# alexlee-gk/video_prediction

Measured on AMD Instinct MI355X. Metric: train frames/sec (whole node), BAIR 64x64 seq30 SAVP, higher is better.
Workload: dtype bf16

## Files before the change

include/savp_hip.h:

```cpp
#ifndef SAVP_HIP_H
#define SAVP_HIP_H

#include <stdint.h>

#ifdef __cplusplus
extern "C" {
#endif

#define SAVP_OK 0
#define SAVP_EINVAL (-1)
#define SAVP_ELAUNCH (-2)

const char* savp_version(void);

int savp_set_option(const char* name, int32_t value);
int savp_get_option(const char* name, int32_t* value);

int savp_allreduce_bucket(void* comm, void* stream, void* buf, int64_t count);

int savp_prof_event_create(void** ev);
int savp_prof_event_destroy(void* ev);
int savp_prof_arm(void* start, void* stop);
int savp_prof_armed(void);
int savp_prof_elapsed_us(void* start, void* stop, float* us);

enum { SAVP_CONV_FPROP = 0, SAVP_CONV_DGRAD = 1, SAVP_CONV_WGRAD = 2 };
enum { SAVP_PREC_F32 = 0, SAVP_PREC_BF16 = 1 };
enum { SAVP_ACT_NONE = 0, SAVP_ACT_LRELU = 1, SAVP_ACT_SIGMOID = 2, SAVP_ACT_DLRELU_FROM_OUT = 3 };

typedef struct SavpConvArgs {
    int32_t mode;
    int32_t N, D, H, W, Cx;
    int32_t Do, Ho, Wo, Cy;
    int32_t kd, kh, kw;
    int32_t sd, sh, sw;
    int32_t pd, ph, pw;
    int32_t beta;
    int32_t act;
    float alpha;
    int32_t splitk;
    int32_t tile;
    int32_t precision;
    void* x; int64_t x_sn, x_sd, x_sh, x_sw;
    void* y; int64_t y_sn, y_sd, y_sh, y_sw;
    void* w;
    const float* bias;
    const float* aux;
    const void* w_bf16;
    int32_t src_bf16;
    int32_t out_bf16;
    double* stats;
    void* ws; int64_t ws_bytes;
    int32_t dst_gap_at, dst_gap;
    const float* nb_x; int64_t nb_x_sn, nb_x_sp;
    const float *nb_mean, *nb_rstd;
    const float *nb_gamma, *nb_beta;
    double* nb_ws;
    int32_t nb_c0, nb_nc, nb_act; float nb_alpha;
    const void* w_frag;
    const void* w_frag_il;
} SavpConvArgs;

int savp_conv(void* stream, const SavpConvArgs* args);

int savp_tiled_z_weff(void* stream, const float* w, int32_t kh, int32_t kw, int32_t ph, int32_t pw, int32_t Cin, int32_t Cout,
                      int32_t z0, int32_t nz, float* weff);
int savp_tiled_z_grad(void* stream, const void* dy, int32_t dy_bf16, int64_t nimg, int32_t H, int32_t W, int32_t C,
                      const float* weff, int32_t nz, float* dz, int32_t beta, void* ws, int64_t ws_bytes);
int64_t savp_tiled_z_workspace_bytes(int64_t nimg, int32_t C);
int savp_conv_stats_ok(const SavpConvArgs* args);
int64_t savp_conv_workspace_bytes(const SavpConvArgs* args);
int savp_conv_special(const SavpConvArgs* args);


typedef struct SavpView { void* p; int64_t sn; int64_t sp; } SavpView;

typedef struct SavpInormArgs {
    int32_t N, HW, C;
    int32_t act; float alpha; float eps;
    SavpView x;
    const float* gamma; const float* beta;
    int32_t nout; SavpView out[4];
    float* mean; float* rstd;
    int32_t ndy; SavpView dy[4];
    SavpView dx; int32_t dx_beta;
    double* dgamma; double* dbeta;
    void* ws;
    int32_t ws_clean;
    int32_t out_c0[4], out_nc[4];
    int32_t dy_c0[4], dy_nc[4];
    int32_t out_bf16;
    int32_t stats_ready;
    const float* stats_shift;
    int32_t dx_bf16;
} SavpInormArgs;
int savp_instnorm_act_fwd(void* stream, const SavpInormArgs* a);
int savp_instnorm_act_bwd(void* stream, const SavpInormArgs* a);

typedef struct SavpGnormArgs {
    SavpInormArgs norm;
    int32_t G;
    double* ws_group;
    double* dsum;
} SavpGnormArgs;
int savp_groupnorm_act_fwd(void* stream, const SavpGnormArgs* a);
int savp_groupnorm_act_bwd(void* stream, const SavpGnormArgs* a);

typedef struct SavpLnLstmArgs {
    int32_t N, HW, F; float forget_bias;
    const float* gn;
    SavpView c_prev;
    float* c_pre;
    const float* cn;
    int32_t nh; SavpView h[4]; int32_t h_bf16;
    int32_t ndh; SavpView dh[4];
    const float* dc_new;
    float* dcn;
    float* dgn;
    const float* dc_pre;
    float* dc_prev;
} SavpLnLstmArgs;
int savp_lnlstm_fwd(void* stream, const SavpLnLstmArgs* a, int32_t stage);
int savp_lnlstm_bwd(void* stream, const SavpLnLstmArgs* a, int32_t stage);

typedef struct SavpLstmArgs {
    int32_t N, HW, F;
    float eps, forget_bias;
    const void* gates;
    SavpView c_prev;
    const float *gamma1, *beta1, *gamma2, *beta2;
    float* c_new;
    int32_t nh; SavpView h[4];
    float *mean1, *rstd1, *mean2, *rstd2;
    int32_t ndh; SavpView dh[4];
    const float* dc_new;
    float* dgates;
    float* dc_prev;
    double *dgamma1, *dbeta1, *dgamma2, *dbeta2;
    float* ws; int64_t ws_floats;
    float* ws_stats;
    int32_t ws_stats_clean;
    int32_t gates_bf16;
    int32_t stats1_ready;
    int32_t h_bf16;
    int32_t dgates_bf16;
    float* dgates_raw;
    int32_t no_norm;
} SavpLstmArgs;
int savp_convlstm_gates_fwd(void* stream, const SavpLstmArgs* a);
int savp_convlstm_gates_bwd(void* stream, const SavpLstmArgs* a);

int savp_tile_channels(void* stream, const float* z, int64_t R, int32_t HW, int32_t C, float scale, SavpView out, int32_t beta);
int savp_tile_channels_bf16(void* stream, const float* z, int64_t R, int32_t HW, int32_t C, float scale, SavpView out);
#define SAVP_COLSUM_WS_FLOATS (1024 * 4 * 256)
int savp_colsum(void* stream, SavpView in, int64_t R, int32_t HW, int32_t C, float scale, float* out, int32_t per_row,
                float* ws, int64_t ws_floats);
int savp_select(void* stream, int32_t N, int32_t HW, int32_t C, const int32_t* mask, SavpView a, SavpView b, int32_t nout,
                const SavpView* outs);
int savp_select_bwd(void* stream, int32_t N, int32_t HW, int32_t C, const int32_t* mask, int32_t nin, const SavpView* dins,
                    SavpView db);
int savp_gather_clips(void* stream, float* src, float* dst, const int32_t* t_start, int32_t B, int32_t clip, int64_t E,
                      int64_t src_t_stride, int32_t adjoint);
int savp_sigmoid_bwd(void* stream, SavpView dy, SavpView y, float* out, int64_t N, int32_t HW, int32_t C);
int savp_dense_fwd(void* stream, const float* x, int64_t x_row_stride, int32_t M, int64_t K, int32_t C, const float* W,
                   const float* bias, const float* scale, float* out, float* ws, int64_t ws_floats);
int savp_axpby(void* stream, int64_t n, float a, const float* x, float b, const float* y, float* out);
int savp_fill_view(void* stream, SavpView out, int64_t R, int32_t HW, int32_t C, float value);
int savp_adam(void* stream, int64_t n, float* p, const float* g, float* m, float* v, float lr_t, float beta1, float beta2,
              float eps, float gscale, const float* lr_t_dev);

int savp_cdna_kernels_fwd(void* stream, const float* raw, float* kern, int32_t N, int32_t kh, int32_t kw, int32_t K);
int savp_cdna_kernels_bwd(void* stream, const float* raw, const double* dkern, float* draw, int32_t N, int32_t kh, int32_t kw,
                          int32_t K);
typedef struct SavpCdnaArgs {
    int32_t N, H, W, C, K, kh, kw;
    SavpView img;
    const float* kern;
    SavpView out;
    SavpView dout;
    SavpView dimg; int32_t dimg_beta;
    double* dkern;
} SavpCdnaArgs;
int savp_cdna_apply_fwd(void* stream, const SavpCdnaArgs* a);
int savp_cdna_apply_bwd(void* stream, const SavpCdnaArgs* a);
#define SAVP_MAX_SOURCES 4
typedef struct SavpCdnaMultiArgs {
    int32_t N, H, W, C, K, kh, kw;
    int32_t nsrc;
    SavpView img[SAVP_MAX_SOURCES];
    const float* kern;
    SavpView out;
    SavpView dout;
    SavpView dimg[SAVP_MAX_SOURCES]; int32_t dimg_beta[SAVP_MAX_SOURCES];
    double* dkern;
} SavpCdnaMultiArgs;
int savp_cdna_apply_multi_fwd(void* stream, const SavpCdnaMultiArgs* a);
int savp_cdna_apply_multi_bwd(void* stream, const SavpCdnaMultiArgs* a);
typedef struct SavpCompositeArgs {
    int32_t N, HW, M, C;
    const float* logits;
// ... 195 lines not shown
```

video_prediction_amd/csrc/common.hip:

```cpp
#include <hip/hip_runtime.h>
#include <dlfcn.h>
#include <string.h>
#include "savp_hip.h"
#include "opts.h"
#include "conv_common.h"

extern "C" const char* savp_version(void) { return "savp_hip 0.1 gfx950"; }

thread_local hipEvent_t g_savp_prof_start = nullptr;
thread_local hipEvent_t g_savp_prof_stop = nullptr;

extern "C" int savp_prof_event_create(void** ev) {
    if (!ev) return SAVP_EINVAL;
    hipEvent_t e;
    if (hipEventCreate(&e) != hipSuccess) return SAVP_ELAUNCH;
    *ev = (void*)e;
    return SAVP_OK;
}
extern "C" int savp_prof_event_destroy(void* ev) { return (ev && hipEventDestroy((hipEvent_t)ev) == hipSuccess) ? SAVP_OK : SAVP_EINVAL; }
extern "C" int savp_prof_arm(void* start, void* stop) {
    if ((start == nullptr) != (stop == nullptr)) return SAVP_EINVAL;
    g_savp_prof_start = (hipEvent_t)start; g_savp_prof_stop = (hipEvent_t)stop;
    return SAVP_OK;
}
extern "C" int savp_prof_armed(void) { return g_savp_prof_start != nullptr; }
extern "C" int savp_prof_elapsed_us(void* start, void* stop, float* us) {
    if (!start || !stop || !us) return SAVP_EINVAL;
    float ms = 0.f;
    if (hipEventElapsedTime(&ms, (hipEvent_t)start, (hipEvent_t)stop) != hipSuccess) return SAVP_ELAUNCH;
    *us = ms * 1e3f;
    return SAVP_OK;
}

static struct { const char* name; int value; } g_opts[OPT_COUNT] = {
    {"conv_ring", 0}, {"s2dgrad", 1}, {"thin", 1}, {"wgp_cfg", 0}, {"wgp_split", 0}, {"inorm_min_hw", 64}, {"colsum_2stage", 1},
    {"dense_legacy", 0}, {"cdna_legacy", 0}, {"lstm_fused", 1}, {"ring_dma", 1}, {"lstm_q", 0}, {"ring_wwarm", 1}, {"wgp_dma", 1}, {"ring_early", 1}, {"gate_kernel", 1}, {"gate_alt", 0}, {"gate_cell", 1}, {"gate_wwarm", 1}, {"splitk_reduced", 0},
};
int savp_opt(int id) { return g_opts[id].value; }
void savp_opt_count(int id) { ++g_opts[id].value; }
extern "C" int savp_set_option(const char* name, int value) {
    if (!name) return SAVP_EINVAL;
    for (int i = 0; i < OPT_COUNT; ++i)
        if (!strcmp(g_opts[i].name, name)) { g_opts[i].value = value; return SAVP_OK; }
    return SAVP_EINVAL;
}
extern "C" int savp_get_option(const char* name, int* value) {
    if (!name || !value) return SAVP_EINVAL;
    for (int i = 0; i < OPT_COUNT; ++i)
        if (!strcmp(g_opts[i].name, name)) { *value = g_opts[i].value; return SAVP_OK; }
    return SAVP_EINVAL;
}

typedef int (*rccl_allreduce_fn)(const void*, void*, size_t, int, int, void*, hipStream_t);
extern "C" int savp_allreduce_bucket(void* comm, void* stream, void* buf, int64_t count) {
    if (!comm || !buf || count < 0) return SAVP_EINVAL;
    if (count == 0) return SAVP_OK;
    static rccl_allreduce_fn fn = nullptr;
    if (!fn) {
        void* h = dlopen("librccl.so", RTLD_NOW | RTLD_GLOBAL);
        if (!h) h = dlopen("librccl.so.1", RTLD_NOW | RTLD_GLOBAL);
        if (!h) h = dlopen("/opt/rocm/lib/librccl.so", RTLD_NOW | RTLD_GLOBAL);
        if (!h) return SAVP_ELAUNCH;
        fn = (rccl_allreduce_fn)dlsym(h, "ncclAllReduce");
        if (!fn) return SAVP_ELAUNCH;
    }
    return fn(buf, buf, (size_t)count, 7, 0, comm, (hipStream_t)stream) == 0 ? SAVP_OK : SAVP_ELAUNCH;
}

int splitk_fit(const SavpConvArgs* a, int want, long long block_elems) {
    if (want <= 1) return 1;
    if (!a->ws || a->ws_bytes <= 0 || block_elems <= 0 || (((uintptr_t)a->ws) & 15)) { savp_opt_count(OPT_SPLITK_REDUCED); return 1; }
    const long long fit = a->ws_bytes / (block_elems * (long long)sizeof(float));
    if (fit < want) savp_opt_count(OPT_SPLITK_REDUCED);
    if (fit < 2) return 1;
    return want < fit ? want : (int)fit;
}

__global__ __launch_bounds__(256) void splitk_fold_kernel(float* __restrict__ out, const float* __restrict__ part, int splitk, long long n4, long long n,
                                                          int beta, int Cd, int gap_at, int gap) {
    const long long stride = (long long)gridDim.x * 256;
    for (long long i = (long long)blockIdx.x * 256 + threadIdx.x; i < n4; i += stride) {
        float4 s = beta ? reinterpret_cast<const float4*>(out)[i] : make_float4(0.f, 0.f, 0.f, 0.f);
        for (int k = 0; k < splitk; ++k) {
            const float4 v = reinterpret_cast<const float4*>(part + (long long)k * n)[i];
            s.x += v.x; s.y += v.y; s.z += v.z; s.w += v.w;
        }
        if (gap) {
            const int c = (int)((i * 4) % Cd);
            float* e = &s.x;
// ... 66 lines not shown
```

video_prediction_amd/csrc/conv_gate.hip:

```cpp
#include "conv_common.h"
#include "opts.h"
#include <hip/hip_ext.h>
#include <type_traits>

extern thread_local hipEvent_t g_savp_prof_start;
extern thread_local hipEvent_t g_savp_prof_stop;

struct GateP {
    const unsigned short* x;
    const uint4* wfrag;
    unsigned short* y;
    double* stats;
    const void* zero16;
    int N, Cy, mtiles, ntiles;
    int wwarm;
    int F; float eps, forget_bias;
    const float* c_prev; long long cp_sn, cp_sp;
    const float *g1, *b1, *g2, *b2;
    float* c_new;
    int nh; void* h[4]; long long h_sn[4], h_sp[4]; int h16;
    float *mean1, *rstd1, *mean2, *rstd2;
};

__device__ __attribute__((aligned(16))) unsigned g_gate_zero[4] = {0u, 0u, 0u, 0u};

#ifdef SAVP_GATE_STAMPS
__device__ unsigned long long g_gate_t[4][8];
__constant__ int g_gate_blk = 0;
#define GT(i) do { if ((int)blockIdx.x == g_gate_blk && (threadIdx.x & 63) == 0) g_gate_t[threadIdx.x >> 6][i] = __builtin_readcyclecounter(); } while (0)
extern "C" int savp_debug_gate_times(unsigned long long* out) { return hipMemcpyFromSymbol(out, HIP_SYMBOL(g_gate_t), sizeof(g_gate_t)) == hipSuccess ? 0 : -1; }
extern "C" int savp_debug_gate_block(int b) { return hipMemcpyToSymbol(HIP_SYMBOL(g_gate_blk), &b, sizeof(int)) == hipSuccess ? 0 : -1; }
#else
#define GT(i) do {} while (0)
#endif

__device__ __forceinline__ void gate_touch4(const void* gsrc, unsigned lds_dst) {
    unsigned keep;
    asm volatile("s_mov_b32 %0, m0\n\ts_mov_b32 m0, %2\n\ts_nop 0\n\tglobal_load_lds_dword %1, off\n\ts_mov_b32 m0, %0"
                 : "=&s"(keep) : "v"(gsrc), "s"(lds_dst) : "memory");
}

__device__ __forceinline__ void gate_dma16(const void* gsrc, unsigned lds_dst) {
    unsigned keep;
    asm volatile("s_mov_b32 %0, m0\n\ts_mov_b32 m0, %2\n\ts_nop 0\n\tglobal_load_lds_dwordx4 %1, off\n\ts_mov_b32 m0, %0"
                 : "=&s"(keep) : "v"(gsrc), "s"(lds_dst) : "memory");
}

template <int S, int CIN, int TM, int TN, int NWN>
struct GateCfg {
    static constexpr int KH = 5, KW = 5, PAD = 2, TAPS = KH * KW;
    static constexpr int KSPLIT = 4 / NWN;
    static constexpr int PIX = 32 * TM;
    static constexpr int C8 = CIN / 8;
    static constexpr int C8P = (C8 & 1) ? C8 : C8 + 1;
    static constexpr int PXB = C8P * 16;
    static constexpr int TC = S >= 16 ? 16 : 8;
    static constexpr int TR = (S * S >= PIX) ? PIX / TC : S;
    static constexpr int NI = PIX / (TR * TC);
    static constexpr int PR = TR + 2 * PAD, PC = TC + 2 * PAD;
    static constexpr int RPAD = (256 - (4 * PXB) % 256) % 256;
    static constexpr int RP = PC * PXB + RPAD;
    static constexpr int IMGB = PR * RP;
    static constexpr int PATCHB = NI * IMGB;
    static constexpr int NCH = TAPS * C8;
    static constexpr int KS = (NCH + 1) / 2;
    static constexpr int KPAD = 8;
    static constexpr int ETABB = ((2 * (KS + KPAD) * 4) + 15) & ~15;
    static constexpr int NCW = 32 * TN;
// ... 222 lines not shown
    const int odd = kq & 1, hi = kq >> 1;
    if (!odd) xput(wave, ICH{}, ICH{}); else xput(wave, IC0{}, ICH{});
    __syncthreads();
    if (!odd) xadd(wave ^ NWN, IC0{}, ICH{}); else xadd(wave ^ NWN, ICH{}, ICH{});
    __syncthreads();
    if constexpr (KSPLIT == 4) {
        if (!odd && !hi) xput(wave, ICQ{}, ICQ{});
        else if (!odd && hi) xput(wave, IC0{}, ICQ{});
        else if (odd && !hi) xput(wave, ICHQ{}, ICQ{});
        else xput(wave, ICH{}, ICQ{});
        __syncthreads();
        if (!odd && !hi) xadd(wave ^ 2, IC0{}, ICQ{});
        else if (!odd && hi) xadd(wave ^ 2, ICQ{}, ICQ{});
        else if (odd && !hi) xadd(wave ^ 2, ICH{}, ICQ{});
        else xadd(wave ^ 2, ICHQ{}, ICQ{});
        __syncthreads();
    }
    GT(5);

#ifndef SAVP_CELL_ABL
#define SAVP_CELL_ABL 0
#endif
    if constexpr (CELL) {
        static_assert(TN == 1 && NWN == 1 && G::TR == S && G::TC == S, "plane-local cell: whole images per tile, one 32-column block per workgroup");
        constexpr int TMFc = TM / 4, HWI = S * S;
        constexpr int FINS[4] = {0, TMQ, TMH, TMH + TMQ};
        const int fin = kq == 0 ? 0 : (kq == 2 ? TMQ : (kq == 1 ? TMH : TMH + TMQ));
        const int F = p.F;
        const int ch = l31 >> 2, g = l31 & 3;
        const int cch = nt * 8 + ch;
        const int pc = g * F + cch;
        float* stat = reinterpret_cast<float*>(gsm + G::PIX * 32 * 2);
        float* stat2 = stat + 4 * 32 * 2;
        unsigned short* T16 = reinterpret_cast<unsigned short*>(gsm);
        float v[TMFc][16];
        auto grab = [&](auto fin_c) {
            constexpr int FIN = decltype(fin_c)::value;
#pragma unroll
            for (int i = 0; i < TMFc; ++i)
#pragma unroll
                for (int r = 0; r < 16; ++r) v[i][r] = acc[FIN + i][0][r];
        };
        if (kq == 0) grab(IC0{}); else if (kq == 2) grab(ICQ{}); else if (kq == 1) grab(ICH{}); else grab(ICHQ{});
        (void)FINS;
        const int pix0 = fin * 32 + 4 * khalf;
        const int im = pix0 / HWI;
        const int n = img0 + im;
        const bool live = n < p.N;
        const int nn = live ? n : p.N - 1;
        constexpr int NE = TMFc * 4;
        auto erow = [&](int i, int m) { return pix0 + i * 32 + g + 8 * m; };
        float cp[NE];
        if (p.c_prev) {
            const float* __restrict__ cpb = p.c_prev + (long long)nn * p.cp_sn + cch;
#pragma unroll
            for (int i = 0; i < TMFc; ++i)
#pragma unroll
                for (int m = 0; m < 4; ++m) cp[i * 4 + m] = cpb[(erow(i, m) % HWI) * (int)p.cp_sp];
        } else {
#pragma unroll
            for (int e = 0; e < NE; ++e) cp[e] = 0.f;
        }
        const float ga1 = p.g1[pc], be1 = p.b1[pc], ga2 = p.g2[cch], be2 = p.b2[cch];
        float xq[TMFc][16];
        {
            float sm = 0.f, q = 0.f;
#pragma unroll
            for (int i = 0; i < TMFc; ++i)
#pragma unroll
                for (int r = 0; r < 16; ++r) {
                    const float a = v[i][r];
                    sm += a; q += a * a;
                    const __bf16 b = (__bf16)a;
                    xq[i][r] = (float)b;
                    const int row = pix0 + i * 32 + (r & 3) + 8 * (r >> 2);
                    T16[row * 32 + g * 8 + ch] = __builtin_bit_cast(unsigned short, b);
                }
            sm += __shfl_xor(sm, 32); q += __shfl_xor(q, 32);
            if (khalf == 0) { stat[(kq * 32 + l31) * 2] = sm; stat[(kq * 32 + l31) * 2 + 1] = q; }
        }
        asm volatile("s_waitcnt lgkmcnt(0)" ::: "memory");
        __builtin_amdgcn_s_barrier();
        constexpr int WPI = 4 / G::NI;
        const float inv = 1.f / (float)HWI;
        float mu, rs;
        {
            float t0 = 0.f, t1 = 0.f;
#pragma unroll
            for (int o = 0; o < WPI; ++o) {
                const int ord = im * WPI + o, w = ((ord & 1) << 1) | (ord >> 1);
                t0 += stat[(w * 32 + l31) * 2]; t1 += stat[(w * 32 + l31) * 2 + 1];
            }
            const double m = (double)t0 * (double)inv;
            mu = (float)m;
            rs = rsqrtf(fmaxf((float)((double)t1 * (double)inv - m * m), 0.f) + p.eps);
        }
        const int first_of_image = (((im * WPI) & 1) << 1) | ((im * WPI) >> 1);
        if (live && kq == first_of_image && khalf == 0) { p.mean1[(long long)n * 4 * F + pc] = mu; p.rstd1[(long long)n * 4 * F + pc] = rs; }
        const float kk = g == 1 ? 2.f : 1.f;
        const float sc = -1.4426950408889634f * kk * rs * ga1, sh = -1.4426950408889634f * kk * (be1 - mu * rs * ga1 + (g == 2 ? p.forget_bias : 0.f));
        const float oa = kk, ob = 1.f - kk;
        float cpre[NE], so[NE];
        float s2 = 0.f, q2 = 0.f;
#pragma unroll
        for (int i = 0; i < TMFc; ++i)
#pragma unroll
            for (int m = 0; m < 4; ++m) {
                float a4[4];
#pragma unroll
                for (int t = 0; t < 4; ++t) {
                    const float e = __builtin_amdgcn_exp2f(xq[i][4 * m + t] * sc + sh);
                    a4[t] = __builtin_amdgcn_rcpf(1.f + e) * oa + ob;
                }
                float gk[4];
#pragma unroll
                for (int k = 0; k < 4; ++k) {
                    float b[4];
#pragma unroll
                    for (int t = 0; t < 4; ++t) {
                        const int ai = __builtin_bit_cast(int, a4[t]);
                        const int bi = k == 0 ? __builtin_amdgcn_mov_dpp(ai, 0x00, 0xF, 0xF, true) : k == 1 ? __builtin_amdgcn_mov_dpp(ai, 0x55, 0xF, 0xF, true)
                                     : k == 2 ? __builtin_amdgcn_mov_dpp(ai, 0xAA, 0xF, 0xF, true) : __builtin_amdgcn_mov_dpp(ai, 0xFF, 0xF, 0xF, true);
                        b[t] = __builtin_bit_cast(float, bi);
                    }
                    gk[k] = g == 0 ? b[0] : (g == 1 ? b[1] : (g == 2 ? b[2] : b[3]));
                }
                const float c = cp[i * 4 + m] * gk[2] + gk[0] * gk[1];
                cpre[i * 4 + m] = c; so[i * 4 + m] = gk[3];
                s2 += c; q2 += c * c;
            }
        s2 += __shfl_xor(s2, 1); q2 += __shfl_xor(q2, 1);
        s2 += __shfl_xor(s2, 2); q2 += __shfl_xor(q2, 2);
        s2 += __shfl_xor(s2, 32); q2 += __shfl_xor(q2, 32);
        if (khalf == 0 && g == 0) { stat2[(kq * 8 + ch) * 2] = s2; stat2[(kq * 8 + ch) * 2 + 1] = q2; }
        asm volatile("s_waitcnt lgkmcnt(0)" ::: "memory");
        __builtin_amdgcn_s_barrier();
        float mu2, rs2;
        {
            float t0 = 0.f, t1 = 0.f;
#pragma unroll
            for (int o = 0; o < WPI; ++o) {
                const int ord = im * WPI + o, w = ((ord & 1) << 1) | (ord >> 1);
                t0 += stat2[(w * 8 + ch) * 2]; t1 += stat2[(w * 8 + ch) * 2 + 1];
            }
            const double m = (double)t0 * (double)inv;
            mu2 = (float)m;
            rs2 = rsqrtf(fmaxf((float)((double)t1 * (double)inv - m * m), 0.f) + p.eps);
        }
        if (live && kq == first_of_image && khalf == 0 && g == 0) { p.mean2[(long long)n * F + cch] = mu2; p.rstd2[(long long)n * F + cch] = rs2; }
        GT(6);
        if (live && !(SAVP_CELL_ABL & 2)) {
            const float sc2 = rs2 * ga2, sh2 = be2 - mu2 * rs2 * ga2;
            float cn[NE], hv[NE];
#pragma unroll
            for (int e = 0; e < NE; ++e) {
                cn[e] = cpre[e] * sc2 + sh2;
                const float ee = __expf(-2.f * fabsf(cn[e]));
                hv[e] = copysignf((1.f - ee) * __builtin_amdgcn_rcpf(1.f + ee), cn[e]) * so[e];
            }
            float* __restrict__ cb = p.c_new + (long long)n * HWI * F + cch;
#pragma unroll
            for (int i = 0; i < TMFc; ++i)
#pragma unroll
                for (int m = 0; m < 4; ++m) cb[(erow(i, m) % HWI) * F] = cn[i * 4 + m];
#pragma unroll
            for (int k = 0; k < 4; ++k) {
                if (k >= p.nh) break;
                const int hsp = (int)p.h_sp[k];
                if ((p.h16 >> k) & 1) {
                    unsigned short* __restrict__ hb = reinterpret_cast<unsigned short*>(p.h[k]) + (long long)n * p.h_sn[k] + cch;
#pragma unroll
                    for (int i = 0; i < TMFc; ++i)
#pragma unroll
                        for (int m = 0; m < 4; ++m) hb[(erow(i, m) % HWI) * hsp] = __builtin_bit_cast(unsigned short, (__bf16)hv[i * 4 + m]);
                } else {
                    float* __restrict__ hb = reinterpret_cast<float*>(p.h[k]) + (long long)n * p.h_sn[k] + cch;
#pragma unroll
                    for (int i = 0; i < TMFc; ++i)
#pragma unroll
                        for (int m = 0; m < 4; ++m) hb[(erow(i, m) % HWI) * hsp] = hv[i * 4 + m];
                }
            }
        }
        for (int idx = tid; idx < G::PIX * 4; idx += 256) {
            const int pix = idx >> 2, gg = idx & 3;
            const int imp = pix / HWI, px = pix - imp * HWI;
            const int np = img0 + imp;
            if (np >= p.N) continue;
            const uint4 w = *reinterpret_cast<const uint4*>(T16 + pix * 32 + gg * 8);
            *reinterpret_cast<uint4*>(p.y + ((long long)np * HWI + px) * (long long)p.Cy + gg * F + nt * 8) = w;
        }
        GT(7);
        return;
    }

    float* stat = reinterpret_cast<float*>(gsm + (4 * G::XB > G::STGB ? 4 * G::XB : G::STGB));
    unsigned* T = reinterpret_cast<unsigned*>(gsm);
    constexpr int TMF = TM / KSPLIT;
    auto finish = [&](auto fin_c) {
        constexpr int FIN = decltype(fin_c)::value;
        const bool oddl = lane & 1;
#pragma unroll
        for (int i = FIN; i < FIN + TMF; ++i)
#pragma unroll
            for (int j = 0; j < TN; ++j) {
                const int cp = (nw * G::NCW + 32 * j + (l31 & ~1)) >> 1;
#pragma unroll
                for (int m = 0; m < 8; ++m) {
                    const float e = acc[i][j][2 * m], o = acc[i][j][2 * m + 1];
                    const float en = __builtin_bit_cast(float, __builtin_amdgcn_mov_dpp(__builtin_bit_cast(int, e), 0xB1, 0xF, 0xF, true));
                    const float on = __builtin_bit_cast(float, __builtin_amdgcn_mov_dpp(__builtin_bit_cast(int, o), 0xB1, 0xF, 0xF, true));
                    const int r = 2 * m + (oddl ? 1 : 0);
                    const int row = i * 32 + (r & 3) + 8 * (r >> 2) + 4 * khalf;
                    typedef __bf16 bf16x2 __attribute__((ext_vector_type(2)));
                    T[row * G::TP + cp] = oddl ? __builtin_bit_cast(unsigned, bf16x2{(__bf16)on, (__bf16)o}) : __builtin_bit_cast(unsigned, bf16x2{(__bf16)e, (__bf16)en});
                }
            }
        if (p.stats) {
#pragma unroll
            for (int j = 0; j < TN; ++j) {
                float sm = 0.f, q = 0.f;
#pragma unroll
                for (int i = FIN; i < FIN + TMF; ++i)
#pragma unroll
                    for (int r = 0; r < 16; ++r) { const float v = acc[i][j][r]; sm += v; q += v * v; }
                sm += __shfl_xor(sm, 32); q += __shfl_xor(q, 32);
                if (khalf == 0) { stat[(kq * NC + nw * G::NCW + 32 * j + l31) * 2] = sm; stat[(kq * NC + nw * G::NCW + 32 * j + l31) * 2 + 1] = q; }
            }
        }
    };
    if constexpr (KSPLIT == 4) {
        if (!odd && !hi) finish(IC0{});
        else if (!odd && hi) finish(ICQ{});
        else if (odd && !hi) finish(ICH{});
        else finish(ICHQ{});
    } else {
        if (!odd) finish(IC0{}); else finish(ICH{});
    }
    __syncthreads();
    GT(6);
    {
        constexpr int CH = NC / 8;
        for (int idx = tid; idx < G::PIX * CH; idx += 256) {
            const int pix = idx / CH, c8 = idx - pix * CH;
            const int im = pix / (G::TR * G::TC), rr = pix - im * (G::TR * G::TC);
            const int n = img0 + im;
            if (n >= p.N) continue;
            const int oy = ty0 + rr / G::TC, ox = tx0 + rr % G::TC;
            const uint4 v = *reinterpret_cast<const uint4*>(T + pix * G::TP + c8 * 4);
            unsigned short* dst = p.y + (((long long)n * S + oy) * S + ox) * (long long)p.Cy + n0 + c8 * 8;
            *reinterpret_cast<uint4*>(dst) = v;
        }
    }
    if (p.stats) {
        constexpr int WPI = KSPLIT / G::NI;
        for (int i = tid; i < G::NI * NC * 2; i += 256) {
            const int im = i / (NC * 2), rem = i - im * (NC * 2);
            const int n = img0 + im;
            if (n >= p.N) continue;
            float t = 0.f;
#pragma unroll
            for (int o = 0; o < WPI; ++o) {
                const int ord = im * WPI + o;
                const int q_ = KSPLIT == 4 ? (((ord & 1) << 1) | (ord >> 1)) : ord;
                t += stat[q_ * NC * 2 + rem];
            }
            unsafeAtomicAdd(p.stats + ((long long)n * p.Cy + n0 + (rem >> 1)) * 2 + (rem & 1), (double)t);
        }
    }
    GT(7);
}

#define GATE_PACK_PAD_KSTEPS 8
__global__ __launch_bounds__(256) void pack_gate_weights_kernel(const float* __restrict__ src, int taps, int Cx, int Cy, uint4* __restrict__ out, int il_F) {
    const int C8 = Cx >> 3, nch = taps * C8, KS = (nch + 1) >> 1;
    const long long total = (long long)(Cy >> 5) * KS * 64;
    for (long long t = total + (long long)blockIdx.x * 256 + threadIdx.x; t < total + GATE_PACK_PAD_KSTEPS * 64; t += (long long)gridDim.x * 256)
        out[t] = make_uint4(0u, 0u, 0u, 0u);
    for (long long t = (long long)blockIdx.x * 256 + threadIdx.x; t < total; t += (long long)gridDim.x * 256) {
        const int lane = (int)(t & 63);
        const long long r = t >> 6;
        const int ks = (int)(r % KS), cb = (int)(r / KS);
        const int c = 2 * ks + (lane >> 5);
        typedef __bf16 bf16x2 __attribute__((ext_vector_type(2)));
        unsigned w[4] = {0u, 0u, 0u, 0u};
        if (c < nch) {
            const int tap = c / C8, ch = c - tap * C8;
            const int l = lane & 31, col = il_F ? (l & 3) * il_F + cb * 8 + (l >> 2) : cb * 32 + l;
            const float* s = src + ((long long)tap * Cx + ch * 8) * Cy + col;
#pragma unroll
            for (int j = 0; j < 4; ++j) w[j] = __builtin_bit_cast(unsigned, bf16x2{(__bf16)s[(long long)(2 * j) * Cy], (__bf16)s[(long long)(2 * j + 1) * Cy]});
        }
        out[t] = make_uint4(w[0], w[1], w[2], w[3]);
    }
// ... 21 lines not shown
    static bool attr = false;
    if (!attr) {
        hipFuncSetAttribute((const void*)conv_gate_kernel<S, CIN, TM, TN, NWN, CELL>, hipFuncAttributeMaxDynamicSharedMemorySize, G::LDSB);
        attr = true;
    }
    const dim3 grid((unsigned)(p.mtiles * p.ntiles));
    if (g_savp_prof_start) {
        hipExtLaunchKernelGGL((conv_gate_kernel<S, CIN, TM, TN, NWN, CELL>), grid, dim3(256), G::LDSB, st, g_savp_prof_start, g_savp_prof_stop, 0, p);
        g_savp_prof_start = g_savp_prof_stop = nullptr;
    } else {
        hipLaunchKernelGGL((conv_gate_kernel<S, CIN, TM, TN, NWN, CELL>), grid, dim3(256), G::LDSB, st, p);
    }
    return hipGetLastError();
}

#define GATE_SHAPES(X)                                                                                                    \
    X(32, 72, 8, 1, 2, 0) X(16, 136, 4, 1, 1, 0) X(8, 264, 4, 1, 1, 0)        \
    X(32, 96, 8, 1, 2, 0) X(16, 160, 4, 1, 1, 0)                            \
    X(32, 64, 8, 1, 2, 0) X(16, 128, 4, 1, 1, 0) X(8, 256, 4, 1, 1, 0)      \
    X(32, 136, 8, 1, 2, 0) X(32, 264, 4, 1, 2, 0) X(16, 264, 4, 1, 2, 0)    \
    X(32, 72, 4, 1, 2, 1) X(16, 136, 4, 1, 2, 2) X(32, 96, 4, 1, 2, 1) X(16, 160, 4, 1, 2, 2) X(32, 72, 4, 1, 1, 4) X(32, 72, 4, 2, 1, 8)

static bool gate_shape_ok(const SavpConvArgs* a) {
#define X(S_, C_, TM_, TN_, NWN_, ALT_) if (a->H == S_ && a->Cx == C_) return true;
    GATE_SHAPES(X)
#undef X
    return false;
}

bool conv_gate_applies(const SavpConvArgs* a) {
    if (!savp_opt(OPT_GATE_KERNEL)) return false;
    if (!(a->mode == SAVP_CONV_FPROP && a->precision == SAVP_PREC_BF16 && a->src_bf16 && a->out_bf16 && a->w_frag && !a->bias && !a->aux &&
          a->act == SAVP_ACT_NONE && !a->beta && !a->dst_gap && !a->nb_ws && a->splitk <= 1))
        return false;
    if (!(a->D == 1 && a->Do == 1 && a->kd == 1 && a->kh == 5 && a->kw == 5 && a->sd == 1 && a->sh == 1 && a->sw == 1 && a->pd == 0 && a->ph == 2 &&
          a->pw == 2 && a->H == a->W && a->Ho == a->H && a->Wo == a->W))
        return false;
    if (!(a->x_sw == a->Cx && a->x_sh == (long long)a->W * a->Cx && a->x_sn == (long long)a->H * a->W * a->Cx && a->y_sw == a->Cy &&
          a->y_sh == (long long)a->W * a->Cy && a->y_sn == (long long)a->H * a->W * a->Cy && aligned16(a->x) && aligned16(a->y) && aligned16(a->w_frag)))
        return false;
    if ((a->Cy & 127) || a->N < 1 || (a->stats && (((uintptr_t)a->stats) & 7))) return false;
    return gate_shape_ok(a);
}

bool conv_gate_try(const SavpConvArgs* a, hipStream_t st, int* rc) {
    if (!conv_gate_applies(a)) return false;
    static const void* zero_of[64] = {nullptr};
    int dev_ord = 0;
    if (hipGetDevice(&dev_ord) != hipSuccess || dev_ord < 0 || dev_ord >= 64) dev_ord = 0;
    if (!zero_of[dev_ord] && hipGetSymbolAddress((void**)&zero_of[dev_ord], HIP_SYMBOL(g_gate_zero)) != hipSuccess) { *rc = SAVP_ELAUNCH; return true; }
    GateP p;
    p.x = (const unsigned short*)a->x; p.wfrag = (const uint4*)a->w_frag; p.y = (unsigned short*)a->y; p.stats = (double*)a->stats;
    p.zero16 = zero_of[dev_ord]; p.N = a->N; p.Cy = a->Cy; p.wwarm = savp_opt(OPT_GATE_WWARM);
    hipError_t err = hipErrorInvalidValue;
    const int alt = savp_opt(OPT_GATE_ALT);
    bool done = false;
#define X(S_, C_, TM_, TN_, NWN_, ALT_)                                                                  \
    if (!done && a->H == S_ && a->Cx == C_ && (want ? (ALT_ & want) != 0 : ALT_ == 0)) {                 \
        using G = GateCfg<S_, C_, TM_, TN_, NWN_>;                                                       \
        p.mtiles = G::NI == 1 ? a->N * G::TPI : (a->N + G::NI - 1) / G::NI; p.ntiles = a->Cy / G::NC;    \
        err = launch_gate<S_, C_, TM_, TN_, NWN_>(p, st);                                                \
        done = true;                                                                                     \
    }
    { const int want = alt; GATE_SHAPES(X) }
    { const int want = 0; GATE_SHAPES(X) }
#undef X
    *rc = err == hipSuccess ? SAVP_OK : SAVP_ELAUNCH;
    return true;
}

#define GATE_CELL_SHAPES(X) X(16, 136, 8) X(8, 264, 4) X(16, 160, 8) X(16, 128, 8) X(8, 256, 4)

bool conv_gate_cell_try(const SavpConvLstmCellArgs* c, hipStream_t st, int* rc) {
    const SavpConvArgs* a = &c->conv;
    const SavpLstmArgs* g = &c->gates;
    if (!savp_opt(OPT_GATE_KERNEL) || !savp_opt(OPT_GATE_CELL) || !a->w_frag_il) return false;
    SavpConvArgs b = *a;
    b.w_frag = a->w_frag_il;
    if (!b.stats) b.stats = (double*)(uintptr_t)16;
    if (!conv_gate_applies(&b)) return false;
    bool shape = false;
#define X(S_, C_, TM_) if (a->H == S_ && a->Cx == C_) shape = true;
    GATE_CELL_SHAPES(X)
#undef X
    if (!shape) return false;
    if (g->no_norm || !g->gates_bf16 || g->F * 4 != a->Cy || g->N != a->N || g->HW != a->H * a->W || g->nh < 0 || g->nh > 4 || !g->gamma1 || !g->beta1 ||
        !g->gamma2 || !g->beta2 || !g->c_new || !g->mean1 || !g->rstd1 || !g->mean2 || !g->rstd2 || (g->F & 7))
        return false;
    if (g->c_prev.sp * (long long)g->HW >= (1ll << 31)) return false;
    for (int i = 0; i < g->nh; ++i)
        if (g->h[i].sp * (long long)g->HW >= (1ll << 31)) return false;
    static const void* zero_of[64] = {nullptr};
    int dev_ord = 0;
    if (hipGetDevice(&dev_ord) != hipSuccess || dev_ord < 0 || dev_ord >= 64) dev_ord = 0;
    if (!zero_of[dev_ord] && hipGetSymbolAddress((void**)&zero_of[dev_ord], HIP_SYMBOL(g_gate_zero)) != hipSuccess) { *rc = SAVP_ELAUNCH; return true; }
    GateP p;
    p.x = (const unsigned short*)a->x; p.wfrag = (const uint4*)a->w_frag_il; p.y = (unsigned short*)a->y; p.stats = nullptr;
    p.zero16 = zero_of[dev_ord]; p.N = a->N; p.Cy = a->Cy; p.wwarm = savp_opt(OPT_GATE_WWARM);
    p.F = g->F; p.eps = g->eps; p.forget_bias = g->forget_bias;
    p.c_prev = (const float*)g->c_prev.p; p.cp_sn = g->c_prev.sn; p.cp_sp = g->c_prev.sp;
    p.g1 = g->gamma1; p.b1 = g->beta1; p.g2 = g->gamma2; p.b2 = g->beta2;
    p.c_new = g->c_new; p.nh = g->nh; p.h16 = g->h_bf16;
    for (int i = 0; i < 4; ++i) { p.h[i] = i < g->nh ? g->h[i].p : nullptr; p.h_sn[i] = i < g->nh ? g->h[i].sn : 0; p.h_sp[i] = i < g->nh ? g->h[i].sp : 0; }
    p.mean1 = g->mean1; p.rstd1 = g->rstd1; p.mean2 = g->mean2; p.rstd2 = g->rstd2;
    hipError_t err = hipErrorInvalidValue;
#define X(S_, C_, TM_)                                                                                   \
    if (a->H == S_ && a->Cx == C_) {                                                                     \
        using G = GateCfg<S_, C_, TM_, 1, 1>;                                                            \
        p.mtiles = (a->N + G::NI - 1) / G::NI; p.ntiles = a->Cy / 32;                                    \
        err = launch_gate<S_, C_, TM_, 1, 1, true>(p, st);                                               \
    }
    GATE_CELL_SHAPES(X)
#undef X
    *rc = err == hipSuccess ? SAVP_OK : SAVP_ELAUNCH;
    return true;
}
```

video_prediction_amd/csrc/conv_igemm.hip:

```cpp
#include <hip/hip_runtime.h>
#include <stdint.h>
#include "savp_hip.h"
#include "zero_fill.h"

#include "conv_common.h"
#include <stdlib.h>

template <int WM, int WN, bool VEC, bool BF16, bool WB16>
__global__ __launch_bounds__(NTHREADS) void conv_fd_kernel(ConvP p) {
    constexpr int BM = 64 * WM, BN = 64 * WN;
    constexpr int BKT = BF16 ? 64 : 32;
    constexpr int KV = BKT / 4;
    constexpr int RP = NTHREADS / KV;
    constexpr int RA = BM / RP, RB = BN / RP;
    constexpr int ROWB = BF16 ? (BKT + 8) * 2 : BKP * 4;
    extern __shared__ __attribute__((aligned(16))) float smem[];
    char* As = reinterpret_cast<char*>(smem);
    char* Bs = As + 2 * BM * ROWB;

    const bool dgrad = (p.mode == SAVP_CONV_DGRAD);
    const int split = blockIdx.z % p.splitk;
    int fz = blockIdx.z / p.splitk;
    int fw = dgrad ? fz % p.sw : 0; fz = dgrad ? fz / p.sw : 0;
    int fh = dgrad ? fz % p.sh : 0; fz = dgrad ? fz / p.sh : 0;
// ... 700 lines not shown
    if (splitk <= 0) {
        long long want = (512 + tiles - 1) / tiles;
        long long maxs = g.ktiles / 8 > 0 ? g.ktiles / 8 : 1;
        splitk = want < maxs ? want : maxs;
    }
    if (splitk > g.ktiles) splitk = g.ktiles;
    if (splitk < 1) splitk = 1;
    const long long per = (g.ktiles + splitk - 1) / splitk;
    g.splitk = (int)((g.ktiles + per - 1) / per);
    g.part_sz = g.M * a->Cy;
    return true;
}

extern "C" int64_t savp_conv_workspace_bytes(const SavpConvArgs* a) {
    if (!a) return 0;
    if (a->mode == SAVP_CONV_FPROP || a->mode == SAVP_CONV_DGRAD) {
        if (a->act != SAVP_ACT_NONE || a->out_bf16 || a->stats || a->splitk == 1) return 0;
        const bool dg = a->mode == SAVP_CONV_DGRAD;
        const long long dD = dg ? a->D : a->Do, dH = dg ? a->H : a->Ho, dW_ = dg ? a->W : a->Wo;
        const long long Cd = (dg ? a->Cx : a->Cy) + (a->dst_gap > 0 ? a->dst_gap : 0);
        const long long block = (long long)a->N * dD * dH * dW_ * Cd;
        long long S = a->splitk;
        if (S <= 0) {
            const long long tiles = ((block / Cd + 255) / 256) * ((Cd + 127) / 128);
            if (tiles > 192) return 0;
            S = 512 / tiles;
            if (S > 16) S = 16;
        }
        return S > 1 ? S * block * (long long)sizeof(float) : 0;
    }
    if (a->mode != SAVP_CONV_WGRAD) return 0;
    const int algo = (a->tile >> 8) & 3;
    long long need = 0;
    const long long thin = algo == 0 ? conv_thin_workspace_bytes(a) : 0;
    if (thin) need = thin;
    else {
        int wm = 0, wn = 0;
        if (a->tile & 0xff) { wm = (a->tile >> 4) & 15; wn = a->tile & 15; if (wm < 1 || wm > 2 || wn < 1 || wn > 2) return 0; }
        ConvP p;
        p.bf16 = (a->precision == SAVP_PREC_BF16) ? 1 : 0;
        int rc = SAVP_OK;
        long long patch_bytes = 0;
        WgPlan g;
        if (algo != 1 && conv_wgrad_patch_try(p, a, nullptr, &rc, &patch_bytes)) need = patch_bytes;
        else if (algo != 2 && wgrad_generic_plan(a, p.bf16 != 0, wm, wn, g) && g.splitk > 1) need = (long long)g.splitk * g.part_sz * (long long)sizeof(float);
        const long long bias = a->bias ? (long long)SAVP_COLSUM_WS_FLOATS * 4 : 0;
        if (bias > need) need = bias;
    }
    return need;
}

extern "C" int savp_conv_special(const SavpConvArgs* a) {
    if (a && conv_gate_applies(a)) return 1;
    if (!a || ((a->tile >> 8) & 3) != 0) return 0;
    return (conv_thin_applies(a) || conv_s2dgrad_applies(a) || conv_gate_applies(a)) ? 1 : 0;
}

extern "C" int savp_conv_stats_ok(const SavpConvArgs* a) {
    if (!a || (a->mode != SAVP_CONV_FPROP && a->mode != SAVP_CONV_DGRAD) || a->precision != SAVP_PREC_BF16) return 0;
    if (((a->tile >> 8) & 3) == 0 && (conv_thin_applies(a) || conv_s2dgrad_applies(a))) return 0;
    const bool dg = a->mode == SAVP_CONV_DGRAD;
    const int Cred = dg ? a->Cy : a->Cx;
    if (!(a->w_bf16 && (Cred % 8 == 0) && aligned16(a->w_bf16))) return 0;
    ConvP p;
    p.bf16 = 1; p.w16 = (const unsigned short*)a->w_bf16; p.src16 = a->src_bf16 ? 1 : 0; p.splitk = 1; p.tm = p.tn = 1;
    p.gap_at = a->dst_gap ? a->dst_gap_at : 0x7fffffff; p.gap = a->dst_gap;
    p.nb_ws = (double*)a->nb_ws; p.nb_c0 = a->nb_c0; p.nb_nc = a->nb_nc; p.part = nullptr; p.part_sz = 0;
    if (a->dst_gap && !a->nb_ws) return 0;
    SavpConvArgs b = *a;
    if (!b.stats && !b.nb_ws) b.stats = (double*)(uintptr_t)16;
    int wm = 0, wn = 0;
    if (b.tile & 0xff) { wm = (b.tile >> 4) & 15; wn = b.tile & 15; if (wm < 1 || wm > 2 || wn < 1 || wn > 2) return 0; }
    int rc = SAVP_OK;
    return conv_ring_try(p, &b, wm, wn, nullptr, &rc, true) ? 1 : 0;
}

extern "C" int savp_conv(void* stream, const SavpConvArgs* a) {
    if (!a || !a->x || !a->y || !a->w) return SAVP_EINVAL;
    if (a->sd < 1 || a->sh < 1 || a->sw < 1 || a->kd < 1 || a->kh < 1 || a->kw < 1) return SAVP_EINVAL;
    hipStream_t st = (hipStream_t)stream;
    ConvP p;
    p.mode = a->mode;
    p.N = a->N; p.D = a->D; p.H = a->H; p.W = a->W; p.Cx = a->Cx;
    p.Do = a->Do; p.Ho = a->Ho; p.Wo = a->Wo; p.Cy = a->Cy;
    p.kd = a->kd; p.kh = a->kh; p.kw = a->kw; p.sd = a->sd; p.sh = a->sh; p.sw = a->sw;
    p.pd = a->pd; p.ph = a->ph; p.pw = a->pw;
    p.beta = a->beta; p.act = a->act; p.alpha = a->alpha;
    p.x = (const float*)a->x; p.x_sn = a->x_sn; p.x_sd = a->x_sd; p.x_sh = a->x_sh; p.x_sw = a->x_sw;
    p.y = (const float*)a->y; p.y_sn = a->y_sn; p.y_sd = a->y_sd; p.y_sh = a->y_sh; p.y_sw = a->y_sw;
    p.w = (const float*)a->w;
    p.w16 = nullptr;
    p.bias = a->bias; p.aux = a->aux;
    p.splitk = 1; p.tm = p.tn = 1; p.part = nullptr; p.part_sz = 0;
    p.src16 = a->src_bf16 ? 1 : 0; p.cell = 0; p.stats = nullptr;
    p.bf16 = (a->precision == SAVP_PREC_BF16) ? 1 : 0;
    const bool gapped = a->dst_gap != 0;
    if (gapped && (a->dst_gap < 0 || a->dst_gap_at < 0 || a->mode == SAVP_CONV_WGRAD)) return SAVP_EINVAL;
    p.gap_at = gapped ? a->dst_gap_at : 0x7fffffff; p.gap = gapped ? a->dst_gap : 0;
    p.nb_ws = (double*)a->nb_ws;
    if (a->nb_ws) {
        if (a->mode == SAVP_CONV_WGRAD || !a->nb_x || !a->nb_mean || !a->nb_rstd || !a->nb_gamma || !a->nb_beta || a->nb_c0 < 0 || a->nb_nc < 1 ||
            a->nb_act < 0 || a->nb_act > 2)
            return SAVP_EINVAL;
        p.nb_x = a->nb_x; p.nb_x_sn = a->nb_x_sn; p.nb_x_sp = a->nb_x_sp; p.nb_mean = a->nb_mean; p.nb_rstd = a->nb_rstd;
        p.nb_gamma = a->nb_gamma; p.nb_beta = a->nb_beta; p.nb_c0 = a->nb_c0; p.nb_nc = a->nb_nc; p.nb_act = a->nb_act; p.nb_alpha = a->nb_alpha;
    }
    p.magW = magic40(a->Wo); p.magHW = magic40(a->Ho * a->Wo); p.magDHW = magic40(a->Do * a->Ho * a->Wo);
    int wm = 0, wn = 0;
    const int algo = (a->tile >> 8) & 3;
    if (a->tile & 0xff) { wm = (a->tile >> 4) & 15; wn = a->tile & 15; if (wm < 1 || wm > 2 || wn < 1 || wn > 2) return SAVP_EINVAL; }
    hipError_t err;
    ablate_init();
    const bool xs4 = (a->x_sn % 4 == 0) && (a->x_sd % 4 == 0) && (a->x_sh % 4 == 0) && (a->x_sw % 4 == 0) && aligned16(a->x);
    const bool ys4 = (a->y_sn % 4 == 0) && (a->y_sd % 4 == 0) && (a->y_sh % 4 == 0) && (a->y_sw % 4 == 0) && aligned16(a->y);
    if (algo == 0 && !gapped && !a->nb_ws) {
        int rc = SAVP_OK;
        if (conv_thin_try(a, st, &rc)) return rc;
    }
    if (algo == 0 && !gapped && !a->nb_ws && a->mode == SAVP_CONV_DGRAD) {
        int rc = SAVP_OK;
        if (conv_s2dgrad_try(a, st, &rc)) return rc;
    }
    if (a->mode == SAVP_CONV_FPROP) {
        int rc = SAVP_OK;
        if (conv_gate_try(a, st, &rc)) return rc;
    }
    if (a->mode == SAVP_CONV_FPROP || a->mode == SAVP_CONV_DGRAD) {
        const bool dg = a->mode == SAVP_CONV_DGRAD;
        p.out = (float*)(dg ? a->x : a->y);
        const int Cred = dg ? a->Cy : a->Cx;
        const int Nout = dg ? a->Cx : a->Cy;
        const bool vec = (Cred % 4 == 0) && (dg ? ys4 : xs4) && aligned16(a->w);
        if (a->w_bf16 && (Cred % 8 == 0) && aligned16(a->w_bf16)) p.w16 = (const unsigned short*)a->w_bf16;
        long long Mmax;
        int phases = 1;
        if (dg) {
            phases = a->sd * a->sh * a->sw;
            Mmax = (long long)a->N * ((a->D + a->sd - 1) / a->sd) * ((a->H + a->sh - 1) / a->sh) * ((a->W + a->sw - 1) / a->sw);
        } else {
            Mmax = (long long)a->N * a->Do * a->Ho * a->Wo;
        }
        if (Mmax <= 0 || Nout <= 0) return SAVP_EINVAL;
        const bool needs_ring = a->out_bf16 || a->src_bf16 || a->stats || gapped || a->nb_ws;
        if (algo == 3 || needs_ring || (algo == 0 && ring_default())) {
            int rc = SAVP_OK;
            if (conv_ring_try(p, a, wm, wn, st, &rc)) return rc;
            if (algo == 3 || needs_ring) return SAVP_EINVAL;
        }
        if (algo != 1) {
            int rc = SAVP_OK;
            if (conv_patch_try(p, a, wm, wn, algo == 2, st, &rc)) return rc;
            if (algo == 2) return SAVP_EINVAL;
        }
        if (!wm) pick_tile(Mmax * phases, Nout, wm, wn);
        const int BM = 64 * wm, BN = 64 * wn;
        int splitk = a->splitk;
        const long long tiles = ((Mmax + BM - 1) / BM) * ((Nout + BN - 1) / BN) * phases;
        const long long taps_max = (long long)a->kd * a->kh * a->kw / (dg ? phases : 1);
        const long long nkt = (taps_max * Cred + (p.bf16 ? 63 : 31)) / (p.bf16 ? 64 : 32);
        const bool can_split = (a->act == SAVP_ACT_NONE);
        if (!can_split) splitk = 1;
        else if (splitk <= 0) {
            splitk = 1;
            if (tiles <= 192 && nkt >= 16) {
                long long s1 = 512 / tiles, s2 = nkt / 8;
                splitk = (int)(s1 < s2 ? s1 : s2);
                if (splitk < 1) splitk = 1;
                if (splitk > 16) splitk = 16;
            }
        }
        if (splitk > 1) {
            const long long dD = dg ? a->D : a->Do, dH = dg ? a->H : a->Ho, dW_ = dg ? a->W : a->Wo;
            const long long s_n = dg ? a->x_sn : a->y_sn, s_d = dg ? a->x_sd : a->y_sd, s_h = dg ? a->x_sh : a->y_sh,
                            s_w = dg ? a->x_sw : a->y_sw;
            const bool dense = (s_w == Nout) && (s_h == dW_ * Nout) && (dD == 1 || s_d == dH * dW_ * Nout) &&
                               (s_n == dD * dH * dW_ * Nout);
            if (!dense) splitk = 1;
            else {
                p.part_sz = (long long)a->N * dD * dH * dW_ * Nout;
// ... 69 lines not shown
```

video_prediction_amd/csrc/fused_ops.hip:

```cpp
#include <hip/hip_runtime.h>
#include <stdint.h>
#include "savp_hip.h"

bool conv_gate_cell_try(const SavpConvLstmCellArgs* c, hipStream_t st, int* rc);

extern "C" int savp_convlstm_cell_fwd(void* stream, const SavpConvLstmCellArgs* a) {
    if (!a || a->conv.mode != SAVP_CONV_FPROP) return SAVP_EINVAL;
    const SavpConvArgs& c = a->conv;
    const SavpLstmArgs& g = a->gates;
    if (c.y != g.gates || (c.out_bf16 != 0) != (g.gates_bf16 != 0)) return SAVP_EINVAL;
    if (c.Cy != 4 * g.F || c.N != g.N || (long long)c.Do * c.Ho * c.Wo != g.HW) return SAVP_EINVAL;
    if ((c.stats != nullptr) != (g.stats1_ready != 0)) return SAVP_EINVAL;
    if (c.stats && (void*)c.stats != g.ws_stats) return SAVP_EINVAL;
    if (c.stats && c.bias) return SAVP_EINVAL;
    {
        int rc1 = SAVP_OK;
        if (conv_gate_cell_try(a, (hipStream_t)stream, &rc1)) return rc1;
    }
    int rc = savp_conv(stream, &c);
    if (rc != SAVP_OK) return rc;
    return savp_convlstm_gates_fwd(stream, &g);
}

extern "C" int savp_convlstm_cell_bwd(void* stream, const SavpConvLstmCellArgs* a) {
    if (!a || a->conv.mode != SAVP_CONV_DGRAD) return SAVP_EINVAL;
    const SavpConvArgs& c = a->conv;
    const SavpLstmArgs& g = a->gates;
    if (c.y != (void*)g.dgates || (c.src_bf16 != 0) != (g.dgates_bf16 != 0)) return SAVP_EINVAL;
    if (c.Cy != 4 * g.F || c.N != g.N || (long long)c.Do * c.Ho * c.Wo != g.HW) return SAVP_EINVAL;
    int rc = savp_convlstm_gates_bwd(stream, &g);
    if (rc != SAVP_OK) return rc;
    return savp_conv(stream, &c);
}

extern "C" int savp_conv_in_act_fwd(void* stream, const SavpConvNormArgs* a) {
    if (!a || (a->conv.mode != SAVP_CONV_FPROP && a->conv.mode != SAVP_CONV_DGRAD)) return SAVP_EINVAL;
    const SavpConvArgs& c = a->conv;
    const SavpInormArgs& n = a->norm;
    const void* dst = c.mode == SAVP_CONV_FPROP ? c.y : c.x;
    const int cdst = c.mode == SAVP_CONV_FPROP ? c.Cy : c.Cx;
    if (dst != n.x.p || cdst != n.C || c.N != n.N) return SAVP_EINVAL;
    if ((c.stats != nullptr) != (n.stats_ready != 0)) return SAVP_EINVAL;
    if (c.stats && (c.stats != n.ws || (c.bias != nullptr) != (n.stats_shift != nullptr) || (c.bias && c.bias != n.stats_shift))) return SAVP_EINVAL;
    int rc = savp_conv(stream, &c);
    if (rc != SAVP_OK) return rc;
    return savp_instnorm_act_fwd(stream, &n);
}

extern "C" int savp_conv_in_act_bwd(void* stream, const SavpConvNormArgs* a) {
    if (!a || (a->conv.mode != SAVP_CONV_FPROP && a->conv.mode != SAVP_CONV_DGRAD)) return SAVP_EINVAL;
    const SavpConvArgs& c = a->conv;
    const SavpInormArgs& n = a->norm;
    const void* src = c.mode == SAVP_CONV_DGRAD ? c.y : c.x;
    if (src != n.dx.p || (c.src_bf16 != 0) != (n.dx_bf16 != 0) || c.N != n.N) return SAVP_EINVAL;
    int rc = savp_instnorm_act_bwd(stream, &n);
    if (rc != SAVP_OK) return rc;
    return savp_conv(stream, &c);
}
```

video_prediction_amd/csrc/norm_lstm.hip:

```cpp
#include <hip/hip_runtime.h>
#include <hip/hip_ext.h>
#include <stdint.h>
#include <stdlib.h>
#include "savp_hip.h"
#include "zero_fill.h"
extern thread_local hipEvent_t g_savp_prof_start, g_savp_prof_stop;
#include "opts.h"

#define NT 256

__device__ __forceinline__ float wave_sum(float v) {
#pragma unroll
    for (int o = 32; o > 0; o >>= 1) v += __shfl_xor(v, o);
    return v;
}

template <int NV>
__device__ __forceinline__ void block_sum(float (&v)[NV], float* sh) {
    const int lane = threadIdx.x & 63, wave = threadIdx.x >> 6;
    __syncthreads();
#pragma unroll
    for (int i = 0; i < NV; ++i) {
        float s = wave_sum(v[i]);
        if (lane == 0) sh[wave * NV + i] = s;
// ... 384 lines not shown
    p.x = (const float*)a->x.p; p.x_sn = a->x.sn; p.x_sp = a->x.sp;
    p.gamma = a->gamma; p.beta = a->beta; p.eps = a->eps; p.act = a->act; p.alpha = a->alpha;
    p.mean = a->mean; p.rstd = a->rstd;
    p.ndy = a->ndy;
    for (int i = 0; i < a->ndy; ++i) {
        p.dy[i] = (const float*)a->dy[i].p; p.dy_sn[i] = a->dy[i].sn; p.dy_sp[i] = a->dy[i].sp;
        p.dy_c0[i] = a->dy_c0[i]; p.dy_c1[i] = a->dy_nc[i] > 0 ? a->dy_c0[i] + a->dy_nc[i] : a->C;
        if ((p.dy_c0[i] & 3) || (p.dy_c1[i] & 3) || p.dy_c0[i] < 0 || p.dy_c1[i] > a->C) return SAVP_EINVAL;
    }
    p.dx = (float*)a->dx.p; p.dx_sn = a->dx.sn; p.dx_sp = a->dx.sp; p.dx_beta = a->dx_beta;
    p.dx16 = a->dx_bf16 ? 1 : 0;
    if (p.dx16 && (a->dx_beta || (a->dx.sn & 3) || (a->dx.sp & 3) || (((uintptr_t)a->dx.p) & 7))) return SAVP_EINVAL;
    p.dgamma = a->dgamma; p.dbeta = a->dbeta;
    if (a->stats_ready) {
        if (!a->ws || a->C > 256 || (NT % (a->C / 4)) != 0) return SAVP_EINVAL;
        hipStream_t st = (hipStream_t)stream;
        p.chunk = inorm_chunk(a);
        dim3 grid((a->HW + p.chunk - 1) / p.chunk, a->N);
        hipLaunchKernelGGL(inorm_bwd_apply_kernel, grid, dim3(NT), 0, st, p, (const double*)a->ws);
        return hipGetLastError() == hipSuccess ? SAVP_OK : SAVP_ELAUNCH;
    }
    if (use_large_plane_path(a)) {
        hipStream_t st = (hipStream_t)stream;
        if (!a->ws_clean) savp_zero_async(a->ws, (size_t)a->N * a->C * 2 * sizeof(double), st);
        p.chunk = inorm_chunk(a);
        dim3 grid((a->HW + p.chunk - 1) / p.chunk, a->N);
        size_t lds = (size_t)(NT / (a->C / 4)) * 2 * a->C * sizeof(float);
        hipLaunchKernelGGL(inorm_bwd_stats_kernel, grid, dim3(NT), lds, st, p, (double*)a->ws);
        hipLaunchKernelGGL(inorm_bwd_apply_kernel, grid, dim3(NT), 0, st, p, (const double*)a->ws);
        return hipGetLastError() == hipSuccess ? SAVP_OK : SAVP_ELAUNCH;
    }
    hipLaunchKernelGGL(inorm_bwd_kernel, dim3(a->N * (a->C / 4)), dim3(NT), 0, (hipStream_t)stream, p);
    return hipGetLastError() == hipSuccess ? SAVP_OK : SAVP_ELAUNCH;
}

#define MAXPPT 4
struct LstmP {
    int N, HW, F;
    const float* gates;
    int gates16, stats1_ready;
    const float* c_prev; long long cp_sn, cp_sp;
    const float *g1, *b1, *g2, *b2;
    float eps, forget_bias;
    float* c_new;
    int nh; float* h[4]; long long h_sn[4], h_sp[4];
    int h16[4];
    float *mean1, *rstd1, *mean2, *rstd2;
    int ndh; const float* dh[4]; long long dh_sn[4], dh_sp[4];
    const float* dc_new;
    float* dgates;
    float* draw;
    int dgates16;
    float* dc_prev;
    double *dg1, *db1, *dg2, *db2;
};

__global__ __launch_bounds__(NT) void lstm_fwd_kernel(LstmP p) {
    __shared__ float sh[4 * 16];
    const int cg = p.F / 4;
    const int n = blockIdx.x / cg, c0 = (blockIdx.x % cg) * 4;
    const int F = p.F;
    const float* gp = p.gates + (long long)n * p.HW * 4 * F + c0;
    float4 gi[MAXPPT], gj[MAXPPT], gf[MAXPPT], go[MAXPPT];
    float s[16];
#pragma unroll
    for (int i = 0; i < 16; ++i) s[i] = 0.f;
#pragma unroll
    for (int t = 0; t < MAXPPT; ++t) {
        const int px = threadIdx.x + t * NT;
        if (px < p.HW) {
            const float* q = gp + (long long)px * 4 * F;
            gi[t] = ld4(q); gj[t] = ld4(q + F); gf[t] = ld4(q + 2 * F); go[t] = ld4(q + 3 * F);
            s[0] += gi[t].x; s[1] += gi[t].y; s[2] += gi[t].z; s[3] += gi[t].w;
            s[4] += gj[t].x; s[5] += gj[t].y; s[6] += gj[t].z; s[7] += gj[t].w;
            s[8] += gf[t].x; s[9] += gf[t].y; s[10] += gf[t].z; s[11] += gf[t].w;
            s[12] += go[t].x; s[13] += go[t].y; s[14] += go[t].z; s[15] += go[t].w;
        }
    }
    block_sum<16>(s, sh);
    const float inv = 1.f / (float)p.HW;
    float mu[16];
#pragma unroll
    for (int i = 0; i < 16; ++i) mu[i] = s[i] * inv;
#pragma unroll
    for (int i = 0; i < 16; ++i) s[i] = 0.f;
#define SQ(a, m) (((a) - (m)) * ((a) - (m)))
#pragma unroll
    for (int t = 0; t < MAXPPT; ++t) {
        const int px = threadIdx.x + t * NT;
        if (px < p.HW) {
            s[0] += SQ(gi[t].x, mu[0]); s[1] += SQ(gi[t].y, mu[1]); s[2] += SQ(gi[t].z, mu[2]); s[3] += SQ(gi[t].w, mu[3]);
            s[4] += SQ(gj[t].x, mu[4]); s[5] += SQ(gj[t].y, mu[5]); s[6] += SQ(gj[t].z, mu[6]); s[7] += SQ(gj[t].w, mu[7]);
            s[8] += SQ(gf[t].x, mu[8]); s[9] += SQ(gf[t].y, mu[9]); s[10] += SQ(gf[t].z, mu[10]); s[11] += SQ(gf[t].w, mu[11]);
            s[12] += SQ(go[t].x, mu[12]); s[13] += SQ(go[t].y, mu[13]); s[14] += SQ(go[t].z, mu[14]); s[15] += SQ(go[t].w, mu[15]);
        }
    }
    block_sum<16>(s, sh);
    float rs[16];
#pragma unroll
    for (int i = 0; i < 16; ++i) rs[i] = rsqrtf(s[i] * inv + p.eps);
    if (threadIdx.x < 16) {
        const int q = threadIdx.x >> 2, c = threadIdx.x & 3;
        p.mean1[(long long)n * 4 * F + q * F + c0 + c] = mu[threadIdx.x];
        p.rstd1[(long long)n * 4 * F + q * F + c0 + c] = rs[threadIdx.x];
    }
    float ga[16], be[16];
// ... 507 lines not shown
    __syncthreads();
    {
        const int i = tid % NV, rest = tid / NV, q = rest % Q, pt = rest / Q;
        float s = 0.f;
#pragma unroll
        for (int k = 0; k < NV; ++k) s += sh[((pt * NV + k) * Q + q) * (NV + 1) + i];
        part[tid] = s;
    }
    __syncthreads();
    constexpr int NP = NT / (NV * Q);
    if (tid < NV * Q) {
        const int i = tid % NV, q = tid / NV;
        float s = 0.f;
#pragma unroll
        for (int k = 0; k < NP; ++k) s += part[(k * Q + q) * NV + i];
        fin[q * NV + i] = s;
    }
    __syncthreads();
    const int q = tid & (Q - 1);
#pragma unroll
    for (int i = 0; i < NV; ++i) v[i] = fin[q * NV + i];
}

#ifdef SAVP_LSTM_STAMPS
__device__ unsigned long long g_lstm_t[3][8];
#define LT(i) do { if (threadIdx.x == 0 && (blockIdx.x == 0 || blockIdx.x == gridDim.x / 2 || blockIdx.x == gridDim.x - 1)) \
    g_lstm_t[blockIdx.x == 0 ? 0 : (blockIdx.x == gridDim.x - 1 ? 2 : 1)][i] = __builtin_readcyclecounter(); } while (0)
#define LT_WAITVM() asm volatile("s_waitcnt vmcnt(0)" ::: "memory")
extern "C" int savp_debug_lstm_times(unsigned long long* out) {
    return hipMemcpyFromSymbol(out, HIP_SYMBOL(g_lstm_t), sizeof(g_lstm_t)) == hipSuccess ? 0 : -1;
}
#else
#define LT(i) do {} while (0)
#define LT_WAITVM() do {} while (0)
#endif

template <bool G16> struct GateQuad;
template <> struct GateQuad<true> {
    uint2 u;
    __device__ __forceinline__ void load(const float* base, long long idx) {
        u = *reinterpret_cast<const uint2*>(reinterpret_cast<const unsigned short*>(base) + idx);
    }
    __device__ __forceinline__ void get(float* o) const {
        o[0] = __uint_as_float(u.x << 16); o[1] = __uint_as_float(u.x & 0xffff0000u);
        o[2] = __uint_as_float(u.y << 16); o[3] = __uint_as_float(u.y & 0xffff0000u);
    }
};
template <> struct GateQuad<false> {
    float4 v;
    __device__ __forceinline__ void load(const float* base, long long idx) { v = ld4(base + idx); }
    __device__ __forceinline__ void get(float* o) const { o[0] = v.x; o[1] = v.y; o[2] = v.z; o[3] = v.w; }
};

__device__ __forceinline__ void lstm_block_owner(int nslab, int xcd_map, int& n, int& slab) {
    const int b = blockIdx.x;
    if (xcd_map) { const int r = b >> 3; slab = r % nslab; n = (b & 7) + 8 * (r / nslab); }
    else { n = b / nslab; slab = b % nslab; }
}

template <int Q, int PPT, bool G16>
__global__ __launch_bounds__(NT) void lstm_fused_fwd_kernel(LstmP p, const double* __restrict__ s1, int nslab, int xcd_map) {
    __shared__ float sh[LSTM_SUM_FLOATS(16, Q)];
    LT(0);
    constexpr int ROWS = NT / Q;
    int n, slab;
    lstm_block_owner(nslab, xcd_map, n, slab);
    const int q = threadIdx.x & (Q - 1), prow = threadIdx.x / Q;
    const int F = p.F, HW = p.HW, c0 = (slab * Q + q) * 4;
    const long long g0 = (long long)n * HW * 4 * F + c0;
    GateQuad<G16> gq[PPT][4];
    float4 cpq[PPT];
    int pxs[PPT];
    bool ok[PPT];
#pragma unroll
    for (int t = 0; t < PPT; ++t) {
        const int px = prow + t * ROWS;
        ok[t] = px < HW;
        pxs[t] = ok[t] ? px : HW - 1;
        const long long idx = g0 + (long long)pxs[t] * 4 * F;
#pragma unroll
        for (int g = 0; g < 4; ++g) gq[t][g].load(p.gates, idx + g * F);
    }
    if (p.c_prev) {
#pragma unroll
        for (int t = 0; t < PPT; ++t) cpq[t] = ld4(p.c_prev + (long long)n * p.cp_sn + (long long)pxs[t] * p.cp_sp + c0);
    } else {
#pragma unroll
        for (int t = 0; t < PPT; ++t) cpq[t] = make_float4(0.f, 0.f, 0.f, 0.f);
    }
    float4 g1q[4], b1q[4];
    double2 sd[4][4];
#pragma unroll
    for (int g = 0; g < 4; ++g) { g1q[g] = ld4(p.g1 + g * F + c0); b1q[g] = ld4(p.b1 + g * F + c0); }
    if (s1) {
#pragma unroll
        for (int g = 0; g < 4; ++g) {
            const double2* s = reinterpret_cast<const double2*>(s1 + ((long long)n * 4 * F + g * F + c0) * 2);
#pragma unroll
            for (int c = 0; c < 4; ++c) sd[g][c] = s[c];
        }
    }
    const float4 g2q = ld4(p.g2 + c0), b2q = ld4(p.b2 + c0);
    LT(1);
    LT_WAITVM();
    LT(2);
    const float inv = 1.f / (float)HW;
    float x[PPT][16];
#pragma unroll
    for (int t = 0; t < PPT; ++t)
#pragma unroll
        for (int g = 0; g < 4; ++g) gq[t][g].get(&x[t][g * 4]);
    float mu[16], rs[16];
    if (s1) {
#pragma unroll
        for (int g = 0; g < 4; ++g) {
#pragma unroll
            for (int c = 0; c < 4; ++c) {
                const double m = sd[g][c].x * (double)inv;
                mu[g * 4 + c] = (float)m;
                rs[g * 4 + c] = rsqrtf(fmaxf((float)(sd[g][c].y * (double)inv - m * m), 0.f) + p.eps);
            }
        }
    } else {
        float s[16];
#pragma unroll
        for (int i = 0; i < 16; ++i) s[i] = 0.f;
#pragma unroll
        for (int t = 0; t < PPT; ++t)
#pragma unroll
            for (int i = 0; i < 16; ++i) s[i] += ok[t] ? x[t][i] : 0.f;
        block_sum_q<16, Q>(s, sh);
#pragma unroll
        for (int i = 0; i < 16; ++i) { mu[i] = s[i] * inv; s[i] = 0.f; }
#pragma unroll
        for (int t = 0; t < PPT; ++t)
#pragma unroll
            for (int i = 0; i < 16; ++i) { const float d = x[t][i] - mu[i]; s[i] += ok[t] ? d * d : 0.f; }
        block_sum_q<16, Q>(s, sh);
// ... 9 lines not shown
        }
    }
    float ga[16], be[16];
#pragma unroll
    for (int g = 0; g < 4; ++g) {
        ga[g * 4] = g1q[g].x; ga[g * 4 + 1] = g1q[g].y; ga[g * 4 + 2] = g1q[g].z; ga[g * 4 + 3] = g1q[g].w;
        be[g * 4] = b1q[g].x; be[g * 4 + 1] = b1q[g].y; be[g * 4 + 2] = b1q[g].z; be[g * 4 + 3] = b1q[g].w;
    }
    float cpre[PPT][4], so[PPT][4];
    float s2[4] = {0.f, 0.f, 0.f, 0.f};
#pragma unroll
    for (int t = 0; t < PPT; ++t) {
        const float cpv[4] = {cpq[t].x, cpq[t].y, cpq[t].z, cpq[t].w};
#pragma unroll
        for (int c = 0; c < 4; ++c) {
            const float in_ = (x[t][c] - mu[c]) * rs[c] * ga[c] + be[c];
            const float jn = (x[t][4 + c] - mu[4 + c]) * rs[4 + c] * ga[4 + c] + be[4 + c];
            const float fn = (x[t][8 + c] - mu[8 + c]) * rs[8 + c] * ga[8 + c] + be[8 + c];
            const float on = (x[t][12 + c] - mu[12 + c]) * rs[12 + c] * ga[12 + c] + be[12 + c];
            cpre[t][c] = cpv[c] * sigmoidf_(fn + p.forget_bias) + sigmoidf_(in_) * tanhf_(jn);
            so[t][c] = sigmoidf_(on);
            s2[c] += ok[t] ? cpre[t][c] : 0.f;
        }
    }
    LT(3);
    block_sum_q<4, Q>(s2, sh);
    LT(4);
    float mu2[4], rs2[4];
#pragma unroll
    for (int c = 0; c < 4; ++c) { mu2[c] = s2[c] * inv; s2[c] = 0.f; }
#pragma unroll
    for (int t = 0; t < PPT; ++t)
#pragma unroll
        for (int c = 0; c < 4; ++c) { const float d = cpre[t][c] - mu2[c]; s2[c] += ok[t] ? d * d : 0.f; }
    block_sum_q<4, Q>(s2, sh);
#pragma unroll
    for (int c = 0; c < 4; ++c) rs2[c] = rsqrtf(s2[c] * inv + p.eps);
    if (prow == 0) {
        st4(p.mean2 + (long long)n * F + c0, make_float4(mu2[0], mu2[1], mu2[2], mu2[3]));
        st4(p.rstd2 + (long long)n * F + c0, make_float4(rs2[0], rs2[1], rs2[2], rs2[3]));
    }
    const float g2v[4] = {g2q.x, g2q.y, g2q.z, g2q.w}, b2v[4] = {b2q.x, b2q.y, b2q.z, b2q.w};
    LT(5);
#pragma unroll
    for (int t = 0; t < PPT; ++t) {
        if (!ok[t]) continue;
        float cn[4], hv[4];
#pragma unroll
        for (int c = 0; c < 4; ++c) {
            cn[c] = (cpre[t][c] - mu2[c]) * rs2[c] * g2v[c] + b2v[c];
            hv[c] = tanhf_(cn[c]) * so[t][c];
        }
        const int px = pxs[t];
        st4(p.c_new + ((long long)n * HW + px) * F + c0, make_float4(cn[0], cn[1], cn[2], cn[3]));
        const float4 h4 = make_float4(hv[0], hv[1], hv[2], hv[3]);
#pragma unroll
        for (int k = 0; k < 4; ++k)
            if (k < p.nh) st4x(p.h[k], (long long)n * p.h_sn[k] + (long long)px * p.h_sp[k] + c0, h4, p.h16[k]);
    }
    LT(6);
    LT_WAITVM();
    LT(7);
}

template <int Q, int PPT, bool G16>
__global__ __launch_bounds__(NT) void lstm_fused_bwd_kernel(LstmP p, int nslab, int xcd_map) {
    __shared__ float sh[LSTM_SUM_FLOATS(32, Q)];
    LT(0);
    constexpr int ROWS = NT / Q;
    int n, slab;
    lstm_block_owner(nslab, xcd_map, n, slab);
    const int q = threadIdx.x & (Q - 1), prow = threadIdx.x / Q;
    const int F = p.F, HW = p.HW, c0 = (slab * Q + q) * 4;
    const long long g0 = (long long)n * HW * 4 * F + c0;
    GateQuad<G16> gq[PPT][4];
    float4 cpq[PPT], dhq[PPT], dcq[PPT];
    int pxs[PPT];
    float okf[PPT];
#pragma unroll
    for (int t = 0; t < PPT; ++t) {
        const int px = prow + t * ROWS;
        okf[t] = px < HW ? 1.f : 0.f;
        pxs[t] = px < HW ? px : HW - 1;
        const long long idx = g0 + (long long)pxs[t] * 4 * F;
#pragma unroll
        for (int g = 0; g < 4; ++g) gq[t][g].load(p.gates, idx + g * F);
        dhq[t] = make_float4(0.f, 0.f, 0.f, 0.f);
        cpq[t] = make_float4(0.f, 0.f, 0.f, 0.f);
        dcq[t] = make_float4(0.f, 0.f, 0.f, 0.f);
    }
    if (p.c_prev) {
#pragma unroll
        for (int t = 0; t < PPT; ++t) cpq[t] = ld4(p.c_prev + (long long)n * p.cp_sn + (long long)pxs[t] * p.cp_sp + c0);
    }
    if (p.dc_new) {
#pragma unroll
        for (int t = 0; t < PPT; ++t) dcq[t] = ld4(p.dc_new + ((long long)n * HW + pxs[t]) * F + c0);
    }
    float4 dhs[3][PPT];
    {
        const int nd = p.ndh > 0 ? p.ndh : 1;
#pragma unroll
        for (int k = 0; k < 3; ++k) {
            const int kk = k < nd ? k : nd - 1;
            const float* src = p.ndh > 0 ? p.dh[kk] : p.gates;
            const long long sn = p.ndh > 0 ? p.dh_sn[kk] : 0, sp = p.ndh > 0 ? p.dh_sp[kk] : 0;
#pragma unroll
            for (int t = 0; t < PPT; ++t) dhs[k][t] = ld4(src + (long long)n * sn + (long long)pxs[t] * sp + (p.ndh > 0 ? c0 : 0));
        }
    }
    if (p.ndh > 3) {
#pragma unroll
        for (int t = 0; t < PPT; ++t) dhq[t] = ld4(p.dh[3] + (long long)n * p.dh_sn[3] + (long long)pxs[t] * p.dh_sp[3] + c0);
    }
    float mu[16], rs[16], ga[16], be[16];
#pragma unroll
    for (int g = 0; g < 4; ++g) {
        const long long o = (long long)n * 4 * F + g * F + c0;
        const float4 m = ld4(p.mean1 + o), r = ld4(p.rstd1 + o), gg = ld4(p.g1 + g * F + c0), bb = ld4(p.b1 + g * F + c0);
        mu[g * 4] = m.x; mu[g * 4 + 1] = m.y; mu[g * 4 + 2] = m.z; mu[g * 4 + 3] = m.w;
        rs[g * 4] = r.x; rs[g * 4 + 1] = r.y; rs[g * 4 + 2] = r.z; rs[g * 4 + 3] = r.w;
        ga[g * 4] = gg.x; ga[g * 4 + 1] = gg.y; ga[g * 4 + 2] = gg.z; ga[g * 4 + 3] = gg.w;
        be[g * 4] = bb.x; be[g * 4 + 1] = bb.y; be[g * 4 + 2] = bb.z; be[g * 4 + 3] = bb.w;
    }
    const float4 m2q = ld4(p.mean2 + (long long)n * F + c0), r2q = ld4(p.rstd2 + (long long)n * F + c0), g2q = ld4(p.g2 + c0), b2q = ld4(p.b2 + c0);
    const float mu2[4] = {m2q.x, m2q.y, m2q.z, m2q.w}, rs2[4] = {r2q.x, r2q.y, r2q.z, r2q.w};
    const float g2v[4] = {g2q.x, g2q.y, g2q.z, g2q.w}, b2v[4] = {b2q.x, b2q.y, b2q.z, b2q.w};
    const float inv = 1.f / (float)HW;
    LT(1);
    LT_WAITVM();
    LT(2);
    float xh[PPT][16];
    float dg[PPT][16];
    float dz[PPT][4];
    float r2[8];
#pragma unroll
    for (int i = 0; i < 8; ++i) r2[i] = 0.f;
#pragma unroll
    for (int t = 0; t < PPT; ++t) {
        float raw[16];
#pragma unroll
        for (int g = 0; g < 4; ++g) gq[t][g].get(&raw[g * 4]);
#pragma unroll
        for (int i = 0; i < 16; ++i) xh[t][i] = (raw[i] - mu[i]) * rs[i];
        const float cpv[4] = {cpq[t].x, cpq[t].y, cpq[t].z, cpq[t].w};
        float dhv[4] = {dhq[t].x, dhq[t].y, dhq[t].z, dhq[t].w};
#pragma unroll
        for (int k = 0; k < 3; ++k) {
            const float wk = k < p.ndh ? 1.f : 0.f;
            dhv[0] += wk * dhs[k][t].x; dhv[1] += wk * dhs[k][t].y; dhv[2] += wk * dhs[k][t].z; dhv[3] += wk * dhs[k][t].w;
        }
        const float dcnv[4] = {dcq[t].x, dcq[t].y, dcq[t].z, dcq[t].w};
#pragma unroll
        for (int c = 0; c < 4; ++c) {
            const float in_ = xh[t][c] * ga[c] + be[c];
            const float jn = xh[t][4 + c] * ga[4 + c] + be[4 + c];
            const float fn = xh[t][8 + c] * ga[8 + c] + be[8 + c];
            const float on = xh[t][12 + c] * ga[12 + c] + be[12 + c];
            const float cpre = cpv[c] * sigmoidf_(fn + p.forget_bias) + sigmoidf_(in_) * tanhf_(jn);
            const float x2 = (cpre - mu2[c]) * rs2[c];
            const float th = tanhf_(x2 * g2v[c] + b2v[c]), so = sigmoidf_(on);
            dz[t][c] = (dhv[c] * so * (1.f - th * th) + dcnv[c]) * okf[t];
            dg[t][12 + c] = dhv[c] * th * so * (1.f - so) * okf[t];
            r2[c] += dz[t][c]; r2[4 + c] += dz[t][c] * x2;
        }
    }
    LT(3);
    block_sum_q<8, Q>(r2, sh);
    LT(4);
    if (prow == 0) {
#pragma unroll
        for (int c = 0; c < 4; ++c) { unsafeAtomicAdd(p.db2 + c0 + c, r2[c]); unsafeAtomicAdd(p.dg2 + c0 + c, r2[4 + c]); }
    }
    float r1[32];
#pragma unroll
    for (int i = 0; i < 32; ++i) r1[i] = 0.f;
#pragma unroll
    for (int t = 0; t < PPT; ++t) {
        const float cpv[4] = {cpq[t].x, cpq[t].y, cpq[t].z, cpq[t].w};
        float dcp[4];
#pragma unroll
        for (int c = 0; c < 4; ++c) {
            const float in_ = xh[t][c] * ga[c] + be[c];
            const float jn = xh[t][4 + c] * ga[4 + c] + be[4 + c];
            const float fn = xh[t][8 + c] * ga[8 + c] + be[8 + c];
            const float si = sigmoidf_(in_), tj = tanhf_(jn), sf = sigmoidf_(fn + p.forget_bias);
            const float x2 = (cpv[c] * sf + si * tj - mu2[c]) * rs2[c];
            const float dcpre = g2v[c] * rs2[c] * (dz[t][c] - r2[c] * inv - x2 * r2[4 + c] * inv) * okf[t];
            dcp[c] = dcpre * sf;
            dg[t][c] = dcpre * tj * si * (1.f - si);
            dg[t][4 + c] = dcpre * si * (1.f - tj * tj);
            dg[t][8 + c] = dcpre * cpv[c] * sf * (1.f - sf);
        }
        if (p.dc_prev && okf[t] != 0.f) st4(p.dc_prev + ((long long)n * HW + pxs[t]) * F + c0, make_float4(dcp[0], dcp[1], dcp[2], dcp[3]));
#pragma unroll
        for (int i = 0; i < 16; ++i) { r1[i] += dg[t][i]; r1[16 + i] += dg[t][i] * xh[t][i]; }
    }
    LT(5);
    block_sum_q<32, Q>(r1, sh);
    LT(6);
    if (prow == 0) {
#pragma unroll
        for (int g = 0; g < 4; ++g)
#pragma unroll
            for (int c = 0; c < 4; ++c) {
                unsafeAtomicAdd(p.db1 + g * F + c0 + c, r1[g * 4 + c]);
                unsafeAtomicAdd(p.dg1 + g * F + c0 + c, r1[16 + g * 4 + c]);
            }
    }
#pragma unroll
    for (int t = 0; t < PPT; ++t) {
        if (okf[t] == 0.f) continue;
        const long long idx = g0 + (long long)pxs[t] * 4 * F;
#pragma unroll
        for (int g = 0; g < 4; ++g) {
            float o[4];
#pragma unroll
            for (int c = 0; c < 4; ++c) {
                const int i = g * 4 + c;
                o[c] = ga[i] * rs[i] * (dg[t][i] - r1[i] * inv - xh[t][i] * r1[16 + i] * inv);
            }
            st4x(p.dgates, idx + g * F, make_float4(o[0], o[1], o[2], o[3]), p.dgates16);
        }
    }
    LT_WAITVM();
    LT(7);
}

static bool lstm_fused_cfg(const SavpLstmArgs* a, bool fwd, int& Q, int& PPT, int& nslab, int& xcd_map) {
    if (!savp_opt(OPT_LSTM_FUSED) || a->F % 4 || a->HW < 1 || a->HW > 4 * NT || a->N < 1) return false;
    if (fwd && a->gates_bf16 && !a->stats1_ready) return false;
    if (fwd && a->stats1_ready && !a->ws_stats) return false;
    Q = 1;
    for (int c = 4; c > 1; c >>= 1)
        if (a->F % (4 * c) == 0 && a->HW <= 4 * (NT / c) && (long long)a->N * (a->F / (4 * c)) >= 256) { Q = c; break; }
    const int fq = savp_opt(OPT_LSTM_Q);
    if ((fq == 1 || fq == 2 || fq == 4) && a->F % (4 * fq) == 0 && a->HW <= 4 * (NT / fq)) Q = fq;
    const int rows = NT / Q;
    PPT = a->HW <= rows ? 1 : (a->HW <= 2 * rows ? 2 : 4);
    nslab = a->F / (4 * Q);
    xcd_map = (a->N % 8 == 0) ? 1 : 0;
    return true;
}

#define LSTM_FUSED_DISPATCH(KERNEL, ...)                                                                                   \
    do {                                                                                                                   \
        const dim3 grid((unsigned)(a->N * nslab));                                                                         \
        if (a->gates_bf16) {                                                                                               \
            if (Q == 1) { if (PPT == 1) KERNEL(1, 1, true, __VA_ARGS__); else if (PPT == 2) KERNEL(1, 2, true, __VA_ARGS__); else KERNEL(1, 4, true, __VA_ARGS__); } \
            else if (Q == 2) { if (PPT == 1) KERNEL(2, 1, true, __VA_ARGS__); else if (PPT == 2) KERNEL(2, 2, true, __VA_ARGS__); else KERNEL(2, 4, true, __VA_ARGS__); } \
            else { if (PPT == 1) KERNEL(4, 1, true, __VA_ARGS__); else if (PPT == 2) KERNEL(4, 2, true, __VA_ARGS__); else KERNEL(4, 4, true, __VA_ARGS__); } \
        } else {                                                                                                           \
            if (Q == 1) { if (PPT == 1) KERNEL(1, 1, false, __VA_ARGS__); else if (PPT == 2) KERNEL(1, 2, false, __VA_ARGS__); else KERNEL(1, 4, false, __VA_ARGS__); } \
            else if (Q == 2) { if (PPT == 1) KERNEL(2, 1, false, __VA_ARGS__); else if (PPT == 2) KERNEL(2, 2, false, __VA_ARGS__); else KERNEL(2, 4, false, __VA_ARGS__); } \
            else { if (PPT == 1) KERNEL(4, 1, false, __VA_ARGS__); else if (PPT == 2) KERNEL(4, 2, false, __VA_ARGS__); else KERNEL(4, 4, false, __VA_ARGS__); } \
        }                                                                                                                  \
    } while (0)
#define LSTM_FWD_LAUNCH(Q_, P_, G_, ...)                                                                                      \
    do {                                                                                                                   \
        if (g_savp_prof_start) {                                                                                           \
            hipExtLaunchKernelGGL((lstm_fused_fwd_kernel<Q_, P_, G_>), grid, dim3(NT), 0, st, g_savp_prof_start, g_savp_prof_stop, 0, __VA_ARGS__); \
            g_savp_prof_start = g_savp_prof_stop = nullptr;                                                                \
        } else hipLaunchKernelGGL((lstm_fused_fwd_kernel<Q_, P_, G_>), grid, dim3(NT), 0, st, __VA_ARGS__);                \
    } while (0)
#define LSTM_BWD_LAUNCH(Q_, P_, G_, ...) hipLaunchKernelGGL((lstm_fused_bwd_kernel<Q_, P_, G_>), grid, dim3(NT), 0, st, __VA_ARGS__)

static int fill_lstm(LstmP& p, const SavpLstmArgs* a) {
    if (!a || a->F % 4 || a->HW < 1) return SAVP_EINVAL;
    p.N = a->N; p.HW = a->HW; p.F = a->F;
    p.gates = (const float*)a->gates; p.gates16 = a->gates_bf16 ? 1 : 0; p.stats1_ready = a->stats1_ready ? 1 : 0;
    p.c_prev = (const float*)a->c_prev.p; p.cp_sn = a->c_prev.sn; p.cp_sp = a->c_prev.sp;
    p.g1 = a->gamma1; p.b1 = a->beta1; p.g2 = a->gamma2; p.b2 = a->beta2;
    p.eps = a->eps; p.forget_bias = a->forget_bias;
    p.c_new = a->c_new;
    p.nh = a->nh;
    if (a->nh < 0 || a->nh > 4 || a->ndh < 0 || a->ndh > 4) return SAVP_EINVAL;
    for (int i = 0; i < a->nh; ++i) { p.h[i] = (float*)a->h[i].p; p.h_sn[i] = a->h[i].sn; p.h_sp[i] = a->h[i].sp; p.h16[i] = (a->h_bf16 >> i) & 1; }
    p.mean1 = a->mean1; p.rstd1 = a->rstd1; p.mean2 = a->mean2; p.rstd2 = a->rstd2;
    p.ndh = a->ndh;
    for (int i = 0; i < a->ndh; ++i) { p.dh[i] = (const float*)a->dh[i].p; p.dh_sn[i] = a->dh[i].sn; p.dh_sp[i] = a->dh[i].sp; }
    p.dc_new = a->dc_new; p.dgates = a->dgates; p.dc_prev = a->dc_prev;
    p.dgates16 = a->dgates_bf16 ? 1 : 0;
    p.draw = a->dgates_bf16 ? a->dgates_raw : a->dgates;
    p.dg1 = a->dgamma1; p.db1 = a->dbeta1; p.dg2 = a->dgamma2; p.db2 = a->dbeta2;
    return SAVP_OK;
}

#define LSTM_RED_FLOATS 22
static long long lstm_ws_floats(const SavpLstmArgs* a) { return (long long)a->N * a->F * ((a->ws_stats ? 0 : LSTM_RED_FLOATS) + (long long)a->HW); }
static bool lstm_coalesced_ok(const SavpLstmArgs* a) {
    const int F = a->F;
    return a->ws && a->ws_floats >= lstm_ws_floats(a) && F >= 16 && F <= 256 && (F & (F - 1)) == 0 && a->HW >= 16;
}

__global__ __launch_bounds__(NT) void lstm_plain_fwd_kernel(LstmP p) {
    const int F4 = p.F >> 2;
    const long long total = (long long)p.N * p.HW * F4;
    for (long long i = (long long)blockIdx.x * NT + threadIdx.x; i < total; i += (long long)gridDim.x * NT) {
        const int c0 = (int)(i % F4) * 4;
        const long long px = i / F4;
        const int n = (int)(px / p.HW), q = (int)(px - (long long)n * p.HW);
        const float* g = p.gates + px * 4 * p.F + c0;
        const float4 gi = ld4(g), gj = ld4(g + p.F), gf = ld4(g + 2 * p.F), go = ld4(g + 3 * p.F);
        float4 cp = make_float4(0.f, 0.f, 0.f, 0.f);
        if (p.c_prev) cp = ld4(p.c_prev + (long long)n * p.cp_sn + (long long)q * p.cp_sp + c0);
        const float iv[4] = {gi.x, gi.y, gi.z, gi.w}, jv[4] = {gj.x, gj.y, gj.z, gj.w}, fv[4] = {gf.x, gf.y, gf.z, gf.w},
                    ov[4] = {go.x, go.y, go.z, go.w}, cv[4] = {cp.x, cp.y, cp.z, cp.w};
        float cn[4], h[4];
#pragma unroll
        for (int c = 0; c < 4; ++c) {
            cn[c] = cv[c] * sigmoidf_(fv[c] + p.forget_bias) + sigmoidf_(iv[c]) * tanhf_(jv[c]);
            h[c] = tanhf_(cn[c]) * sigmoidf_(ov[c]);
        }
        st4(p.c_new + px * p.F + c0, make_float4(cn[0], cn[1], cn[2], cn[3]));
        for (int k = 0; k < p.nh; ++k)
            st4x(p.h[k], (long long)n * p.h_sn[k] + (long long)q * p.h_sp[k] + c0, make_float4(h[0], h[1], h[2], h[3]), p.h16[k]);
    }
}

__global__ __launch_bounds__(NT) void lstm_plain_bwd_kernel(LstmP p) {
    const int F4 = p.F >> 2;
    const long long total = (long long)p.N * p.HW * F4;
    for (long long i = (long long)blockIdx.x * NT + threadIdx.x; i < total; i += (long long)gridDim.x * NT) {
        const int c0 = (int)(i % F4) * 4;
        const long long px = i / F4;
        const int n = (int)(px / p.HW), q = (int)(px - (long long)n * p.HW);
        const float* g = p.gates + px * 4 * p.F + c0;
        const float4 gi = ld4(g), gj = ld4(g + p.F), gf = ld4(g + 2 * p.F), go = ld4(g + 3 * p.F);
        float4 cp = make_float4(0.f, 0.f, 0.f, 0.f), dcn = cp, dh4 = cp;
        if (p.c_prev) cp = ld4(p.c_prev + (long long)n * p.cp_sn + (long long)q * p.cp_sp + c0);
        if (p.dc_new) dcn = ld4(p.dc_new + px * p.F + c0);
        for (int k = 0; k < p.ndh; ++k) {
            const float4 t = ld4(p.dh[k] + (long long)n * p.dh_sn[k] + (long long)q * p.dh_sp[k] + c0);
            dh4.x += t.x; dh4.y += t.y; dh4.z += t.z; dh4.w += t.w;
        }
        const float iv[4] = {gi.x, gi.y, gi.z, gi.w}, jv[4] = {gj.x, gj.y, gj.z, gj.w}, fv[4] = {gf.x, gf.y, gf.z, gf.w},
                    ov[4] = {go.x, go.y, go.z, go.w}, cv[4] = {cp.x, cp.y, cp.z, cp.w}, dhv[4] = {dh4.x, dh4.y, dh4.z, dh4.w},
                    dcv[4] = {dcn.x, dcn.y, dcn.z, dcn.w};
        float di[4], dj[4], df[4], dO[4], dcp[4];
#pragma unroll
        for (int c = 0; c < 4; ++c) {
            const float si = sigmoidf_(iv[c]), tj = tanhf_(jv[c]), sf = sigmoidf_(fv[c] + p.forget_bias), so = sigmoidf_(ov[c]);
            const float tc = tanhf_(cv[c] * sf + si * tj);
            const float dc = dhv[c] * so * (1.f - tc * tc) + dcv[c];
            di[c] = dc * tj * si * (1.f - si);
            dj[c] = dc * si * (1.f - tj * tj);
            df[c] = dc * cv[c] * sf * (1.f - sf);
            dO[c] = dhv[c] * tc * so * (1.f - so);
            dcp[c] = dc * sf;
        }
        float* d = p.dgates + px * 4 * p.F + c0;
        st4(d, make_float4(di[0], di[1], di[2], di[3])); st4(d + p.F, make_float4(dj[0], dj[1], dj[2], dj[3]));
        st4(d + 2 * p.F, make_float4(df[0], df[1], df[2], df[3])); st4(d + 3 * p.F, make_float4(dO[0], dO[1], dO[2], dO[3]));
        if (p.dc_prev) st4(p.dc_prev + px * p.F + c0, make_float4(dcp[0], dcp[1], dcp[2], dcp[3]));
    }
}

static int lstm_plain(void* stream, const SavpLstmArgs* a, const LstmP& p, bool fwd) {
    if (a->gates_bf16 || a->dgates_bf16 || a->stats1_ready || !a->gates || (((uintptr_t)a->gates) & 15)) return SAVP_EINVAL;
    if (fwd ? !a->c_new : !a->dgates) return SAVP_EINVAL;
    const long long total = (long long)a->N * a->HW * (a->F / 4);
    long long blocks = (total + NT - 1) / NT;
    if (blocks > 4096) blocks = 4096;
    if (fwd) hipLaunchKernelGGL(lstm_plain_fwd_kernel, dim3((unsigned)blocks), dim3(NT), 0, (hipStream_t)stream, p);
    else hipLaunchKernelGGL(lstm_plain_bwd_kernel, dim3((unsigned)blocks), dim3(NT), 0, (hipStream_t)stream, p);
    return hipGetLastError() == hipSuccess ? SAVP_OK : SAVP_ELAUNCH;
}

extern "C" int savp_convlstm_gates_fwd(void* stream, const SavpLstmArgs* a) {
    LstmP p;
    int rc = fill_lstm(p, a);
    if (rc) return rc;
    if (a->no_norm) return lstm_plain(stream, a, p, true);
    hipStream_t st = (hipStream_t)stream;
    {
        int Q, PPT, nslab, xcd_map;
        if (lstm_fused_cfg(a, true, Q, PPT, nslab, xcd_map)) {
            const double* s1 = a->stats1_ready ? (const double*)a->ws_stats : nullptr;
            LSTM_FUSED_DISPATCH(LSTM_FWD_LAUNCH, p, s1, nslab, xcd_map);
            return hipGetLastError() == hipSuccess ? SAVP_OK : SAVP_ELAUNCH;
        }
    }
    if (lstm_coalesced_ok(a)) {
        const int N = a->N, F = a->F, HW = a->HW;
        LstmWs w;
        float* red = a->ws_stats ? a->ws_stats : a->ws;
        if (((uintptr_t)red) & 7) return SAVP_EINVAL;
        w.s1 = reinterpret_cast<double*>(red);
        w.s2 = w.s1 + (size_t)N * 4 * F * 2; w.k2 = reinterpret_cast<float*>(w.s2 + (size_t)N * F * 2);
        w.so = a->ws_stats ? a->ws : red + (size_t)N * F * LSTM_RED_FLOATS;
        if (a->stats1_ready && !a->ws_stats) return SAVP_EINVAL;
        if (!a->stats1_ready) {
        if (!(a->ws_stats && a->ws_stats_clean)) savp_zero_async(w.s1, (size_t)N * F * 20 * sizeof(float), st);
        if (a->gates_bf16) return SAVP_EINVAL;
        InormP q;
        q.N = N; q.HW = HW; q.C = 4 * F;
        q.x = (const float*)a->gates; q.x_sn = (long long)HW * 4 * F; q.x_sp = 4 * F;
        const int rows1 = NT / F;
        long long c1 = ((long long)HW * N + 511) / 512;
        if (c1 < rows1) c1 = rows1;
        if (c1 > 256) c1 = 256;
        q.chunk = (int)c1;
        hipLaunchKernelGGL(inorm_stats_kernel, dim3((HW + q.chunk - 1) / q.chunk, N), dim3(NT), (size_t)rows1 * 2 * 4 * F * sizeof(float), st,
                           q, w.s1);
        }
        const int rows2 = NT / (F / 4);
        long long c2 = ((long long)HW * N + 511) / 512;
        if (c2 < rows2) c2 = rows2;
        if (c2 > 256) c2 = 256;
        dim3 grid((HW + (int)c2 - 1) / (int)c2, N);
        hipLaunchKernelGGL(lstm_cell_kernel, grid, dim3(NT), (size_t)rows2 * 2 * F * sizeof(float), st, p, w, (int)c2);
        hipLaunchKernelGGL(lstm_out_kernel, grid, dim3(NT), 0, st, p, w, (int)c2);
        return hipGetLastError() == hipSuccess ? SAVP_OK : SAVP_ELAUNCH;
    }
    if (a->HW > MAXPPT * NT || a->gates_bf16 || a->stats1_ready) return SAVP_EINVAL;
    hipLaunchKernelGGL(lstm_fwd_kernel, dim3(a->N * (a->F / 4)), dim3(NT), 0, st, p);
    return hipGetLastError() == hipSuccess ? SAVP_OK : SAVP_ELAUNCH;
}

extern "C" int savp_convlstm_gates_bwd(void* stream, const SavpLstmArgs* a) {
    LstmP p;
    int rc = fill_lstm(p, a);
    if (rc) return rc;
    if (a->no_norm) return lstm_plain(stream, a, p, false);
    {
        int Q, PPT, nslab, xcd_map;
        if (lstm_fused_cfg(a, false, Q, PPT, nslab, xcd_map)) {
            hipStream_t st = (hipStream_t)stream;
            LSTM_FUSED_DISPATCH(LSTM_BWD_LAUNCH, p, nslab, xcd_map);
            return hipGetLastError() == hipSuccess ? SAVP_OK : SAVP_ELAUNCH;
        }
    }
    if (a->dgates_bf16 && !a->dgates_raw) return SAVP_EINVAL;
    if (lstm_coalesced_ok(a)) {
        hipStream_t st = (hipStream_t)stream;
        const int N = a->N, F = a->F, HW = a->HW;
        LstmBws w;
        float* red = a->ws_stats ? a->ws_stats : a->ws;
        if (((uintptr_t)red) & 7) return SAVP_EINVAL;
        w.r2 = reinterpret_cast<double*>(red);
        w.r1 = w.r2 + (size_t)N * F * 2;
        w.dz2 = a->ws_stats ? a->ws : red + (size_t)N * F * LSTM_RED_FLOATS;
        if (!(a->ws_stats && a->ws_stats_clean)) savp_zero_async(w.r2, (size_t)N * F * 20 * sizeof(float), st);
        const int rows = NT / (F / 4);
        long long c = ((long long)HW * N + 511) / 512;
        if (c < rows) c = rows;
        if (c > 256) c = 256;
        dim3 grid((HW + (int)c - 1) / (int)c, N);
        hipLaunchKernelGGL(lstm_bwd1_kernel, grid, dim3(NT), (size_t)rows * 2 * F * sizeof(float), st, p, w, (int)c);
        hipLaunchKernelGGL(lstm_bwd2_kernel, grid, dim3(NT), (size_t)rows * 8 * F * sizeof(float), st, p, w, (int)c);
        hipLaunchKernelGGL(lstm_bwd3_kernel, grid, dim3(NT), 0, st, p, w, (int)c);
        return hipGetLastError() == hipSuccess ? SAVP_OK : SAVP_ELAUNCH;
    }
    if (a->HW > MAXPPT * NT || a->gates_bf16 || a->dgates_bf16) return SAVP_EINVAL;
    hipLaunchKernelGGL(lstm_bwd_kernel, dim3(a->N * (a->F / 4)), dim3(NT), 0, (hipStream_t)stream, p);
    return hipGetLastError() == hipSuccess ? SAVP_OK : SAVP_ELAUNCH;
}
```

video_prediction_amd/csrc/opts.h:

```cpp
#pragma once

enum SavpOptId {
    OPT_CONV_RING = 0,
    OPT_S2DGRAD,
    OPT_THIN,
    OPT_WGP_CFG,
    OPT_WGP_SPLIT,
    OPT_INORM_MIN_HW,
    OPT_COLSUM_2STAGE,
    OPT_DENSE_LEGACY,
    OPT_CDNA_LEGACY,
    OPT_LSTM_FUSED,
    OPT_RING_DMA,
    OPT_LSTM_Q,
    OPT_RING_WWARM,
    OPT_WGP_DMA,
    OPT_RING_EARLY,
    OPT_GATE_KERNEL,
    OPT_GATE_ALT,
    OPT_GATE_CELL,
    OPT_GATE_WWARM,
    OPT_SPLITK_REDUCED,
    OPT_COUNT
};

int savp_opt(int id);
void savp_opt_count(int id);

#ifdef __HIPCC__
template <int BYTES>
__device__ __forceinline__ void kernarg_warm() {
    constexpr int LINES = (BYTES + 63) / 64;
    const unsigned long long ka = (unsigned long long)__builtin_amdgcn_kernarg_segment_ptr();
    unsigned t[LINES];
#pragma unroll
    for (int i = 0; i < LINES; ++i) asm volatile("s_load_dword %0, %1, %2" : "=&s"(t[i]) : "s"(ka), "n"(i * 64) : "memory");
    asm volatile("s_waitcnt lgkmcnt(0)" ::: "memory");
#pragma unroll
    for (int i = 0; i < LINES; ++i) asm volatile("" :: "s"(t[i]));
}
#endif
```

video_prediction_amd/engine.py:

```python
import math
import os
from collections import OrderedDict

import numpy as np
import torch

from . import kernels as K
from . import lib
from .variables import is_trainable


def _align4(n):
    return (n + 3) // 4 * 4


class Arena(object):

    def __init__(self, shapes, device):
        self.offsets = OrderedDict()
        off = 0
        for name, shape in shapes.items():
            n = int(np.prod(shape)) if len(shape) else 1
            self.offsets[name] = (off, n, tuple(shape))
            off += _align4(n)
# ... 214 lines not shown
        self.need_wt = self.need_wd = True
        self.wfrag = None
        self.wfrag_il = None
        self.prof = None
        self.ktimer = None

    def sn_entry(self, update_u=False):
        return {'W': self.W, 'u': self.u.reshape(-1), 'ws': self.sn_ws, 'u_new': self.u_next.reshape(-1) if update_u else None}

    def sn_bwd_entry(self):
        return {'W': self.W, 'u': self.u.reshape(-1), 'ws': self.sn_ws, 'G': self.dwf, 'dW': self.dW, 'beta': 1}

    def prep(self, update_u=False, sn_done=False, defer_pack=None):
        scale = None
        if self.kind == 'pool':
            K.fold_pool(self.W, self.wf, self.W.shape[0])
        elif self.kind == 'up':
            k, _, cin, f = self.W.shape
            K.fold_bilinear(self.W, self.wf, k, cin, f)
        if self.sn_u_name:
            if not sn_done:
                K.sn_fwd(self.W, self.u.reshape(-1), self.sn_ws, self.u_next.reshape(-1) if update_u else None)
            scale = self.sn_ws[1:2]
        src = self.wf
        if self.padded:
            copy_view(self.wf.reshape(self.taps, self.cx0, self.cy0), [self.wfp[:, :self.cx0, :self.cy0]])
            if self.bias is not None:
                K.axpby(1.0, self.bias_master, 0.0, None, self.bias[:self.cy0])
            src = self.wfp
        b16 = K.PRECISION['value'] == 1
        entry = {'src': src, 'wt': self.wt if self.need_wt else None, 'wd': self.wd if self.need_wd else None, 'scale': scale,
                 'wt16': self.wt16 if (b16 and self.need_wt) else None, 'wd16': self.wd16 if (b16 and self.need_wd) else None}
        if defer_pack is not None:
            defer_pack.append(entry)
        else:
            K.pack_weights(**entry)
        if self.wfrag is not None and b16:
            K.pack_gate_weights(src, self.wfrag)
            if self.wfrag_il is not None:
                K.pack_gate_weights(src, self.wfrag_il, interleave=True)

    def enable_gate_pack(self, cell=False):
        if self.kind == 'conv' and not self.padded and not self.sn_u_name:
            n = K.gate_weights_elems(self.taps, self.cx, self.cy)
            if n:
                self.wfrag = torch.empty(n, device=self.W.device, dtype=torch.bfloat16)
                if cell and self.cy % 32 == 0:
                    self.wfrag_il = torch.empty(n, device=self.W.device, dtype=torch.bfloat16)

    def commit_u(self):
        if self.sn_u_name:
            self.u.copy_(self.u_next)

    def forward(self, x, y, beta=0, act=0, alpha=0.0, use_bias=True, stats=None, defer=False):
        b = self.bias if use_bias else None
        if self.kind == 'conv' and x.dim() == 2 and x.shape[0] <= 64 and not act and not beta and y.is_contiguous():
            if defer:
                return None
            K.dense_fwd(x, self.W.reshape(-1, self.cy), b, y, scale=self.sn_ws[1:2] if self.sn_u_name else None)
            return
        if defer:
            if self.ktimer is not None or self.prof is not None:
                return None
            if self.kind == 'up':
                return K.conv(lib.CONV_DGRAD, self.geom, y, x, self.wd, bias=b, beta=beta, act=act, alpha=alpha, w16=self.wd16, stats=stats,
                              defer=True)
            return K.conv(lib.CONV_FPROP, self.geom, x, y, self.wt, bias=b, beta=beta, act=act, alpha=alpha, w16=self.wt16, stats=stats,
                          defer=True, w_frag=self.wfrag, w_frag_il=self.wfrag_il)
        if self.ktimer is not None:
            self.ktimer.arm()
        if self.prof is not None:
            e0, e1 = torch.cuda.Event(enable_timing=True), torch.cuda.Event(enable_timing=True)
            e0.record()
        if self.kind == 'up':
            K.conv(lib.CONV_DGRAD, self.geom, y, x, self.wd, bias=b, beta=beta, act=act, alpha=alpha, w16=self.wd16, stats=stats)
        else:
            K.conv(lib.CONV_FPROP, self.geom, x, y, self.wt, bias=b, beta=beta, act=act, alpha=alpha, w16=self.wt16, stats=stats, w_frag=self.wfrag)
        if self.prof is not None:
            e1.record()
            self.prof.append((e0, e1))
        if self.ktimer is not None:
            self.ktimer.taken()

    def stats_ok(self, x, y):
        if K.PRECISION['value'] != 1:
            return False
        if self.kind == 'up':
            return K.conv_stats_ok(lib.CONV_DGRAD, self.geom, y, x, self.wd, bias=self.bias, w16=self.wd16)
        return K.conv_stats_ok(lib.CONV_FPROP, self.geom, x, y, self.wt, bias=self.bias, w16=self.wt16)

    def backward_data(self, dy, dx, beta=0, act=0, alpha=0.0, aux=None, skip=None, norm_bwd=None, defer=False):
        if self.kind == 'up':
            return K.conv(lib.CONV_FPROP, self.geom, dy, dx, self.wt, beta=beta, act=act, alpha=alpha, aux=aux, w16=self.wt16, dst_gap=skip,
                          norm_bwd=norm_bwd, defer=defer)
        return K.conv(lib.CONV_DGRAD, self.geom, dx, dy, self.wd, beta=beta, act=act, alpha=alpha, aux=aux, w16=self.wd16, dst_gap=skip,
                      norm_bwd=norm_bwd, defer=defer)

    def norm_bwd_ok(self, dy, dx, norm_bwd, skip=None):
        if K.PRECISION['value'] != 1:
            return False
        nb = dict(norm_bwd, ws=None)
        if self.kind == 'up':
            return K.conv_stats_ok(lib.CONV_FPROP, self.geom, dy, dx, self.wt, w16=self.wt16, dst_gap=skip, norm_bwd=nb)
        return K.conv_stats_ok(lib.CONV_DGRAD, self.geom, dx, dy, self.wd, w16=self.wd16, dst_gap=skip, norm_bwd=nb)

    def backward_weights(self, x, dy, feeds_instance_norm=False):
        target = self.dwfp if self.padded else (self.dwf if self.dwf is not None else self.dW)
        if dy.dtype == torch.bfloat16 and self.dbias is not None and not feeds_instance_norm:
            raise NotImplementedError('bias gradient from a bf16 output gradient: only for a convolution in front of an instance norm '
                                      '(feeds_instance_norm=True), whose bias gradient is identically zero')
        db = None if (feeds_instance_norm and dy.dtype == torch.bfloat16) else self.dbias
        if self.kind == 'up':
            K.conv(lib.CONV_WGRAD, self.geom, dy, x, target)
            if db is not None:
                K.colsum(dy, db)
        else:
            K.conv(lib.CONV_WGRAD, self.geom, x, dy, target, bias=db)

    def finish_weight_grad(self, sn_done=False):
        if self.padded:
            copy_view(self.dwfp[:, :self.cx0, :self.cy0], [self.dw_tmp])
            tgt = self.dwf if self.dwf is not None else self.dW
            K.axpby(1.0, self.dw_tmp.reshape(-1), 1.0, tgt.reshape(-1), tgt.reshape(-1))
            self.dwfp.zero_()
            if self.bias is not None:
                K.axpby(1.0, self.dbias[:self.cy0], 1.0, self.dbias_master, self.dbias_master)
                self.dbias.zero_()
        if self.dwf is None:
            return
        if self.sn_u_name:
# ... 130 lines not shown
```

video_prediction_amd/kernels.py:

```python
import ctypes

import torch

from . import debug as _debug
from . import lib
from .lib import (c_f32, c_i32, c_i64, c_vp, ptr)


def _nd(t):
    if t.stride(-1) != 1 and t.shape[-1] != 1:
        raise ValueError('channel stride must be 1')
    if t.dim() == 4:
        N, H, W, C = t.shape
        sn, sh, sw, _ = t.stride()
        return N, 1, H, W, C, sn, 0, sh, sw
    if t.dim() == 5:
        N, D, H, W, C = t.shape
        sn, sd, sh, sw, _ = t.stride()
        return N, D, H, W, C, sn, sd, sh, sw
    if t.dim() == 2:
        N, C = t.shape
        return N, 1, 1, 1, C, t.stride(0), 0, 0, 0
    raise ValueError('expected 2-D, 4-D or 5-D tensor')

# ... 209 lines not shown
    def run(cfg):
        out = torch.zeros(ext, device=like.device, dtype=like.dtype)
        sts = torch.zeros(max(nst, 1), device=like.device, dtype=torch.float64)
        nbs = torch.zeros(max(nnb, 1), device=like.device, dtype=torch.float64)
        if mode == lib.CONV_WGRAD:
            a.w = out.data_ptr()
        elif mode == lib.CONV_DGRAD:
            a.x = out.data_ptr()
        else:
            a.y = out.data_ptr()
        if nst:
            a.stats = sts.data_ptr()
        if nnb:
            a.nb_ws = nbs.data_ptr()
        a.tile, a.splitk = cfg
        a.ws, a.ws_bytes = None, 0
        if mode == lib.CONV_WGRAD or cfg[1] != 1:
            _conv_scratch(a, like.device)
        rc = fn(st, ctypes.byref(a))
        return rc, out, sts, nbs

    def differs(got, ref, tol):
        g, r = got.double(), ref.double()
        scale = float(r.abs().max())
        err = float((g - r).abs().max()) if g.numel() else 0.0
        if not (err <= tol * max(scale, 1e-30)):
            return 'max |diff| %.3g against max |ref| %.3g (tol %.1g)' % (err, scale, tol)
        return None

    bad = []
    try:
        rc, ref, ref_st, ref_nb = run((0, 0))
        if rc != 0:
            return []
        tol = 2e-2 if out_bf16 else (1e-2 if a.precision == 1 and mode == lib.CONV_WGRAD else 2e-4)
        for cfg in cfgs:
            rc, out, sts, nbs = run(cfg)
            why = 'rc %d' % rc if rc != 0 else (differs(out, ref, tol) or (nst and differs(sts, ref_st, 1e-3)) or (nnb and differs(nbs, ref_nb, 1e-3)))
            if why:
                bad.append((cfg, why))
    finally:
        a.x, a.y, a.w, a.stats, a.nb_ws, a.tile, a.splitk, a.ws, a.ws_bytes, a.beta = keep
    return bad


def _conv_scratch(a, device):
    need = lib.get().savp_conv_workspace_bytes(ctypes.byref(a))
    if need:
        ws = scratch(device, (need + 3) // 4)
        a.ws, a.ws_bytes = ws.data_ptr(), ws.numel() * 4


def conv(mode, geom, x, y, w, bias=None, beta=0, act=0, alpha=0.0, aux=None, splitk=0, tile=0, precision=None, w16=None, stats=None,
         dst_gap=None, norm_bwd=None, defer=False, w_frag=None, w_frag_il=None):
    lib.require_device(w, bias, aux)
    lib.require_stats(stats, (norm_bwd or {}).get('ws'))
    lib.require_device_any(x, y)
    a = _fill_conv_args(mode, geom, x, y, w, bias, beta, act, alpha, aux, splitk, tile, precision, w16, stats, dst_gap, norm_bwd, w_frag, w_frag_il)
    if AUTOTUNE['enabled'] and tile == 0 and splitk == 0 and not lib.get().savp_conv_special(ctypes.byref(a)):
        key = (mode, a.precision, a.N, a.D, a.H, a.W, a.Cx, a.Do, a.Ho, a.Wo, a.Cy, geom.k, geom.s, geom.p, a.act, a.beta,
               a.x_sw, a.y_sw, bias is not None, w16 is not None, a.src_bf16, a.out_bf16, stats is not None)
        if a.dst_gap:
            key = key + ((a.dst_gap_at, a.dst_gap),)
        if norm_bwd is not None:
            key = key + (('nb', a.nb_c0, a.nb_nc),)
        cfg = AUTOTUNE['cache'].get(key)
        if cfg is None:
            dst = x if mode == lib.CONV_DGRAD else y
            cfg = _tune(a, mode, dst, w)
            for bad_cfg, why in getattr(_tune, 'last_rejected', []):
                AUTOTUNE['rejected'].append((key, {'cfg': list(bad_cfg), 'why': why}))
            if AUTOTUNE['dist'] is not None:
                t = torch.tensor([int(cfg[0]), int(cfg[1])], dtype=torch.int32, device=dst.device)
                AUTOTUNE['dist'].broadcast(t, src=0)
                cfg = tuple(int(v) for v in t.tolist())
            AUTOTUNE['cache'][key] = cfg
            AUTOTUNE['log'].append((key, cfg))
        a.tile, a.splitk = cfg
        if INSITU is not None:
            if INSITU['mode'] == 'rank':
                if key in INSITU['targets'] and key not in INSITU['ranked']:
                    INSITU['ranked'][key] = _tune(a, mode, x if mode == lib.CONV_DGRAD else y, w, return_all=True)
                    a.tile, a.splitk = cfg
            elif INSITU['mode'] == 'all' or key in INSITU['targets']:
                if mode == lib.CONV_WGRAD or a.splitk != 1:
                    _conv_scratch(a, w.device)
                e0, e1 = torch.cuda.Event(enable_timing=True), torch.cuda.Event(enable_timing=True)
                e0.record()
                lib.check(lib.get().savp_conv(lib.stream(), ctypes.byref(a)), 'savp_conv')
                e1.record()
                INSITU['events'].append((key, e0, e1))
                return
    if mode == lib.CONV_WGRAD or a.splitk != 1:
        _conv_scratch(a, w.device)
    if CONV_CALL_LOG is not None:
        CONV_CALL_LOG.append((mode, a.N, a.D, a.H, a.W, a.Cx, a.Do, a.Ho, a.Wo, a.Cy, tuple(geom.k), tuple(geom.s), a.tile, a.splitk))
    if defer:
        return a
    rc = lib.get().savp_conv(lib.stream(), ctypes.byref(a))
    if rc:
        lib.check(rc, 'savp_conv(%s)' % describe_conv(a))


def describe_conv(a):
    return ('%s N=%d in=%dx%dx%dx%d out=%dx%dx%dx%d k=%dx%dx%d s=%dx%dx%d prec=%s x=%s%s y=%s%s tile=0x%x splitk=%d act=%d beta=%d bias=%d' %
            (('fprop', 'dgrad', 'wgrad')[a.mode], a.N, a.D, a.H, a.W, a.Cx, a.Do, a.Ho, a.Wo, a.Cy, a.kd, a.kh, a.kw, a.sd, a.sh, a.sw,
             'bf16' if a.precision == 1 else 'f32', 'bf16' if a.src_bf16 else 'f32', '/sw%d' % a.x_sw, 'bf16' if a.out_bf16 else 'f32',
             '/sw%d' % a.y_sw, a.tile, a.splitk, a.act, a.beta, 1 if a.bias else 0))


def conv_stats_ok(mode, geom, x, y, w, bias=None, w16=None, dst_gap=None, norm_bwd=None):
# ... 313 lines not shown
    a.cn, a.dc_new, a.dcn, a.dgn = _contig(cn), _contig(dc_new), _contig(dcn), _contig(dgn)
    a.ndh = len(dhs)
    _set_views(a.dh, dhs)
    lib.check(lib.get().savp_lnlstm_bwd(lib.stream(), ctypes.byref(a), 0), 'savp_lnlstm_bwd')


def lnlstm_state_bwd(gn, c_prev, dc_pre, dgn, dc_prev, forget_bias=1.0):
    a = _lnlstm_args(gn, c_prev, forget_bias)
    a.dc_pre, a.dgn, a.dc_prev = _contig(dc_pre), _contig(dgn), _contig(dc_prev)
    lib.check(lib.get().savp_lnlstm_bwd(lib.stream(), ctypes.byref(a), 1), 'savp_lnlstm_bwd')


def _lstm_args(gates, c_prev, g1, b1, g2, b2, stats, eps, forget_bias):
    a = lib.SavpLstmArgs()
    N = gates.shape[0]
    F = gates.shape[-1] // 4
    a.N, a.HW, a.F = N, _hw(gates), F
    a.eps, a.forget_bias = float(eps), float(forget_bias)
    if not gates.is_contiguous():
        raise ValueError('gates must be contiguous')
    a.gates = gates.data_ptr()
    a.gates_bf16 = int(gates.dtype == torch.bfloat16)
    if c_prev is not None:
        a.c_prev = view(c_prev)
    if g1 is None:
        a.no_norm = 1
        return a
    a.gamma1, a.beta1, a.gamma2, a.beta2 = g1.data_ptr(), b1.data_ptr(), g2.data_ptr(), b2.data_ptr()
    a.mean1, a.rstd1, a.mean2, a.rstd2 = [s.data_ptr() for s in stats]
    return a


LSTM_RED_FLOATS = 22


def lstm_ws_floats(N, HW, F):
    return N * F * HW


def _lstm_ws(a, gates, ws, ws_stats=None):
    if ws is not None:
        lib.require_device(ws)
        a.ws, a.ws_floats = ws.data_ptr(), ws.numel()
    if ws_stats is None:
        ws_stats = zero_arena(gates.device).take(a.N * a.F * LSTM_RED_FLOATS)
    a.ws_stats, a.ws_stats_clean = ws_stats.data_ptr(), 1


def lstm_stats_ws(device, N, F):
    ws = zero_arena(device).take(N * F * LSTM_RED_FLOATS)
    return ws, ws[:N * 4 * F * 4].view(torch.float64).view(N, 4 * F, 2)


def convlstm_gates_fwd(gates, c_prev, g1, b1, g2, b2, c_new, hs, stats, eps=1e-6, forget_bias=1.0, ws=None, stats1=None, defer=False):
    a = _lstm_args(gates, c_prev, g1, b1, g2, b2, stats, eps, forget_bias)
    a.c_new = c_new.data_ptr()
    if ws is not None or stats1 is not None:
        _lstm_ws(a, gates, ws, stats1)
        a.stats1_ready = int(stats1 is not None)
    a.nh = len(hs)
    _set_views(a.h, hs, any_dtype=True)
    a.h_bf16 = _bf16_mask(hs)
    if defer:
        return a
    lib.check(lib.get().savp_convlstm_gates_fwd(lib.stream(), ctypes.byref(a)), 'savp_convlstm_gates_fwd')


def convlstm_gates_bwd(gates, c_prev, g1, b1, g2, b2, stats, dhs, dc_new, dgates, dc_prev, dparams, eps=1e-6,
                       forget_bias=1.0, ws=None, dgates_raw=None, defer=False):
    a = _lstm_args(gates, c_prev, g1, b1, g2, b2, stats, eps, forget_bias)
    if dgates.dtype == torch.bfloat16:
        if dgates_raw is None or dgates_raw.dtype != torch.float32 or dgates_raw.numel() < dgates.numel():
            raise ValueError('bf16 dgates need an fp32 dgates_raw scratch of the same size')
        a.dgates_bf16 = 1
        a.dgates_raw = dgates_raw.data_ptr()
    if ws is not None:
        _lstm_ws(a, gates, ws)
    a.ndh = len(dhs)
    _set_views(a.dh, dhs)
    a.dc_new = dc_new.data_ptr() if dc_new is not None else None
    a.dgates = dgates.data_ptr()
    a.dc_prev = dc_prev.data_ptr() if dc_prev is not None else None
    acc = _Acc64(*(dparams if not a.no_norm else ()))
    if not a.no_norm:
        a.dgamma1, a.dbeta1, a.dgamma2, a.dbeta2 = [acc.addr(i) for i in range(4)]
    if defer:
        acc.finish(deferred=True)
        return a
    lib.check(lib.get().savp_convlstm_gates_bwd(lib.stream(), ctypes.byref(a)), 'savp_convlstm_gates_bwd')
    acc.finish()


def fused_ok():
    return INSITU is None and CONV_CALL_LOG is None


def convlstm_cell_fwd(conv_args, lstm_args):
    c = lib.SavpConvLstmCellArgs()
    c.conv, c.gates = conv_args, lstm_args
    lib.check(lib.get().savp_convlstm_cell_fwd(lib.stream(), ctypes.byref(c)), 'savp_convlstm_cell_fwd')


def convlstm_cell_bwd(conv_args, lstm_args):
    c = lib.SavpConvLstmCellArgs()
    c.conv, c.gates = conv_args, lstm_args
    lib.check(lib.get().savp_convlstm_cell_bwd(lib.stream(), ctypes.byref(c)), 'savp_convlstm_cell_bwd')


def conv_in_act_fwd(conv_args, norm_args):
    c = lib.SavpConvNormArgs()
    c.conv, c.norm = conv_args, norm_args
    lib.check(lib.get().savp_conv_in_act_fwd(lib.stream(), ctypes.byref(c)), 'savp_conv_in_act_fwd')


def conv_in_act_bwd(conv_args, norm_args):
    c = lib.SavpConvNormArgs()
    c.conv, c.norm = conv_args, norm_args
    lib.check(lib.get().savp_conv_in_act_bwd(lib.stream(), ctypes.byref(c)), 'savp_conv_in_act_bwd')


def _L():
    return lib.get()

# ... 349 lines not shown
    acc = _Acc64(loss_out)
    lib.check(_L().savp_lp_loss(lib.stream(), rows, row_len, pred.stride(0), target.stride(0), int(p2), _p(pred), _p(target),
                                float(weight), acc.addr(0), _p(dpred)), 'savp_lp_loss')
    acc.finish()


def tv_loss(flows, n_channels, s1, s2, weight, loss_out=None, dflows=None):
    lib.require_device_any(flows)
    assert flows.dtype == torch.float32 and flows.dim() == 4 and flows.stride(3) == 1 and flows.stride(1) == flows.shape[2] * flows.stride(2)
    if dflows is not None:
        assert dflows.stride() == flows.stride() and dflows.dtype == torch.float32
    lib.require_stats(loss_out)
    n, H, W, _ = flows.shape
    lib.check(_L().savp_tv_loss(lib.stream(), _p(flows), n, H, W, int(n_channels), flows.stride(0), flows.stride(2), float(s1), float(s2),
                                float(weight), _p(loss_out), _p(dflows)), 'savp_tv_loss')


def lsgan_loss(logits, label, weight, loss_out=None, dlogits=None, beta=0):
    acc = _Acc64(loss_out)
    lib.check(_L().savp_lsgan_loss(lib.stream(), logits.numel(), _p(logits), float(label), float(weight), acc.addr(0), _p(dlogits),
                                   int(beta)), 'savp_lsgan_loss')
    acc.finish()


def cosine_distance(f0, f1, weight, loss_out=None, df0=None, beta=0, eps=1e-10):
    assert f0.is_contiguous() and f1.is_contiguous()
    C = f0.shape[-1]
    acc = _Acc64(loss_out)
    lib.check(_L().savp_cosine_distance(lib.stream(), f0.numel() // C, C, _p(f0), _p(f1), float(weight), float(eps), acc.addr(0),
                                        _p(df0), int(beta)), 'savp_cosine_distance')
    acc.finish()


def pack_weights(src, wt=None, wd=None, scale=None, wt16=None, wd16=None):
    Cx, Cy = src.shape[-2], src.shape[-1]
    T = src.numel() // (Cx * Cy)
    lib.check(_L().savp_pack_weights(lib.stream(), _p(src), T, Cx, Cy, _p(scale), _p(wt), _p(wd), _p(wt16), _p(wd16)),
              'savp_pack_weights')


def pack_weights_batch(entries):
    for lo in range(0, len(entries), 32):
        part = entries[lo:lo + 32]
        arr = (lib.SavpPackItem * len(part))()
        for i, e in enumerate(part):
            src = e['src']
            lib.require_device(src)
            it = arr[i]
            it.src, it.scale = _p(src), _p(e.get('scale'))
            it.wt, it.wd, it.wt_bf16, it.wd_bf16 = _p(e.get('wt')), _p(e.get('wd')), _p(e.get('wt16')), _p(e.get('wd16'))
            it.Cx, it.Cy = src.shape[-2], src.shape[-1]
            it.T = src.numel() // (it.Cx * it.Cy)
        lib.check(_L().savp_pack_weights_batch(lib.stream(), len(part), arr), 'savp_pack_weights_batch')


def gate_weights_elems(taps, Cx, Cy):
    return int(lib.get().savp_gate_weights_bytes(int(taps), int(Cx), int(Cy))) // 2


def pack_gate_weights(src, out, interleave=False):
    lib.require_device(src)
    Cx, Cy = src.shape[-2], src.shape[-1]
    taps = src.numel() // (Cx * Cy)
    if out.dtype != torch.bfloat16 or out.numel() != gate_weights_elems(taps, Cx, Cy):
        raise ValueError('gate weight pack: expected %d bf16 elements' % gate_weights_elems(taps, Cx, Cy))
    lib.check(_L().savp_pack_gate_weights(lib.stream(), _p(src), taps, Cx, Cy, _p(out), int(bool(interleave))), 'savp_pack_gate_weights')


def fold_pool(inp, out, k, adjoint=False):
    C = (out.numel() if adjoint else inp.numel()) // (k * k)
    lib.check(_L().savp_fold_pool(lib.stream(), _p(inp), _p(out), k, C, int(adjoint)), 'savp_fold_pool')


def fold_bilinear(inp, out, k, Cin, F, adjoint=False):
    lib.check(_L().savp_fold_bilinear(lib.stream(), _p(inp), _p(out), k, Cin, F, int(adjoint)), 'savp_fold_bilinear')


def sn_ws_size(K, C):
    return 8 + 2 * C + 2 * K + 2 * (C + 2)


def sn_fwd(W, u, ws, u_new=None):
    C = W.shape[-1]
    K = W.numel() // C
    lib.check(_L().savp_sn_fwd(lib.stream(), _p(W), K, C, _p(u), _p(ws), _p(u_new)), 'savp_sn_fwd')


def _sn_items(entries, bwd):
    arr = (lib.SavpSnItem * len(entries))()
    for i, e in enumerate(entries):
        W = e['W']
        C = W.shape[-1]
        arr[i].W, arr[i].K, arr[i].C = W.data_ptr(), W.numel() // C, C
        arr[i].u, arr[i].ws = e['u'].data_ptr(), e['ws'].data_ptr()
        arr[i].u_new = e['u_new'].data_ptr() if e.get('u_new') is not None else None
        if bwd:
            arr[i].G, arr[i].dW, arr[i].beta = e['G'].data_ptr(), e['dW'].data_ptr(), int(e.get('beta', 0))
    return arr


def sn_fwd_batch(entries):
    for lo in range(0, len(entries), 16):
        part = entries[lo:lo + 16]
        arr = _sn_items(part, False)
        lib.check(_L().savp_sn_fwd_batch(lib.stream(), len(part), arr), 'savp_sn_fwd_batch')

# ... 300 lines not shown
```

video_prediction_amd/lib.py:

```python
import ctypes
import os

import torch

from . import debug as _debug

_HERE = os.path.dirname(os.path.abspath(__file__))
LIB_PATH = os.environ.get('SAVP_LIB') or os.path.join(_HERE, 'libsavp_hip.so')

c_i32, c_i64, c_f32, c_vp = ctypes.c_int32, ctypes.c_int64, ctypes.c_float, ctypes.c_void_p

CONV_FPROP, CONV_DGRAD, CONV_WGRAD = 0, 1, 2
ACT_NONE, ACT_LRELU, ACT_SIGMOID, ACT_DLRELU_FROM_OUT = 0, 1, 2, 3


class SavpConvArgs(ctypes.Structure):
    _fields_ = [
        ('mode', c_i32),
        ('N', c_i32), ('D', c_i32), ('H', c_i32), ('W', c_i32), ('Cx', c_i32),
        ('Do', c_i32), ('Ho', c_i32), ('Wo', c_i32), ('Cy', c_i32),
        ('kd', c_i32), ('kh', c_i32), ('kw', c_i32),
        ('sd', c_i32), ('sh', c_i32), ('sw', c_i32),
        ('pd', c_i32), ('ph', c_i32), ('pw', c_i32),
        ('beta', c_i32), ('act', c_i32), ('alpha', c_f32), ('splitk', c_i32), ('tile', c_i32), ('precision', c_i32),
        ('x', c_vp), ('x_sn', c_i64), ('x_sd', c_i64), ('x_sh', c_i64), ('x_sw', c_i64),
        ('y', c_vp), ('y_sn', c_i64), ('y_sd', c_i64), ('y_sh', c_i64), ('y_sw', c_i64),
        ('w', c_vp), ('bias', c_vp), ('aux', c_vp), ('w_bf16', c_vp),
        ('src_bf16', c_i32), ('out_bf16', c_i32), ('stats', c_vp),
        ('ws', c_vp), ('ws_bytes', c_i64),
        ('dst_gap_at', c_i32), ('dst_gap', c_i32),
        ('nb_x', c_vp), ('nb_x_sn', c_i64), ('nb_x_sp', c_i64), ('nb_mean', c_vp), ('nb_rstd', c_vp), ('nb_gamma', c_vp), ('nb_beta', c_vp),
        ('nb_ws', c_vp), ('nb_c0', c_i32), ('nb_nc', c_i32), ('nb_act', c_i32), ('nb_alpha', c_f32),
        ('w_frag', c_vp), ('w_frag_il', c_vp),
    ]


_lib = None


def get():
    global _lib
    if _lib is None:
        if not os.path.exists(LIB_PATH):
            raise RuntimeError(
                'libsavp_hip.so not found at %s -- build it first (python -c "import __graft_entry__ as g; g.build()"). '
                'video_prediction_amd has no non-HIP fallback.' % LIB_PATH)
        lib = ctypes.CDLL(LIB_PATH)
        lib.savp_version.restype = ctypes.c_char_p
        _declare(lib)
        _lib = lib
        _forward_env_options(lib)
    if _debug.POISON['lds']:
        return _LdsPoisonProxy(_lib)
    return _lib


def get_raw():
    lib = get()
    return lib._lib if isinstance(lib, _LdsPoisonProxy) else lib


class _LdsPoisonProxy(object):

    def __init__(self, lib):
        self._lib = lib

    def __getattr__(self, name):
        fn = getattr(self._lib, name)
        at = getattr(fn, 'argtypes', None)
        if not name.startswith('savp_') or name.startswith(('savp_debug_', 'savp_prof_')) or not at or at[0] is not c_vp or \
                name in ('savp_allreduce_bucket',):
            return fn
        poison = self._lib.savp_debug_poison_lds

        def call(st, *args):
            poison(st, _debug.NAN_WORD, None)
            _debug.COUNTS['lds'] += 1
            return fn(st, *args)
        return call


OPTION_NAMES = ('conv_ring', 's2dgrad', 'thin', 'wgp_cfg', 'wgp_split', 'inorm_min_hw', 'colsum_2stage', 'dense_legacy', 'cdna_legacy',
                'lstm_fused', 'ring_dma', 'lstm_q', 'ring_wwarm', 'wgp_dma', 'ring_early', 'gate_kernel', 'gate_alt', 'gate_cell', 'gate_wwarm', 'splitk_reduced')


def set_option(name, value):
    check(get().savp_set_option(name.encode(), int(value)), 'savp_set_option(%s)' % name)


def get_option(name):
    v = c_i32()
    check(get().savp_get_option(name.encode(), ctypes.byref(v)), 'savp_get_option(%s)' % name)
    return v.value


def _forward_env_options(lib):
    for name in OPTION_NAMES:
        v = os.environ.get('SAVP_' + name.upper())
        if v is not None:
            check(lib.savp_set_option(name.encode(), int(v)), 'savp_set_option(%s)' % name)


EXPORTS = {}


def _sig(lib, name, argtypes, restype=c_i32):
    try:
        fn = getattr(lib, name)
    except AttributeError:
        if os.environ.get('SAVP_LIB'):
            return None
        raise
    fn.argtypes = argtypes
    fn.restype = restype
    EXPORTS[name] = fn
    return fn


def _declare(lib):
    P = ctypes.POINTER
    _sig(lib, 'savp_conv', [c_vp, P(SavpConvArgs)])
    _sig(lib, 'savp_conv_workspace_bytes', [P(SavpConvArgs)], restype=c_i64)
    _sig(lib, 'savp_conv_special', [P(SavpConvArgs)])
    _sig(lib, 'savp_gate_weights_bytes', [c_i32, c_i32, c_i32], restype=c_i64)
    _sig(lib, 'savp_conv_stats_ok', [P(SavpConvArgs)])
    _sig(lib, 'savp_set_option', [ctypes.c_char_p, c_i32])
    _sig(lib, 'savp_get_option', [ctypes.c_char_p, P(c_i32)])
    _sig(lib, 'savp_allreduce_bucket', [c_vp, c_vp, c_vp, c_i64])
    _sig(lib, 'savp_tiled_z_weff', [c_vp, c_vp, c_i32, c_i32, c_i32, c_i32, c_i32, c_i32, c_i32, c_i32, c_vp])
    _sig(lib, 'savp_tiled_z_grad', [c_vp, c_vp, c_i32, c_i64, c_i32, c_i32, c_i32, c_vp, c_i32, c_vp, c_i32, c_vp, c_i64])
    _sig(lib, 'savp_tiled_z_workspace_bytes', [c_i64, c_i32], restype=c_i64)
    _sig(lib, 'savp_eval_fold_ws_floats', [c_i32, c_i32, c_i32, c_i32], restype=c_i64)
    for name, argtypes in _EXTRA_SIGS.items():
        _sig(lib, name, argtypes)


# ... 54 lines not shown
        if t.dtype != torch.float64 or (t.data_ptr() & 7):
            raise RuntimeError('statistics workspaces are float64 (kernels.stats_ws), got %s' % t.dtype)


def require_device_any(*tensors):
    for t in tensors:
        if t is None:
            continue
        if not t.is_cuda:
            raise RuntimeError('video_prediction_amd kernels need device tensors (got %s); there is no CPU path' % t.device)
        if t.dtype not in (torch.float32, torch.bfloat16):
            raise RuntimeError('expected float32 or bfloat16, got %s' % t.dtype)


class SavpView(ctypes.Structure):
    _fields_ = [('p', c_vp), ('sn', c_i64), ('sp', c_i64)]


class SavpInormArgs(ctypes.Structure):
    _fields_ = [
        ('N', c_i32), ('HW', c_i32), ('C', c_i32), ('act', c_i32), ('alpha', c_f32), ('eps', c_f32),
        ('x', SavpView), ('gamma', c_vp), ('beta', c_vp),
        ('nout', c_i32), ('out', SavpView * 4), ('mean', c_vp), ('rstd', c_vp),
        ('ndy', c_i32), ('dy', SavpView * 4), ('dx', SavpView), ('dx_beta', c_i32),
        ('dgamma', c_vp), ('dbeta', c_vp), ('ws', c_vp), ('ws_clean', c_i32),
        ('out_c0', c_i32 * 4), ('out_nc', c_i32 * 4), ('dy_c0', c_i32 * 4), ('dy_nc', c_i32 * 4), ('out_bf16', c_i32),
        ('stats_ready', c_i32), ('stats_shift', c_vp), ('dx_bf16', c_i32),
    ]


class SavpGnormArgs(ctypes.Structure):
    _fields_ = [('norm', SavpInormArgs), ('G', c_i32), ('ws_group', c_vp), ('dsum', c_vp)]


class SavpLnLstmArgs(ctypes.Structure):
    _fields_ = [
        ('N', c_i32), ('HW', c_i32), ('F', c_i32), ('forget_bias', c_f32), ('gn', c_vp), ('c_prev', SavpView), ('c_pre', c_vp),
        ('cn', c_vp), ('nh', c_i32), ('h', SavpView * 4), ('h_bf16', c_i32), ('ndh', c_i32), ('dh', SavpView * 4),
        ('dc_new', c_vp), ('dcn', c_vp), ('dgn', c_vp), ('dc_pre', c_vp), ('dc_prev', c_vp),
    ]


class SavpLstmArgs(ctypes.Structure):
    _fields_ = [
        ('N', c_i32), ('HW', c_i32), ('F', c_i32), ('eps', c_f32), ('forget_bias', c_f32),
        ('gates', c_vp), ('c_prev', SavpView),
        ('gamma1', c_vp), ('beta1', c_vp), ('gamma2', c_vp), ('beta2', c_vp),
        ('c_new', c_vp), ('nh', c_i32), ('h', SavpView * 4),
        ('mean1', c_vp), ('rstd1', c_vp), ('mean2', c_vp), ('rstd2', c_vp),
        ('ndh', c_i32), ('dh', SavpView * 4), ('dc_new', c_vp), ('dgates', c_vp), ('dc_prev', c_vp),
        ('dgamma1', c_vp), ('dbeta1', c_vp), ('dgamma2', c_vp), ('dbeta2', c_vp),
        ('ws', c_vp), ('ws_floats', ctypes.c_int64), ('ws_stats', c_vp), ('ws_stats_clean', c_i32),
        ('gates_bf16', c_i32), ('stats1_ready', c_i32), ('h_bf16', c_i32), ('dgates_bf16', c_i32), ('dgates_raw', c_vp), ('no_norm', c_i32),
    ]


class SavpConvLstmCellArgs(ctypes.Structure):
    _fields_ = [('conv', SavpConvArgs), ('gates', SavpLstmArgs)]


class SavpConvNormArgs(ctypes.Structure):
    _fields_ = [('conv', SavpConvArgs), ('norm', SavpInormArgs)]


register('savp_convlstm_cell_fwd', [c_vp, ctypes.POINTER(SavpConvLstmCellArgs)])
register('savp_convlstm_cell_bwd', [c_vp, ctypes.POINTER(SavpConvLstmCellArgs)])
register('savp_conv_in_act_fwd', [c_vp, ctypes.POINTER(SavpConvNormArgs)])
register('savp_conv_in_act_bwd', [c_vp, ctypes.POINTER(SavpConvNormArgs)])
register('savp_instnorm_act_fwd', [c_vp, ctypes.POINTER(SavpInormArgs)])
register('savp_instnorm_act_bwd', [c_vp, ctypes.POINTER(SavpInormArgs)])
register('savp_groupnorm_act_fwd', [c_vp, ctypes.POINTER(SavpGnormArgs)])
register('savp_groupnorm_act_bwd', [c_vp, ctypes.POINTER(SavpGnormArgs)])
register('savp_lnlstm_fwd', [c_vp, ctypes.POINTER(SavpLnLstmArgs), c_i32])
register('savp_lnlstm_bwd', [c_vp, ctypes.POINTER(SavpLnLstmArgs), c_i32])
register('savp_convlstm_gates_fwd', [c_vp, ctypes.POINTER(SavpLstmArgs)])
register('savp_convlstm_gates_bwd', [c_vp, ctypes.POINTER(SavpLstmArgs)])


class SavpCdnaArgs(ctypes.Structure):
    _fields_ = [
        ('N', c_i32), ('H', c_i32), ('W', c_i32), ('C', c_i32), ('K', c_i32), ('kh', c_i32), ('kw', c_i32),
        ('img', SavpView), ('kern', c_vp), ('out', SavpView), ('dout', SavpView),
        ('dimg', SavpView), ('dimg_beta', c_i32), ('dkern', c_vp),
    ]


class SavpCompositeArgs(ctypes.Structure):
    _fields_ = [
        ('N', c_i32), ('HW', c_i32), ('M', c_i32), ('C', c_i32),
        ('logits', c_vp), ('logits_stride', c_i32), ('timgs', SavpView), ('gen', SavpView), ('masks', c_vp),
        ('dgen', SavpView), ('dlogits', c_vp), ('drow', SavpView), ('timgs_offset', c_i32), ('row_channels', c_i32),
        ('nnext', c_i32), ('next', SavpView * 2), ('gt_mask', c_vp), ('gt_img', SavpView),
    ]


_PV = ctypes.POINTER(SavpView)
register('savp_tile_channels', [c_vp, c_vp, c_i64, c_i32, c_i32, c_f32, SavpView, c_i32])
register('savp_tile_channels_bf16', [c_vp, c_vp, c_i64, c_i32, c_i32, c_f32, SavpView])
register('savp_colsum', [c_vp, SavpView, c_i64, c_i32, c_i32, c_f32, c_vp, c_i32, c_vp, c_i64])
register('savp_select', [c_vp, c_i32, c_i32, c_i32, c_vp, SavpView, SavpView, c_i32, _PV])
register('savp_select_bwd', [c_vp, c_i32, c_i32, c_i32, c_vp, c_i32, _PV, SavpView])
register('savp_gather_clips', [c_vp, c_vp, c_vp, c_vp, c_i32, c_i32, c_i64, c_i64, c_i32])
register('savp_sigmoid_bwd', [c_vp, SavpView, SavpView, c_vp, c_i64, c_i32, c_i32])
register('savp_axpby', [c_vp, c_i64, c_f32, c_vp, c_f32, c_vp, c_vp])
register('savp_fill_view', [c_vp, SavpView, c_i64, c_i32, c_i32, c_f32])
register('savp_u8_frames_to_f32', [c_vp, c_vp, c_vp, c_i32, c_i32, c_i64])
# ... 131 lines not shown
```

video_prediction_amd/models/savp_cell.py:

```python
import os

import torch

from .. import kernels as K
from .. import lib
from ..engine import ConcatConv, ConvLayer, same_pad_before, copy_view, add_views, prep_layers
from ..variables import NORM_SCOPES, layer_specs, num_masks

CONV_STATS = os.environ.get('SAVP_CONV_STATS', '1') == '1'
FUSED_ENTRIES = os.environ.get('SAVP_FUSED_ENTRIES', '1') == '1'
NORM_BWD_STATS = os.environ.get('SAVP_NORM_BWD_STATS', '1') == '1'
EPS_IN = 1e-6


def check_norm_layers(hp):
    if hp.conv_rnn not in ('lstm', 'gru'):
        raise NotImplementedError("conv_rnn=%r" % hp.conv_rnn)
    if hp.norm_layer not in ('instance', 'layer'):
        raise NotImplementedError("norm_layer=%r: the HIP path covers 'instance' and 'layer'" % hp.norm_layer)
    if hp.conv_rnn_norm_layer not in ('instance', 'layer', 'none'):
        raise NotImplementedError("conv_rnn_norm_layer=%r: the HIP path covers 'instance', 'layer' and 'none'" % hp.conv_rnn_norm_layer)
    layer = 'layer' in (hp.norm_layer, hp.conv_rnn_norm_layer)
    if layer and not hp.use_tile_concat:
        raise NotImplementedError("use_tile_concat=False with norm_layer=%r, conv_rnn_norm_layer=%r: the untiled latent is only "
# ... 168 lines not shown
                L['conv'] = ConvLayer(store, s + 'conv_pool2d/kernel', s + 'conv_pool2d/bias', 'pool', (k, k), (2, 2),
                                      (same_pad_before(k + 1, 2, h_), same_pad_before(k + 1, 2, w_)),
                                      cx_pad=ceil8(cx + zc))
                h_, w_ = h_ // 2, w_ // 2
            else:
                j = i - self.ne
                skip = 0 if j == 0 else self.layers[self.ne - j - 1]['f']
                cx = prev_f + skip
                L['in'] = Act((T1, N, h_, w_, cx + zc), dev, grad=g, dtype=a16 if (cx + zc) % 8 == 0 else torch.float32)
                L['zoff_in'] = cx
                L['skip_off'] = prev_f
                h_, w_ = h_ * 2, w_ * 2
                L['conv'] = ConvLayer(store, s + 'upsample_conv2d/kernel', s + 'upsample_conv2d/bias', 'up', (3, 3), (2, 2),
                                      (same_pad_before(6, 2, h_), same_pad_before(6, 2, w_)))
            L['hw'] = (h_, w_)
            pre16 = f % 8 == 0 and (i < self.ne or L['in'].v.dtype == torch.bfloat16 or not self.act16)
            L['pre'] = Act((T1, N, h_, w_, f), dev, grad=g, grad_dtype=a16 if pre16 else torch.float32)
            L['norm'] = self._norm(s, f, bias=L['conv'].bias_name)
            if use_rnn and self.abl_rnn:
                r = prefix + 'conv_h%d/' % i
                L['a'] = Act((T1, N, h_, w_, ceil4(f + zr)), dev, grad=g, dtype=a16 if ceil4(f + zr) % 8 == 0 else torch.float32)
                L['pre2'] = Act((T1, N, h_, w_, f), dev, grad=g, grad_dtype=a16 if f % 8 == 0 else torch.float32)
                L['rconv'] = ConvLayer(store, r + 'conv2d/kernel', r + 'conv2d/bias', 'conv', (5, 5), (1, 1), (2, 2), cx_pad=ceil4(f + zr))
                L['n2'] = self._norm(r, f, bias=r + 'conv2d/bias')
            elif use_rnn and hp.conv_rnn == 'gru':
                r = prefix + 'gru_h%d/conv2dgru_cell/' % i
                L['cin1'] = f + zr + f
                L['a'] = Act((T1, N, h_, w_, f + zr + 2 * f), dev, grad=g)
                L['gates'] = Act((T1, N, h_, w_, 2 * f), dev, grad=g)
                L['cand'] = Act((T1, N, h_, w_, f), dev, grad=g)
                L['u'] = torch.empty(T1, N, h_, w_, f, device=dev)
                L['du'] = torch.empty(N, h_, w_, f, device=dev) if g else None
                L['dh_tmp'] = torch.empty(N, h_, w_, f, device=dev) if g else None
                L['rconv'] = ConvLayer(store, r + 'gates/kernel', None, 'conv', (5, 5), (1, 1), (2, 2))
                L['cconv'] = ConvLayer(store, r + 'candidate/kernel', None, 'conv', (5, 5), (1, 1), (2, 2))
                L['n1'] = Norm(store, r + 'gates/reset_update/', T1, N, 2 * f, dev)
                L['n2'] = Norm(store, r + 'candidate/state/', T1, N, f, dev)
            elif use_rnn:
                r = prefix + 'lstm_h%d/basic_conv2dlstm_cell/' % i
                L['fused'] = (K.PRECISION['value'] == 1 and os.environ.get('SAVP_FUSED_CELL', '1') == '1' and not self.cell_plain and
                              not self.cell_ln and
                              h_ % 8 == 0 and w_ % 8 == 0 and 16 <= f <= 256 and (f & (f - 1)) == 0 and (f + zr + f) % 8 == 0)
                a_dt = torch.bfloat16 if (L['fused'] and os.environ.get('SAVP_BF16_ACT', '1') == '1') else torch.float32
                L['a'] = Act((T1, N, h_, w_, f + zr + f), dev, grad=g, dtype=a_dt)
                dg_dt = torch.bfloat16 if (L['fused'] and g and os.environ.get('SAVP_BF16_DGATES', '1') == '1') else torch.float32
                L['gates'] = Act((T1, N, h_, w_, 4 * f), dev, grad=g, dtype=torch.bfloat16 if L['fused'] else torch.float32,
                                 grad_dtype=dg_dt)
                L['dg_raw'] = torch.empty(N, h_, w_, 4 * f, device=dev) if dg_dt == torch.bfloat16 else None
                L['c'] = Act((T1, N, h_, w_, f), dev, grad=False)
                L['dc'] = [torch.empty(N, h_, w_, f, device=dev), torch.empty(N, h_, w_, f, device=dev)] if g else None
                L['rconv'] = ConvLayer(store, r + 'kernel', (r + 'bias') if self.cell_plain else None, 'conv', (5, 5), (1, 1), (2, 2))
                if not self.cell_plain and not self.cell_ln:
                    L['rconv'].enable_gate_pack(cell=bool(L['fused']) and h_ * w_ <= 256)
                if self.cell_ln:
                    L['gn4'] = ConcatNorm([Norm(store, r + nm + '/', T1, N, f, dev, groups=1) for nm in ('input', 'transform', 'forget', 'output')],
                                          T1, N, dev)
                    L['nS'] = Norm(store, r + 'state/', T1, N, f, dev, groups=1)
                    L['gnv'] = Act((T1, N, h_, w_, 4 * f), dev, grad=g)
                    L['cpre'] = Act((T1, N, h_, w_, f), dev, grad=g)
                    L['dcn'] = torch.empty(N, h_, w_, f, device=dev) if g else None
                elif not self.cell_plain:
                    L['n1'] = Norm(store, r + 'input_transform_forget_output/', T1, N, 4 * f, dev)
                    L['n2'] = Norm(store, r + 'state/', T1, N, f, dev)
                if self.out_norm:
                    L['h_raw'] = Act((T1, N, h_, w_, f), dev, grad=g)
                    L['onorm'] = self._norm(prefix + 'lstm_h%d/' % i, f, hp.conv_rnn_norm_layer)
                L['zless'] = bool(g and zr and not cw and L['fused'] and os.environ.get('SAVP_ZLESS_DGRAD', '1') == '1' and
                                  K.tiled_z_ok(h_, w_, 4 * f, zr, L['rconv'].geom))
                if L['zless']:
                    L['weff'] = torch.empty(25, 4 * f, K.tiled_z_pad(zr), device=dev)
            else:
                L['out'] = None
            self.layers.append(L)
            prev_f = f
        nl = len(self.layers)
        last = self.layers[-1]
        ngf = hp.ngf
        self.M = M = num_masks(hp)
        self.L = hp.last_frames
        self.nk = nk = hp.last_frames * hp.num_transformed_images
        self.nti = hp.num_transformed_images
        kh, kw = hp.kernel_size
        self.kh, self.kw = kh, kw

        self.tf = hp.transformation
        self.h_last = Act((T1, N, H, W, last['f']), dev, grad=g, dtype=a16 if last['f'] % 8 == 0 else torch.float32)
        tf_convs = []
        if self.tf == 'cdna':
            sh_, sw_ = H // 2 ** self.ne, W // 2 ** self.ne
            small_f = self.layers[self.ne - 1]['f']
            self.hsmall = Act((T1, N, sh_, sw_, small_f), dev, grad=g)
            self.cdna_dense = ConvLayer(store, prefix + 'cdna_kernels/dense/kernel', prefix + 'cdna_kernels/dense/bias', 'conv',
                                        (1, 1), (1, 1), (0, 0))
            self.cdna_raw = Act((T1, N, kh * kw * nk), dev, grad=g)
            self.cdna_kern = Act((T1, N, kh * kw, nk), dev, grad=False)
            self.cdna_dkern = torch.zeros(N, kh * kw, nk, device=dev, dtype=torch.float64) if g else None
            tf_convs = [self.cdna_dense]
        else:
            hs, os_, cy = (('h%d_flow/' % nl, 'flows/', 2 * nk) if self.tf == 'flow' else
                           ('h%d_dna_kernel/' % nl, 'dna_kernels/', kh * kw * nk))
            s = prefix + hs
            self.tf_conv = ConvLayer(store, s + 'conv2d/kernel', s + 'conv2d/bias', 'conv', (3, 3), (1, 1), (1, 1))
            self.tf_pre = Act((T1, N, H, W, ngf), dev, grad=g)
            self.tf_norm = self._norm(s, ngf, bias=s + 'conv2d/bias')
            self.tf_h = Act((T1, N, H, W, ngf), dev, grad=g)
            self.tf_out = ConvLayer(store, prefix + os_ + 'conv2d/kernel', prefix + os_ + 'conv2d/bias', 'conv', (3, 3), (1, 1),
# ... 162 lines not shown
        f = L['f']
        return [buf.v[t][..., off:off + f] for buf, off in L['routes']]

    def _out_grads(self, L, t):
        f = L['f']
        return [buf.g[t][..., off:off + f] for buf, off in L['routes']]

    def forward(self, images, zs=None, gt_mask=None, collect_masks=False, actions=None, states=None):
        T1, N, C = self.T1, self.N, self.C
        nz = self.nz
        self.images = images
        self.gt_mask = gt_mask
        cw, na = self.cw, self.na
        if cw:
            if (na and actions is None) or (self.ns and states is None):
                raise ValueError('this generator was built for inputs with actions / states (cond=%r)' % ((na, self.ns),))
            if self.ns:
                K.state_pred_fwd(actions[:T1].contiguous() if na else None, states[:T1].contiguous(), gt_mask, self.spW, self.spb, self.sa,
                                 self.gen_states.v)
                self.saz[..., :cw].copy_(self.sa)
            else:
                self.saz[..., :na].copy_(actions[:T1])
        if nz:
            self.zs.v.copy_(zs)
            if self.use_rnn_z and self.abl_rnn:
                self.fc_z.forward(self.zs.v.reshape(T1 * N, 1, 1, nz), self.fcz_pre.v)
                torch.tanh(self.fcz_pre.v.reshape(T1, N, nz), out=self.rnn_z.v)
            elif self.use_rnn_z and self.hp.rnn == 'gru':
                self.zA[..., :nz].copy_(self.zs.v)
                K.gru_seq_fwd(self.zA, self.zA2, self.zg.W, self.zg.bias, self.zc.W, self.zc.bias, self.rnn_z.v, self.z_ru, self.z_cand, nz,
                              h0=self.z_h0 if self.learn_init else None)
            elif self.use_rnn_z:
                K.lstm_z_fwd(self.zs.v, self.zW, self.zb, self.rnn_z.v, self.z_gates, self.z_cs,
                             init=(self.z_c0, self.z_h0) if self.learn_init else None)
            else:
                self.rnn_z.v.copy_(self.zs.v)
            if cw:
                self.saz[..., cw:].copy_(self.rnn_z.v)
        if self.zw:
            zw = self.zw
            zflat = (self.saz if cw else self.rnn_z.v).reshape(T1 * N, zw)
            for L in self.layers:
                b = L['in']
                if L['zc']:
                    K.tile_channels(zflat, b.flat(b.v)[..., L['zoff_in']:L['zoff_in'] + zw])
                if L['rnn'] and L['zr']:
                    a = L['a']
                    K.tile_channels(zflat, a.flat(a.v)[..., L['f']:L['f'] + zw])
        if self.learn_init:
            for L in self.layers:
                if L['rnn']:
                    f, hoff = L['f'], L['f'] + L['zr']
                    L['a'].v[0][..., hoff:hoff + f].copy_(L['h0v'])
                    if not self.gru:
                        L['c0'].copy_(L['c0v'])
        in0, maskin = self.layers[0]['in'], self.maskin
        if self._ones is None:
            self._ones = torch.ones(max(N, T1), dtype=torch.int32, device=self.dev)
        NH = N * self.H
        mflat = maskin.v.reshape(T1, NH, self.W, -1)

        def frame_all_steps(k, t0=0):
            return images[k].reshape(1, NH, self.W, C).expand(T1 - t0, NH, self.W, C)
        first_dsts = [in0.v.reshape(T1, NH, self.W, -1)[..., C:2 * C]]
        for bg, off in zip(self.bgs, self.o_bg):
            if bg == ('fixed', 0):
                first_dsts.append(mflat[..., off:off + C])
        K.select(self._ones, frame_all_steps(0), None, first_dsts)
        cf = self.hp.context_frames
        for bg, off in zip(self.bgs, self.o_bg):
            if bg[0] == 'fixed' and bg[1] != 0:
                K.select(self._ones, frame_all_steps(bg[1]), None, [mflat[..., off:off + C]])
            elif bg[0] == 'last_context':
                n = min(cf, T1)
                copy_view(images[:n].reshape(n, NH, self.W, C), [mflat[:n][..., off:off + C]])
                if T1 > n:
                    K.select(self._ones, frame_all_steps(cf - 1, n), None, [mflat[n:][..., off:off + C]])
        fuse_select = os.environ.get('SAVP_FUSE_SELECT', '1') == '1'

        def image_slots(t):
            return [in0.v[t][..., 0:C]] + ([maskin.v[t][..., self.o_prev:self.o_prev + C]] if self.o_prev is not None else [])
        for t in range(T1):
            if t == 0 or not fuse_select:
                prev_gen = self.gen.v[t - 1] if t > 0 else None
                K.select(gt_mask[t], images[t], prev_gen, image_slots(t))
            for L in self.layers:
                f = L['f']
                ck = ('cstats', K.PRECISION['value'])
                if ck not in L:
                    L[ck] = (CONV_STATS and f <= 256 and (f & (f - 1)) == 0 and L['conv'].stats_ok(L['in'].v[t], L['pre'].v[t]))
                st = K.stats_ws(self.dev, N, f) if L[ck] else None
                nrm = L['norm']
                if L['rnn'] and self.abl_rnn:
                    a = L['a']
                    self._conv_in_act(L['conv'], L['in'].v[t], L['pre'].v[t], st, nrm, [a.v[t][..., 0:f]], t)
                    self._conv_norm(('abl', L['idx']), L['rconv'], a.v[t], L['pre2'].v[t], L['n2'], self._out_views(L, t), t)
                elif L['rnn'] and self.gru:
                    L['conv'].forward(L['in'].v[t], L['pre'].v[t], stats=st)
                    a = L['a']
                    hs, rs_, cin1 = f + L['zr'], f + L['zr'] + f, L['cin1']
                    norm_fwd(nrm, L['pre'].v[t], [a.v[t][..., 0:f]], nrm.mean[t], nrm.rstd[t],
                             act='relu', eps=EPS_IN, stats=st, stats_shift=L['conv'].bias if st is not None else None)
                    n1, n2 = L['n1'], L['n2']
                    hprev = a.v[t][..., hs:hs + f]
                    L['rconv'].forward(a.v[t][..., 0:cin1], L['gates'].v[t], use_bias=False)
                    K.convgru_gates_fwd(L['gates'].v[t], hprev, n1.gamma, n1.beta, n1.mean[t], n1.rstd[t], L['u'][t],
                                        a.v[t][..., rs_:rs_ + f], eps=EPS_IN)
                    L['cconv'].forward(a.v[t], L['cand'].v[t], use_bias=False)
                    outs = self._out_views(L, t)
                    if t + 1 < T1:
                        outs.append(a.v[t + 1][..., hs:hs + f])
                    K.convgru_out_fwd(L['cand'].v[t], hprev, n2.gamma, n2.beta, n2.mean[t], n2.rstd[t], L['u'][t], outs, eps=EPS_IN)
                elif L['rnn'] and self.cell_plain:
                    a = L['a']
                    self._conv_in_act(L['conv'], L['in'].v[t], L['pre'].v[t], st, nrm, [a.v[t][..., 0:f]], t)
                    L['rconv'].forward(a.v[t], L['gates'].v[t])
                    nxt_h = [a.v[t + 1][..., f + L['zr']:f + L['zr'] + f]] if t + 1 < T1 else []
                    hdst = ([L['h_raw'].v[t]] if self.out_norm else self._out_views(L, t)) + nxt_h
                    K.convlstm_gates_fwd(L['gates'].v[t], L['c'].v[t - 1] if t > 0 else L.get('c0'), None, None, None, None, L['c'].v[t], hdst, None)
                    if self.out_norm:
                        on = L['onorm']
                        norm_fwd(on, L['h_raw'].v[t], self._out_views(L, t), on.mean[t], on.rstd[t], act='none', eps=EPS_IN)
                elif L['rnn'] and self.cell_ln:
                    a, g4, nS = L['a'], L['gn4'], L['nS']
                    self._conv_in_act(L['conv'], L['in'].v[t], L['pre'].v[t], st, nrm, [a.v[t][..., 0:f]], t)
                    L['rconv'].forward(a.v[t], L['gates'].v[t], use_bias=False)
                    K.groupnorm_act_fwd(L['gates'].v[t], g4.gamma, g4.beta, [L['gnv'].v[t]], g4.mean[t], g4.rstd[t], groups=4, act='none')
                    K.lnlstm_state_fwd(L['gnv'].v[t], L['c'].v[t - 1] if t > 0 else L.get('c0'), L['cpre'].v[t])
                    K.groupnorm_act_fwd(L['cpre'].v[t], nS.gamma, nS.beta, [L['c'].v[t]], nS.mean[t], nS.rstd[t], groups=1, act='none')
                    outs = self._out_views(L, t)
                    if t + 1 < T1:
                        outs.append(a.v[t + 1][..., f + L['zr']:f + L['zr'] + f])
                    K.lnlstm_out_fwd(L['gnv'].v[t], L['c'].v[t], outs)
                elif L['rnn']:
                    a = L['a']
                    self._conv_in_act(L['conv'], L['in'].v[t], L['pre'].v[t], st, nrm, [a.v[t][..., 0:f]], t)
                    stats1 = s1 = None
                    if L['fused']:
                        stats1, s1 = K.lstm_stats_ws(self.dev, N, f)
                    cp = L.get('cell_prof')
                    if cp is not None:
                        ce0, ce1 = torch.cuda.Event(enable_timing=True), torch.cuda.Event(enable_timing=True)
                        ce0.record()
                    outs = self._out_views(L, t)
                    if t + 1 < T1:
                        outs.append(a.v[t + 1][..., f + L['zr']:f + L['zr'] + f])
                    n1, n2 = L['n1'], L['n2']
                    gk = L.get('gate_ktimer')
                    gargs = (L['gates'].v[t], L['c'].v[t - 1] if t > 0 else L.get('c0'), n1.gamma, n1.beta, n2.gamma, n2.beta, L['c'].v[t], outs,
                             [n1.mean[t], n1.rstd[t], n2.mean[t], n2.rstd[t]])
                    ca = (L['rconv'].forward(a.v[t], L['gates'].v[t], use_bias=False, stats=s1, defer=True)
                          if (FUSED_ENTRIES and cp is None and gk is None and K.fused_ok()) else None)
                    if ca is not None:
                        ck = L.get('cell_ktimer')
                        if ck is not None:
                            ck.arm()
                        K.convlstm_cell_fwd(ca, K.convlstm_gates_fwd(*gargs, eps=EPS_IN, ws=self._lstm_ws(L), stats1=stats1, defer=True))
                        if ck is not None:
                            ck.taken()
                    else:
                        L['rconv'].forward(a.v[t], L['gates'].v[t], use_bias=False, stats=s1)
                        if gk is not None:
                            gk.arm()
                        K.convlstm_gates_fwd(*gargs, eps=EPS_IN, ws=self._lstm_ws(L), stats1=stats1)
                        if gk is not None:
                            gk.taken()
                    if cp is not None:
                        ce1.record()
                        cp.append((ce0, ce1))
                else:
                    self._conv_in_act(L['conv'], L['in'].v[t], L['pre'].v[t], st, nrm, self._out_views(L, t), t)
            tslot = maskin.v[t][..., self.o_cdna:self.o_cdna + self.nk * C]
            ngf = self.hp.ngf
            if self.merge_heads:
                hn = self.heads_norm
                outs = ([self.scratch_h.v[t]] if self.scratch else []) + [maskin.v[t][..., 0:ngf]] + \
                       ([self.tf_h.v[t]] if self.tf != 'cdna' else [])
                self._conv_norm('heads', self.heads_conv, self.h_last.v[t], self.heads_pre.v[t], hn, outs, t,
                                out_ranges=[(i * ngf, ngf) for i in range(self.nheads)])
            srcs = [in0.v[s][..., 0:C] for s in last_frame_steps(t, self.L)] if self.L > 1 else None
            if self.tf == 'cdna':
                self.cdna_dense.forward(self.hsmall.v[t].reshape(N, -1), self.cdna_raw.v[t])
                K.cdna_kernels_fwd(self.cdna_raw.v[t], self.cdna_kern.v[t], self.kh, self.kw, self.nk)
                if srcs is None:
                    K.cdna_apply_fwd(in0.v[t][..., 0:C], self.cdna_kern.v[t], tslot, self.kh, self.kw, self.nk)
                else:
                    K.cdna_apply_multi_fwd(srcs, self.cdna_kern.v[t], tslot, self.kh, self.kw, self.nti)
            else:
                if not self.merge_heads:
                    self._conv_norm('tf', self.tf_conv, self.h_last.v[t], self.tf_pre.v[t], self.tf_norm, [self.tf_h.v[t]], t)
                self.tf_out.forward(self.tf_h.v[t], self.tf_raw.v[t])
                if self.tf == 'flow' and srcs is None:
                    K.image_warp_fwd(in0.v[t][..., 0:C], self.tf_raw.v[t], tslot, self.nk)
                elif self.tf == 'flow':
                    K.image_warp_multi_fwd(srcs, self.tf_raw.v[t], tslot, self.nti)
                elif srcs is None:
                    K.dna_apply_fwd(in0.v[t][..., 0:C], self.tf_raw.v[t], self.dna_kern[t], tslot, self.kh, self.kw, self.nk)
                else:
                    K.dna_apply_multi_fwd(srcs, self.tf_raw.v[t], self.dna_kern[t], tslot, self.kh, self.kw, self.nti)
            if self.scratch and not self.merge_heads:
                self._conv_norm('scratch', self.scratch_conv, self.h_last.v[t], self.scratch_pre.v[t], self.scratch_norm,
                                [self.scratch_h.v[t]], t)
            if self.scratch:
                self.scratch_out.forward(self.scratch_h.v[t], maskin.v[t][..., self.o_scratch:self.o_scratch + self.Cs],
                                         act=lib.ACT_SIGMOID)
            if not self.merge_heads:
                self._conv_norm('masks', self.masks_conv, self.h_last.v[t], self.masks_pre.v[t], self.masks_norm,
                                [maskin.v[t][..., 0:self.hp.ngf]], t)
            self.masks_out.forward(maskin.v[t][..., 0:self.mask_cin], self.logits.v[t])
            nxt = (gt_mask[t + 1], images[t + 1], image_slots(t + 1)) if (fuse_select and t + 1 < T1) else None
            K.composite_fwd(self.logits.v[t], maskin.v[t][..., self.hp.ngf:self.hp.ngf + self.M * C], self.gen.v[t],
                            self.masks[t] if collect_masks else None, M=self.M, next_inputs=nxt)
        return self.gen.v

    def _norm(self, scope, c, kind=None, bias=None):
        kind = kind or self.hp.norm_layer
        return Norm(self.store, scope + NORM_SCOPES[kind], self.T1, self.N, c, self.dev, groups=1 if kind == 'layer' else None, bias=bias)
# ... 148 lines not shown
                                      L['cand'].g[t], L['du'], L['dh_tmp'], n2.dgamma, n2.dbeta, eps=EPS_IN)
                    L['cconv'].backward_data(L['cand'].g[t], a.g[t], beta=0)
                    add_views([L['dh_tmp']], a.g[t][..., hs:hs + f])
                    K.convgru_gates_bwd(L['gates'].v[t], hprev, n1.gamma, n1.beta, n1.mean[t], n1.rstd[t], L['du'],
                                        a.g[t][..., rs_:rs_ + f], L['gates'].g[t], a.g[t][..., hs:hs + f], n1.dgamma, n1.dbeta,
                                        eps=EPS_IN)
                    L['rconv'].backward_data(L['gates'].g[t], a.g[t][..., 0:cin1], beta=1)
                    norm_bwd(nrm, L['pre'].v[t], a.v[t][..., 0:f], nrm.mean[t], nrm.rstd[t],
                                       [a.g[t][..., 0:f]], L['pre'].g[t], nrm.dgamma, nrm.dbeta, act='relu', eps=EPS_IN)
                elif L['rnn'] and self.cell_plain:
                    a = L['a']
                    if self.out_norm:
                        on = L['onorm']
                        norm_bwd(on, L['h_raw'].v[t], self._out_views(L, t)[0], on.mean[t], on.rstd[t], dys,
                                           L['h_raw'].g[t], on.dgamma, on.dbeta, act='none', eps=EPS_IN)
                        dys = [L['h_raw'].g[t]]
                    if t + 1 < T1:
                        dys.append(a.g[t + 1][..., f + L['zr']:f + L['zr'] + f])
                    dc_new = L['dc'][(t + 1) & 1] if t + 1 < T1 else None
                    dc_prev = L['dc'][t & 1] if (t > 0 or self.learn_init) else None
                    K.convlstm_gates_bwd(L['gates'].v[t], L['c'].v[t - 1] if t > 0 else L.get('c0'), None, None, None, None, None, dys, dc_new,
                                         L['gates'].g[t], dc_prev, None)
                    L['rconv'].backward_data(L['gates'].g[t], a.g[t], beta=0)
                    self._in_act_conv_bwd(L, t, a.v[t][..., 0:f], [a.g[t][..., 0:f]], None)
                    continue
                elif L['rnn']:
                    a = L['a']
                    if t + 1 < T1:
                        dys.append(a.g[t + 1][..., f + L['zr']:f + L['zr'] + f])
                    dc_new = L['dc'][(t + 1) & 1] if t + 1 < T1 else None
                    dc_prev = L['dc'][t & 1] if (t > 0 or self.learn_init) else None
                    if self.cell_ln:
                        g4, nS, gnv, cpre = L['gn4'], L['nS'], L['gnv'], L['cpre']
                        c_prev = L['c'].v[t - 1] if t > 0 else L.get('c0')
                        K.lnlstm_out_bwd(gnv.v[t], L['c'].v[t], dys, dc_new, L['dcn'], gnv.g[t])
                        K.groupnorm_act_bwd(cpre.v[t], nS.gamma, nS.beta, nS.mean[t], nS.rstd[t], [L['dcn']], cpre.g[t], nS.dgamma, nS.dbeta,
                                            groups=1, act='none')
                        K.lnlstm_state_bwd(gnv.v[t], c_prev, cpre.g[t], gnv.g[t], dc_prev)
                        K.groupnorm_act_bwd(L['gates'].v[t], g4.gamma, g4.beta, g4.mean[t], g4.rstd[t], [gnv.g[t]], L['gates'].g[t],
                                            g4.dgamma, g4.dbeta, groups=4, act='none')
                        L['rconv'].backward_data(L['gates'].g[t], a.g[t], beta=0)
                        self._in_act_conv_bwd(L, t, a.v[t][..., 0:f], [a.g[t][..., 0:f]], None)
                        continue
                    n1, n2 = L['n1'], L['n2']
                    bargs = (L['gates'].v[t], L['c'].v[t - 1] if t > 0 else L.get('c0'), n1.gamma, n1.beta, n2.gamma, n2.beta,
                             [n1.mean[t], n1.rstd[t], n2.mean[t], n2.rstd[t]], dys, dc_new, L['gates'].g[t], dc_prev,
                             [n1.dgamma, n1.dbeta, n2.dgamma, n2.dbeta])
                    skip = (f, L['zr']) if L['zless'] else None
                    nb = self._norm_bwd('nbstats', L, L['rconv'], L['gates'].g[t], a.g[t], nrm, L['pre'].v[t], skip)
                    if nb is not None:
                        nb['mean'], nb['rstd'] = nrm.mean[t], nrm.rstd[t]
                    if FUSED_ENTRIES and K.fused_ok():
                        K.convlstm_cell_bwd(L['rconv'].backward_data(L['gates'].g[t], a.g[t], beta=0, skip=skip, norm_bwd=nb, defer=True),
                                            K.convlstm_gates_bwd(*bargs, eps=EPS_IN, ws=self._lstm_ws(L), dgates_raw=L.get('dg_raw'), defer=True))
                    else:
                        K.convlstm_gates_bwd(*bargs, eps=EPS_IN, ws=self._lstm_ws(L), dgates_raw=L.get('dg_raw'))
                        L['rconv'].backward_data(L['gates'].g[t], a.g[t], beta=0, skip=skip, norm_bwd=nb)
                    self._in_act_conv_bwd(L, t, a.v[t][..., 0:f], [a.g[t][..., 0:f]], nb['ws'] if nb is not None else None)
                    continue
                else:
                    y0 = self._out_views(L, t)[0]
                    st_ = nb_last['ws'] if (L is self.layers[-1] and nb_last is not None and len(dys) == 1) else None
                    self._in_act_conv_bwd(L, t, y0, dys, st_)
                    continue
                L['conv'].backward_data(L['pre'].g[t], L['in'].g[t], beta=0)
            if t > 0:
                K.select_bwd(self.gt_mask[t], [in0.g[t][..., 0:C], self.dimg_cdna if self.L == 1 else self.dimg_acc[t]] +
                             ([maskin.g[t][..., self.o_prev:self.o_prev + C]] if self.o_prev is not None else []), self.gen.g[t - 1])
        if self.learn_init:
            for L in self.layers:
                if L['rnn']:
                    f, hoff = L['f'], L['f'] + L['zr']
                    L['h0g'].add_(L['a'].g[0][..., hoff:hoff + f].float().sum(0))
                    if not self.gru:
                        L['c0g'].add_(L['dc'][0].sum(0))
        for L in self.layers:
            b, pre = L['in'], L['pre']
            L['conv'].backward_weights(b.flat(b.v), pre.flat(pre.g), feeds_instance_norm=True)
            if L['rnn'] and self.abl_rnn:
                a, p2 = L['a'], L['pre2']
                L['rconv'].backward_weights(a.flat(a.v), p2.flat(p2.g), feeds_instance_norm=True)
            elif L['rnn'] and self.gru:
                a, gt, cd = L['a'], L['gates'], L['cand']
                L['rconv'].backward_weights(a.flat(a.v)[..., 0:L['cin1']], gt.flat(gt.g))
                L['cconv'].backward_weights(a.flat(a.v), cd.flat(cd.g))
            elif L['rnn']:
                a, gt = L['a'], L['gates']
                L['rconv'].backward_weights(a.flat(a.v), gt.flat(gt.g))
                if 'gn4' in L:
                    L['gn4'].finish()
        hl = self.h_last
        if self.tf == 'cdna':
            hs = self.hsmall
            self.cdna_dense.backward_weights(hs.v.reshape(T1 * N, -1), self.cdna_raw.g.reshape(T1 * N, -1))
        else:
            if not self.merge_heads:
                self.tf_conv.backward_weights(hl.flat(hl.v), hl.flat(self.tf_pre.g), feeds_instance_norm=True)
            self.tf_out.backward_weights(hl.flat(self.tf_h.v), hl.flat(self.tf_raw.g))
        if self.merge_heads:
            self.heads_conv.backward_weights(hl.flat(hl.v), hl.flat(self.heads_pre.g), feeds_instance_norm=True)
            self.heads_norm.finish()
        else:
            if self.scratch:
                self.scratch_conv.backward_weights(hl.flat(hl.v), hl.flat(self.scratch_pre.g), feeds_instance_norm=True)
            self.masks_conv.backward_weights(hl.flat(hl.v), hl.flat(self.masks_pre.g), feeds_instance_norm=True)
        if self.scratch:
            self.scratch_out.backward_weights(hl.flat(self.scratch_h.v), self.dscratch_pre.reshape(T1 * N, self.H, self.W, self.Cs))
        self.masks_out.backward_weights(hl.flat(maskin.v)[..., 0:self.mask_cin], hl.flat(self.logits.g))
        for c in self.convs:
            c.finish_weight_grad()
        if self.ns and state_grad:
            K.state_pred_bwd(self.gt_mask, self.spW, self.sa, self.gen_states.g, self.dspW, self.dspb)
        if not nz:
            return None
        drz = self.rnn_z.g
        drz.zero_()
        cw = self.cw
        for L in self.layers:
            b = L['in']
            if L['zc']:
                K.colsum(b.flat(b.g)[..., L['zoff_in'] + cw:L['zoff_in'] + cw + nz], drz, per_row=True)
            if L['rnn'] and L['zr'] and L.get('zless'):
                gt = L['gates']
                K.tiled_z_weff(L['rconv'].W, L['rconv'].geom, L['f'], nz, L['weff'])
                K.tiled_z_grad(gt.flat(gt.g), L['weff'], drz.reshape(T1 * N, nz), beta=1)
            elif L['rnn'] and L['zr']:
                a = L['a']
# ... 25 lines not shown
```

Baseline: 10440.

## Store ConvLSTM gates and cell state in slab-major 4-channel layout

Adds an optional slab-major layout for the bf16 gate tensor and the fp32 cell state. Each pixel's four gates for a 4-channel group sit contiguously, so the fused LSTM forward and backward kernels read one 32-byte record instead of four strided loads, and cell state is read and written as contiguous float4s. The gate conv epilogue writes directly in this layout, and the Python side permutes the initial cell state and its gradient to match. It is enabled by default for small spatial layers that pass the new checks; other conv paths reject slab outputs, which risks falling back or erroring in untested configurations.

New measurement: 10470, median of 6. No clear change (+0.3%).

```diff
diff --git a/include/savp_hip.h b/include/savp_hip.h
--- a/include/savp_hip.h
+++ b/include/savp_hip.h
@@ -59,6 +59,7 @@
     int32_t nb_c0, nb_nc, nb_act; float nb_alpha;
     const void* w_frag;
     const void* w_frag_il;
+    int32_t y_slab;
 } SavpConvArgs;
 
 int savp_conv(void* stream, const SavpConvArgs* args);
@@ -146,6 +147,7 @@
     int32_t dgates_bf16;
     float* dgates_raw;
     int32_t no_norm;
+    int32_t slab;
 } SavpLstmArgs;
 int savp_convlstm_gates_fwd(void* stream, const SavpLstmArgs* a);
 int savp_convlstm_gates_bwd(void* stream, const SavpLstmArgs* a);
diff --git a/video_prediction_amd/csrc/common.hip b/video_prediction_amd/csrc/common.hip
--- a/video_prediction_amd/csrc/common.hip
+++ b/video_prediction_amd/csrc/common.hip
@@ -35,6 +35,7 @@
 static struct { const char* name; int value; } g_opts[OPT_COUNT] = {
     {"conv_ring", 0}, {"s2dgrad", 1}, {"thin", 1}, {"wgp_cfg", 0}, {"wgp_split", 0}, {"inorm_min_hw", 64}, {"colsum_2stage", 1},
     {"dense_legacy", 0}, {"cdna_legacy", 0}, {"lstm_fused", 1}, {"ring_dma", 1}, {"lstm_q", 0}, {"ring_wwarm", 1}, {"wgp_dma", 1}, {"ring_early", 1}, {"gate_kernel", 1}, {"gate_alt", 0}, {"gate_cell", 1}, {"gate_wwarm", 1}, {"splitk_reduced", 0},
+    {"gate_slab", 1},
 };
 int savp_opt(int id) { return g_opts[id].value; }
 void savp_opt_count(int id) { ++g_opts[id].value; }
diff --git a/video_prediction_amd/csrc/conv_gate.hip b/video_prediction_amd/csrc/conv_gate.hip
--- a/video_prediction_amd/csrc/conv_gate.hip
+++ b/video_prediction_amd/csrc/conv_gate.hip
@@ -14,6 +14,7 @@
     const void* zero16;
     int N, Cy, mtiles, ntiles;
     int wwarm;
+    int slab;
     int F; float eps, forget_bias;
     const float* c_prev; long long cp_sn, cp_sp;
     const float *g1, *b1, *g2, *b2;
@@ -342,11 +343,13 @@
         auto erow = [&](int i, int m) { return pix0 + i * 32 + g + 8 * m; };
         float cp[NE];
         if (p.c_prev) {
-            const float* __restrict__ cpb = p.c_prev + (long long)nn * p.cp_sn + cch;
+            const float* __restrict__ cpb = p.slab ? p.c_prev + ((long long)nn * (F >> 2) + (cch >> 2)) * (HWI * 4) + (cch & 3)
+                                                   : p.c_prev + (long long)nn * p.cp_sn + cch;
+            const int cps = p.slab ? 4 : (int)p.cp_sp;
 #pragma unroll
             for (int i = 0; i < TMFc; ++i)
 #pragma unroll
-                for (int m = 0; m < 4; ++m) cp[i * 4 + m] = cpb[(erow(i, m) % HWI) * (int)p.cp_sp];
+                for (int m = 0; m < 4; ++m) cp[i * 4 + m] = cpb[(erow(i, m) % HWI) * cps];
         } else {
 #pragma unroll
             for (int e = 0; e < NE; ++e) cp[e] = 0.f;
@@ -448,11 +451,12 @@
                 const float ee = __expf(-2.f * fabsf(cn[e]));
                 hv[e] = copysignf((1.f - ee) * __builtin_amdgcn_rcpf(1.f + ee), cn[e]) * so[e];
             }
-            float* __restrict__ cb = p.c_new + (long long)n * HWI * F + cch;
+            float* __restrict__ cb = p.slab ? p.c_new + ((long long)n * (F >> 2) + (cch >> 2)) * (HWI * 4) + (cch & 3) : p.c_new + (long long)n * HWI * F + cch;
+            const int cns = p.slab ? 4 : F;
 #pragma unroll
             for (int i = 0; i < TMFc; ++i)
 #pragma unroll
-                for (int m = 0; m < 4; ++m) cb[(erow(i, m) % HWI) * F] = cn[i * 4 + m];
+                for (int m = 0; m < 4; ++m) cb[(erow(i, m) % HWI) * cns] = cn[i * 4 + m];
 #pragma unroll
             for (int k = 0; k < 4; ++k) {
                 if (k >= p.nh) break;
@@ -472,13 +476,24 @@
                 }
             }
         }
-        for (int idx = tid; idx < G::PIX * 4; idx += 256) {
-            const int pix = idx >> 2, gg = idx & 3;
-            const int imp = pix / HWI, px = pix - imp * HWI;
-            const int np = img0 + imp;
-            if (np >= p.N) continue;
-            const uint4 w = *reinterpret_cast<const uint4*>(T16 + pix * 32 + gg * 8);
-            *reinterpret_cast<uint4*>(p.y + ((long long)np * HWI + px) * (long long)p.Cy + gg * F + nt * 8) = w;
+        if (p.slab) {
+            for (int idx = tid; idx < G::PIX * 8; idx += 256) {
+                const int gg = idx & 3, rest = idx >> 2, pix = rest % G::PIX, sl = rest / G::PIX;
+                const int imp = pix / HWI, px = pix - imp * HWI;
+                const int np = img0 + imp;
+                if (np >= p.N) continue;
+                const uint2 w = *reinterpret_cast<const uint2*>(T16 + pix * 32 + gg * 8 + sl * 4);
+                *reinterpret_cast<uint2*>(p.y + (((long long)np * (F >> 2) + nt * 2 + sl) * HWI + px) * 16 + gg * 4) = w;
+            }
+        } else {
+            for (int idx = tid; idx < G::PIX * 4; idx += 256) {
+                const int pix = idx >> 2, gg = idx & 3;
+                const int imp = pix / HWI, px = pix - imp * HWI;
+                const int np = img0 + imp;
+                if (np >= p.N) continue;
+                const uint4 w = *reinterpret_cast<const uint4*>(T16 + pix * 32 + gg * 8);
+                *reinterpret_cast<uint4*>(p.y + ((long long)np * HWI + px) * (long long)p.Cy + gg * F + nt * 8) = w;
+            }
         }
         GT(7);
         return;
@@ -529,7 +544,22 @@
     }
     __syncthreads();
     GT(6);
-    {
+    if (p.slab) {
+        const int F = p.Cy >> 2;
+        const int ngw = NC >= F ? NC / F : 1;
+        for (int idx = tid; idx < G::PIX * (NC / 4); idx += 256) {
+            const int gl = idx % ngw, rest = idx / ngw;
+            const int pix = rest % G::PIX, sl = rest / G::PIX;
+            const int im = pix / (G::TR * G::TC), rr = pix - im * (G::TR * G::TC);
+            const int n = img0 + im;
+            if (n >= p.N) continue;
+            const int lc = gl * F + sl * 4;
+            const int col = n0 + lc, g = col / F, ch = col - g * F;
+            const int px = (ty0 + rr / G::TC) * S + tx0 + rr % G::TC;
+            const uint2 v = *reinterpret_cast<const uint2*>(T + pix * G::TP + (lc >> 1));
+            *reinterpret_cast<uint2*>(p.y + (((long long)n * (F >> 2) + (ch >> 2)) * (S * S) + px) * 16 + g * 4) = v;
+        }
+    } else {
         constexpr int CH = NC / 8;
         for (int idx = tid; idx < G::PIX * CH; idx += 256) {
             const int pix = idx / CH, c8 = idx - pix * CH;
@@ -657,6 +687,7 @@
     GateP p;
     p.x = (const unsigned short*)a->x; p.wfrag = (const uint4*)a->w_frag; p.y = (unsigned short*)a->y; p.stats = (double*)a->stats;
     p.zero16 = zero_of[dev_ord]; p.N = a->N; p.Cy = a->Cy; p.wwarm = savp_opt(OPT_GATE_WWARM);
+    p.slab = a->y_slab ? 1 : 0;
     hipError_t err = hipErrorInvalidValue;
     const int alt = savp_opt(OPT_GATE_ALT);
     bool done = false;
@@ -664,6 +695,8 @@
     if (!done && a->H == S_ && a->Cx == C_ && (want ? (ALT_ & want) != 0 : ALT_ == 0)) {                 \
         using G = GateCfg<S_, C_, TM_, TN_, NWN_>;                                                       \
         p.mtiles = G::NI == 1 ? a->N * G::TPI : (a->N + G::NI - 1) / G::NI; p.ntiles = a->Cy / G::NC;    \
+        const int F_ = a->Cy / 4;                                                                        \
+        if (p.slab && G::NC % F_ != 0 && F_ % G::NC != 0) { *rc = SAVP_EINVAL; return true; }           \
         err = launch_gate<S_, C_, TM_, TN_, NWN_>(p, st);                                                \
         done = true;                                                                                     \
     }
@@ -693,6 +726,8 @@
         !g->gamma2 || !g->beta2 || !g->c_new || !g->mean1 || !g->rstd1 || !g->mean2 || !g->rstd2 || (g->F & 7))
         return false;
     if (g->c_prev.sp * (long long)g->HW >= (1ll << 31)) return false;
+    if ((a->y_slab != 0) != (g->slab != 0)) { *rc = SAVP_EINVAL; return true; }
+    if (g->slab && g->c_prev.p && (g->c_prev.sn != (long long)g->HW * g->F || g->c_prev.sp != g->F)) { *rc = SAVP_EINVAL; return true; }
     for (int i = 0; i < g->nh; ++i)
         if (g->h[i].sp * (long long)g->HW >= (1ll << 31)) return false;
     static const void* zero_of[64] = {nullptr};
@@ -702,6 +737,7 @@
     GateP p;
     p.x = (const unsigned short*)a->x; p.wfrag = (const uint4*)a->w_frag_il; p.y = (unsigned short*)a->y; p.stats = nullptr;
     p.zero16 = zero_of[dev_ord]; p.N = a->N; p.Cy = a->Cy; p.wwarm = savp_opt(OPT_GATE_WWARM);
+    p.slab = a->y_slab ? 1 : 0;
     p.F = g->F; p.eps = g->eps; p.forget_bias = g->forget_bias;
     p.c_prev = (const float*)g->c_prev.p; p.cp_sn = g->c_prev.sn; p.cp_sp = g->c_prev.sp;
     p.g1 = g->gamma1; p.b1 = g->beta1; p.g2 = g->gamma2; p.b2 = g->beta2;
diff --git a/video_prediction_amd/csrc/conv_igemm.hip b/video_prediction_amd/csrc/conv_igemm.hip
--- a/video_prediction_amd/csrc/conv_igemm.hip
+++ b/video_prediction_amd/csrc/conv_igemm.hip
@@ -776,6 +776,7 @@
 
 extern "C" int savp_conv_special(const SavpConvArgs* a) {
     if (a && conv_gate_applies(a)) return 1;
+    if (a && a->y_slab) return 0;
     if (!a || ((a->tile >> 8) & 3) != 0) return 0;
     return (conv_thin_applies(a) || conv_s2dgrad_applies(a) || conv_gate_applies(a)) ? 1 : 0;
 }
@@ -837,11 +838,11 @@
     ablate_init();
     const bool xs4 = (a->x_sn % 4 == 0) && (a->x_sd % 4 == 0) && (a->x_sh % 4 == 0) && (a->x_sw % 4 == 0) && aligned16(a->x);
     const bool ys4 = (a->y_sn % 4 == 0) && (a->y_sd % 4 == 0) && (a->y_sh % 4 == 0) && (a->y_sw % 4 == 0) && aligned16(a->y);
-    if (algo == 0 && !gapped && !a->nb_ws) {
+    if (algo == 0 && !gapped && !a->nb_ws && !a->y_slab) {
         int rc = SAVP_OK;
         if (conv_thin_try(a, st, &rc)) return rc;
     }
-    if (algo == 0 && !gapped && !a->nb_ws && a->mode == SAVP_CONV_DGRAD) {
+    if (algo == 0 && !gapped && !a->nb_ws && !a->y_slab && a->mode == SAVP_CONV_DGRAD) {
         int rc = SAVP_OK;
         if (conv_s2dgrad_try(a, st, &rc)) return rc;
     }
@@ -849,6 +850,7 @@
         int rc = SAVP_OK;
         if (conv_gate_try(a, st, &rc)) return rc;
     }
+    if (a->y_slab) return SAVP_EINVAL;
     if (a->mode == SAVP_CONV_FPROP || a->mode == SAVP_CONV_DGRAD) {
         const bool dg = a->mode == SAVP_CONV_DGRAD;
         p.out = (float*)(dg ? a->x : a->y);
diff --git a/video_prediction_amd/csrc/fused_ops.hip b/video_prediction_amd/csrc/fused_ops.hip
--- a/video_prediction_amd/csrc/fused_ops.hip
+++ b/video_prediction_amd/csrc/fused_ops.hip
@@ -9,6 +9,7 @@
     const SavpConvArgs& c = a->conv;
     const SavpLstmArgs& g = a->gates;
     if (c.y != g.gates || (c.out_bf16 != 0) != (g.gates_bf16 != 0)) return SAVP_EINVAL;
+    if ((c.y_slab != 0) != (g.slab != 0)) return SAVP_EINVAL;
     if (c.Cy != 4 * g.F || c.N != g.N || (long long)c.Do * c.Ho * c.Wo != g.HW) return SAVP_EINVAL;
     if ((c.stats != nullptr) != (g.stats1_ready != 0)) return SAVP_EINVAL;
     if (c.stats && (void*)c.stats != g.ws_stats) return SAVP_EINVAL;
diff --git a/video_prediction_amd/csrc/norm_lstm.hip b/video_prediction_amd/csrc/norm_lstm.hip
--- a/video_prediction_amd/csrc/norm_lstm.hip
+++ b/video_prediction_amd/csrc/norm_lstm.hip
@@ -460,6 +460,7 @@
     float* draw;
     int dgates16;
     float* dc_prev;
+    int slab;
     double *dg1, *db1, *dg2, *db2;
 };
 
@@ -1073,14 +1074,22 @@
     __device__ __forceinline__ void get(float* o) const { o[0] = v.x; o[1] = v.y; o[2] = v.z; o[3] = v.w; }
 };
 
+__device__ __forceinline__ long long lstm_slab_row(int n, int F, int c0, int HW) { return ((long long)n * (F >> 2) + (c0 >> 2)) * HW; }
+__device__ __forceinline__ void load_gate_record(GateQuad<true> (&gq)[4], const float* gates, long long rec) {
+    const uint4* r = reinterpret_cast<const uint4*>(reinterpret_cast<const unsigned short*>(gates) + rec * 16);
+    const uint4 a = r[0], b = r[1];
+    gq[0].u = make_uint2(a.x, a.y); gq[1].u = make_uint2(a.z, a.w); gq[2].u = make_uint2(b.x, b.y); gq[3].u = make_uint2(b.z, b.w);
+}
+
 __device__ __forceinline__ void lstm_block_owner(int nslab, int xcd_map, int& n, int& slab) {
     const int b = blockIdx.x;
     if (xcd_map) { const int r = b >> 3; slab = r % nslab; n = (b & 7) + 8 * (r / nslab); }
     else { n = b / nslab; slab = b % nslab; }
 }
 
-template <int Q, int PPT, bool G16>
+template <int Q, int PPT, bool G16, bool SLAB>
 __global__ __launch_bounds__(NT) void lstm_fused_fwd_kernel(LstmP p, const double* __restrict__ s1, int nslab, int xcd_map) {
+    static_assert(G16 || !SLAB, "the slab-major gate tensor is bf16");
     __shared__ float sh[LSTM_SUM_FLOATS(16, Q)];
     LT(0);
     constexpr int ROWS = NT / Q;
@@ -1089,6 +1098,7 @@
     const int q = threadIdx.x & (Q - 1), prow = threadIdx.x / Q;
     const int F = p.F, HW = p.HW, c0 = (slab * Q + q) * 4;
     const long long g0 = (long long)n * HW * 4 * F + c0;
+    const long long srow = lstm_slab_row(n, F, c0, HW);
     GateQuad<G16> gq[PPT][4];
     float4 cpq[PPT];
     int pxs[PPT];
@@ -1098,13 +1108,18 @@
         const int px = prow + t * ROWS;
         ok[t] = px < HW;
         pxs[t] = ok[t] ? px : HW - 1;
-        const long long idx = g0 + (long long)pxs[t] * 4 * F;
-#pragma unroll
-        for (int g = 0; g < 4; ++g) gq[t][g].load(p.gates, idx + g * F);
+        if constexpr (SLAB) {
+            load_gate_record(gq[t], p.gates, srow + pxs[t]);
+        } else {
+            const long long idx = g0 + (long long)pxs[t] * 4 * F;
+#pragma unroll
+            for (int g = 0; g < 4; ++g) gq[t][g].load(p.gates, idx + g * F);
+        }
     }
     if (p.c_prev) {
 #pragma unroll
-        for (int t = 0; t < PPT; ++t) cpq[t] = ld4(p.c_prev + (long long)n * p.cp_sn + (long long)pxs[t] * p.cp_sp + c0);
+        for (int t = 0; t < PPT; ++t)
+            cpq[t] = SLAB ? ld4(p.c_prev + (srow + pxs[t]) * 4) : ld4(p.c_prev + (long long)n * p.cp_sn + (long long)pxs[t] * p.cp_sp + c0);
     } else {
 #pragma unroll
         for (int t = 0; t < PPT; ++t) cpq[t] = make_float4(0.f, 0.f, 0.f, 0.f);
@@ -1220,7 +1235,7 @@
             hv[c] = tanhf_(cn[c]) * so[t][c];
         }
         const int px = pxs[t];
-        st4(p.c_new + ((long long)n * HW + px) * F + c0, make_float4(cn[0], cn[1], cn[2], cn[3]));
+        st4(SLAB ? p.c_new + (srow + px) * 4 : p.c_new + ((long long)n * HW + px) * F + c0, make_float4(cn[0], cn[1], cn[2], cn[3]));
         const float4 h4 = make_float4(hv[0], hv[1], hv[2], hv[3]);
 #pragma unroll
         for (int k = 0; k < 4; ++k)
@@ -1231,8 +1246,9 @@
     LT(7);
 }
 
-template <int Q, int PPT, bool G16>
+template <int Q, int PPT, bool G16, bool SLAB>
 __global__ __launch_bounds__(NT) void lstm_fused_bwd_kernel(LstmP p, int nslab, int xcd_map) {
+    static_assert(G16 || !SLAB, "the slab-major gate tensor is bf16");
     __shared__ float sh[LSTM_SUM_FLOATS(32, Q)];
     LT(0);
     constexpr int ROWS = NT / Q;
@@ -1241,6 +1257,7 @@
     const int q = threadIdx.x & (Q - 1), prow = threadIdx.x / Q;
     const int F = p.F, HW = p.HW, c0 = (slab * Q + q) * 4;
     const long long g0 = (long long)n * HW * 4 * F + c0;
+    const long long srow = lstm_slab_row(n, F, c0, HW);
     GateQuad<G16> gq[PPT][4];
     float4 cpq[PPT], dhq[PPT], dcq[PPT];
     int pxs[PPT];
@@ -1250,20 +1267,25 @@
         const int px = prow + t * ROWS;
         okf[t] = px < HW ? 1.f : 0.f;
         pxs[t] = px < HW ? px : HW - 1;
-        const long long idx = g0 + (long long)pxs[t] * 4 * F;
-#pragma unroll
-        for (int g = 0; g < 4; ++g) gq[t][g].load(p.gates, idx + g * F);
+        if constexpr (SLAB) {
+            load_gate_record(gq[t], p.gates, srow + pxs[t]);
+        } else {
+            const long long idx = g0 + (long long)pxs[t] * 4 * F;
+#pragma unroll
+            for (int g = 0; g < 4; ++g) gq[t][g].load(p.gates, idx + g * F);
+        }
         dhq[t] = make_float4(0.f, 0.f, 0.f, 0.f);
         cpq[t] = make_float4(0.f, 0.f, 0.f, 0.f);
         dcq[t] = make_float4(0.f, 0.f, 0.f, 0.f);
     }
     if (p.c_prev) {
 #pragma unroll
-        for (int t = 0; t < PPT; ++t) cpq[t] = ld4(p.c_prev + (long long)n * p.cp_sn + (long long)pxs[t] * p.cp_sp + c0);
+        for (int t = 0; t < PPT; ++t)
+            cpq[t] = SLAB ? ld4(p.c_prev + (srow + pxs[t]) * 4) : ld4(p.c_prev + (long long)n * p.cp_sn + (long long)pxs[t] * p.cp_sp + c0);
     }
     if (p.dc_new) {
 #pragma unroll
-        for (int t = 0; t < PPT; ++t) dcq[t] = ld4(p.dc_new + ((long long)n * HW + pxs[t]) * F + c0);
+        for (int t = 0; t < PPT; ++t) dcq[t] = ld4(SLAB ? p.dc_new + (srow + pxs[t]) * 4 : p.dc_new + ((long long)n * HW + pxs[t]) * F + c0);
     }
     float4 dhs[3][PPT];
     {
@@ -1282,10 +1304,12 @@
         for (int t = 0; t < PPT; ++t) dhq[t] = ld4(p.dh[3] + (long long)n * p.dh_sn[3] + (long long)pxs[t] * p.dh_sp[3] + c0);
     }
     float mu[16], rs[16], ga[16], be[16];
+    int cv = c0;
+    if constexpr (Q == 1 && PPT == 4) asm volatile("" : "+v"(cv));
 #pragma unroll
     for (int g = 0; g < 4; ++g) {
         const long long o = (long long)n * 4 * F + g * F + c0;
-        const float4 m = ld4(p.mean1 + o), r = ld4(p.rstd1 + o), gg = ld4(p.g1 + g * F + c0), bb = ld4(p.b1 + g * F + c0);
+        const float4 m = ld4(p.mean1 + o), r = ld4(p.rstd1 + o), gg = ld4(p.g1 + g * F + cv), bb = ld4(p.b1 + g * F + cv);
         mu[g * 4] = m.x; mu[g * 4 + 1] = m.y; mu[g * 4 + 2] = m.z; mu[g * 4 + 3] = m.w;
         rs[g * 4] = r.x; rs[g * 4 + 1] = r.y; rs[g * 4 + 2] = r.z; rs[g * 4 + 3] = r.w;
         ga[g * 4] = gg.x; ga[g * 4 + 1] = gg.y; ga[g * 4 + 2] = gg.z; ga[g * 4 + 3] = gg.w;
@@ -1360,7 +1384,8 @@
             dg[t][4 + c] = dcpre * si * (1.f - tj * tj);
             dg[t][8 + c] = dcpre * cpv[c] * sf * (1.f - sf);
         }
-        if (p.dc_prev && okf[t] != 0.f) st4(p.dc_prev + ((long long)n * HW + pxs[t]) * F + c0, make_float4(dcp[0], dcp[1], dcp[2], dcp[3]));
+        if (p.dc_prev && okf[t] != 0.f)
+            st4(SLAB ? p.dc_prev + (srow + pxs[t]) * 4 : p.dc_prev + ((long long)n * HW + pxs[t]) * F + c0, make_float4(dcp[0], dcp[1], dcp[2], dcp[3]));
 #pragma unroll
         for (int i = 0; i < 16; ++i) { r1[i] += dg[t][i]; r1[16 + i] += dg[t][i] * xh[t][i]; }
     }
@@ -1411,27 +1436,27 @@
     return true;
 }
 
+#define LSTM_FUSED_DISPATCH_Q(KERNEL, G_, S_, ...)                                                                         \
+    do {                                                                                                                   \
+        if (Q == 1) { if (PPT == 1) KERNEL(1, 1, G_, S_, __VA_ARGS__); else if (PPT == 2) KERNEL(1, 2, G_, S_, __VA_ARGS__); else KERNEL(1, 4, G_, S_, __VA_ARGS__); } \
+        else if (Q == 2) { if (PPT == 1) KERNEL(2, 1, G_, S_, __VA_ARGS__); else if (PPT == 2) KERNEL(2, 2, G_, S_, __VA_ARGS__); else KERNEL(2, 4, G_, S_, __VA_ARGS__); } \
+        else { if (PPT == 1) KERNEL(4, 1, G_, S_, __VA_ARGS__); else if (PPT == 2) KERNEL(4, 2, G_, S_, __VA_ARGS__); else KERNEL(4, 4, G_, S_, __VA_ARGS__); } \
+    } while (0)
 #define LSTM_FUSED_DISPATCH(KERNEL, ...)                                                                                   \
     do {                                                                                                                   \
         const dim3 grid((unsigned)(a->N * nslab));                                                                         \
-        if (a->gates_bf16) {                                                                                               \
-            if (Q == 1) { if (PPT == 1) KERNEL(1, 1, true, __VA_ARGS__); else if (PPT == 2) KERNEL(1, 2, true, __VA_ARGS__); else KERNEL(1, 4, true, __VA_ARGS__); } \
-            else if (Q == 2) { if (PPT == 1) KERNEL(2, 1, true, __VA_ARGS__); else if (PPT == 2) KERNEL(2, 2, true, __VA_ARGS__); else KERNEL(2, 4, true, __VA_ARGS__); } \
-            else { if (PPT == 1) KERNEL(4, 1, true, __VA_ARGS__); else if (PPT == 2) KERNEL(4, 2, true, __VA_ARGS__); else KERNEL(4, 4, true, __VA_ARGS__); } \
-        } else {                                                                                                           \
-            if (Q == 1) { if (PPT == 1) KERNEL(1, 1, false, __VA_ARGS__); else if (PPT == 2) KERNEL(1, 2, false, __VA_ARGS__); else KERNEL(1, 4, false, __VA_ARGS__); } \
-            else if (Q == 2) { if (PPT == 1) KERNEL(2, 1, false, __VA_ARGS__); else if (PPT == 2) KERNEL(2, 2, false, __VA_ARGS__); else KERNEL(2, 4, false, __VA_ARGS__); } \
-            else { if (PPT == 1) KERNEL(4, 1, false, __VA_ARGS__); else if (PPT == 2) KERNEL(4, 2, false, __VA_ARGS__); else KERNEL(4, 4, false, __VA_ARGS__); } \
-        }                                                                                                                  \
+        if (a->slab) LSTM_FUSED_DISPATCH_Q(KERNEL, true, true, __VA_ARGS__);                                               \
+        else if (a->gates_bf16) LSTM_FUSED_DISPATCH_Q(KERNEL, true, false, __VA_ARGS__);                                   \
+        else LSTM_FUSED_DISPATCH_Q(KERNEL, false, false, __VA_ARGS__);                                                     \
     } while (0)
-#define LSTM_FWD_LAUNCH(Q_, P_, G_, ...)                                                                                      \
+#define LSTM_FWD_LAUNCH(Q_, P_, G_, S_, ...)                                                                                  \
     do {                                                                                                                   \
         if (g_savp_prof_start) {                                                                                           \
-            hipExtLaunchKernelGGL((lstm_fused_fwd_kernel<Q_, P_, G_>), grid, dim3(NT), 0, st, g_savp_prof_start, g_savp_prof_stop, 0, __VA_ARGS__); \
+            hipExtLaunchKernelGGL((lstm_fused_fwd_kernel<Q_, P_, G_, S_>), grid, dim3(NT), 0, st, g_savp_prof_start, g_savp_prof_stop, 0, __VA_ARGS__); \
             g_savp_prof_start = g_savp_prof_stop = nullptr;                                                                \
-        } else hipLaunchKernelGGL((lstm_fused_fwd_kernel<Q_, P_, G_>), grid, dim3(NT), 0, st, __VA_ARGS__);                \
+        } else hipLaunchKernelGGL((lstm_fused_fwd_kernel<Q_, P_, G_, S_>), grid, dim3(NT), 0, st, __VA_ARGS__);            \
     } while (0)
-#define LSTM_BWD_LAUNCH(Q_, P_, G_, ...) hipLaunchKernelGGL((lstm_fused_bwd_kernel<Q_, P_, G_>), grid, dim3(NT), 0, st, __VA_ARGS__)
+#define LSTM_BWD_LAUNCH(Q_, P_, G_, S_, ...) hipLaunchKernelGGL((lstm_fused_bwd_kernel<Q_, P_, G_, S_>), grid, dim3(NT), 0, st, __VA_ARGS__)
 
 static int fill_lstm(LstmP& p, const SavpLstmArgs* a) {
     if (!a || a->F % 4 || a->HW < 1) return SAVP_EINVAL;
@@ -1451,6 +1476,13 @@
     p.dgates16 = a->dgates_bf16 ? 1 : 0;
     p.draw = a->dgates_bf16 ? a->dgates_raw : a->dgates;
     p.dg1 = a->dgamma1; p.db1 = a->dbeta1; p.dg2 = a->dgamma2; p.db2 = a->dbeta2;
+    p.slab = a->slab ? 1 : 0;
+    if (a->slab) {
+        auto a16 = [](const void* q) { return (((uintptr_t)q) & 15) == 0; };
+        if (a->no_norm || !a->gates_bf16 || !a16(a->gates) || !a16(a->c_prev.p) || !a16(a->c_new) || !a16(a->dc_new) || !a16(a->dc_prev) ||
+            (a->c_prev.p && (a->c_prev.sn != (long long)a->HW * a->F || a->c_prev.sp != a->F)))
+            return SAVP_EINVAL;
+    }
     return SAVP_OK;
 }
 
@@ -1549,6 +1581,7 @@
             return hipGetLastError() == hipSuccess ? SAVP_OK : SAVP_ELAUNCH;
         }
     }
+    if (a->slab) return SAVP_EINVAL;
     if (lstm_coalesced_ok(a)) {
         const int N = a->N, F = a->F, HW = a->HW;
         LstmWs w;
@@ -1599,6 +1632,7 @@
             return hipGetLastError() == hipSuccess ? SAVP_OK : SAVP_ELAUNCH;
         }
     }
+    if (a->slab) return SAVP_EINVAL;
     if (a->dgates_bf16 && !a->dgates_raw) return SAVP_EINVAL;
     if (lstm_coalesced_ok(a)) {
         hipStream_t st = (hipStream_t)stream;
diff --git a/video_prediction_amd/csrc/opts.h b/video_prediction_amd/csrc/opts.h
--- a/video_prediction_amd/csrc/opts.h
+++ b/video_prediction_amd/csrc/opts.h
@@ -21,6 +21,7 @@
     OPT_GATE_CELL,
     OPT_GATE_WWARM,
     OPT_SPLITK_REDUCED,
+    OPT_GATE_SLAB,
     OPT_COUNT
 };
 
diff --git a/video_prediction_amd/engine.py b/video_prediction_amd/engine.py
--- a/video_prediction_amd/engine.py
+++ b/video_prediction_amd/engine.py
@@ -290,7 +290,7 @@
         if self.sn_u_name:
             self.u.copy_(self.u_next)
 
-    def forward(self, x, y, beta=0, act=0, alpha=0.0, use_bias=True, stats=None, defer=False):
+    def forward(self, x, y, beta=0, act=0, alpha=0.0, use_bias=True, stats=None, defer=False, slab=False):
         b = self.bias if use_bias else None
         if self.kind == 'conv' and x.dim() == 2 and x.shape[0] <= 64 and not act and not beta and y.is_contiguous():
             if defer:
@@ -304,7 +304,7 @@
                 return K.conv(lib.CONV_DGRAD, self.geom, y, x, self.wd, bias=b, beta=beta, act=act, alpha=alpha, w16=self.wd16, stats=stats,
                               defer=True)
             return K.conv(lib.CONV_FPROP, self.geom, x, y, self.wt, bias=b, beta=beta, act=act, alpha=alpha, w16=self.wt16, stats=stats,
-                          defer=True, w_frag=self.wfrag, w_frag_il=self.wfrag_il)
+                          defer=True, w_frag=self.wfrag, w_frag_il=self.wfrag_il, y_slab=slab)
         if self.ktimer is not None:
             self.ktimer.arm()
         if self.prof is not None:
@@ -313,7 +313,8 @@
         if self.kind == 'up':
             K.conv(lib.CONV_DGRAD, self.geom, y, x, self.wd, bias=b, beta=beta, act=act, alpha=alpha, w16=self.wd16, stats=stats)
         else:
-            K.conv(lib.CONV_FPROP, self.geom, x, y, self.wt, bias=b, beta=beta, act=act, alpha=alpha, w16=self.wt16, stats=stats, w_frag=self.wfrag)
+            K.conv(lib.CONV_FPROP, self.geom, x, y, self.wt, bias=b, beta=beta, act=act, alpha=alpha, w16=self.wt16, stats=stats, w_frag=self.wfrag,
+                   y_slab=slab)
         if self.prof is not None:
             e1.record()
             self.prof.append((e0, e1))
diff --git a/video_prediction_amd/kernels.py b/video_prediction_amd/kernels.py
--- a/video_prediction_amd/kernels.py
+++ b/video_prediction_amd/kernels.py
@@ -285,11 +285,12 @@
 
 
 def conv(mode, geom, x, y, w, bias=None, beta=0, act=0, alpha=0.0, aux=None, splitk=0, tile=0, precision=None, w16=None, stats=None,
-         dst_gap=None, norm_bwd=None, defer=False, w_frag=None, w_frag_il=None):
+         dst_gap=None, norm_bwd=None, defer=False, w_frag=None, w_frag_il=None, y_slab=False):
     lib.require_device(w, bias, aux)
     lib.require_stats(stats, (norm_bwd or {}).get('ws'))
     lib.require_device_any(x, y)
     a = _fill_conv_args(mode, geom, x, y, w, bias, beta, act, alpha, aux, splitk, tile, precision, w16, stats, dst_gap, norm_bwd, w_frag, w_frag_il)
+    a.y_slab = int(bool(y_slab))
     if AUTOTUNE['enabled'] and tile == 0 and splitk == 0 and not lib.get().savp_conv_special(ctypes.byref(a)):
         key = (mode, a.precision, a.N, a.D, a.H, a.W, a.Cx, a.Do, a.Ho, a.Wo, a.Cy, geom.k, geom.s, geom.p, a.act, a.beta,
                a.x_sw, a.y_sw, bias is not None, w16 is not None, a.src_bf16, a.out_bf16, stats is not None)
@@ -709,8 +710,10 @@
     return ws, ws[:N * 4 * F * 4].view(torch.float64).view(N, 4 * F, 2)
 
 
-def convlstm_gates_fwd(gates, c_prev, g1, b1, g2, b2, c_new, hs, stats, eps=1e-6, forget_bias=1.0, ws=None, stats1=None, defer=False):
+def convlstm_gates_fwd(gates, c_prev, g1, b1, g2, b2, c_new, hs, stats, eps=1e-6, forget_bias=1.0, ws=None, stats1=None, defer=False,
+                       slab=False):
     a = _lstm_args(gates, c_prev, g1, b1, g2, b2, stats, eps, forget_bias)
+    a.slab = int(bool(slab))
     a.c_new = c_new.data_ptr()
     if ws is not None or stats1 is not None:
         _lstm_ws(a, gates, ws, stats1)
@@ -724,8 +727,9 @@
 
 
 def convlstm_gates_bwd(gates, c_prev, g1, b1, g2, b2, stats, dhs, dc_new, dgates, dc_prev, dparams, eps=1e-6,
-                       forget_bias=1.0, ws=None, dgates_raw=None, defer=False):
+                       forget_bias=1.0, ws=None, dgates_raw=None, defer=False, slab=False):
     a = _lstm_args(gates, c_prev, g1, b1, g2, b2, stats, eps, forget_bias)
+    a.slab = int(bool(slab))
     if dgates.dtype == torch.bfloat16:
         if dgates_raw is None or dgates_raw.dtype != torch.float32 or dgates_raw.numel() < dgates.numel():
             raise ValueError('bf16 dgates need an fp32 dgates_raw scratch of the same size')
@@ -1181,6 +1185,12 @@
             it.Cx, it.Cy = src.shape[-2], src.shape[-1]
             it.T = src.numel() // (it.Cx * it.Cy)
         lib.check(_L().savp_pack_weights_batch(lib.stream(), len(part), arr), 'savp_pack_weights_batch')
+
+
+def gate_slab_ok(geom, x, y, w, w_frag):
+    a = _fill_conv_args(lib.CONV_FPROP, geom, x, y, w, None, 0, 0, 0.0, None, 0, 0, 1, w_frag=w_frag)
+    a.y_slab = 1
+    return bool(lib.get().savp_conv_special(ctypes.byref(a)))
 
 
 def gate_weights_elems(taps, Cx, Cy):
diff --git a/video_prediction_amd/lib.py b/video_prediction_amd/lib.py
--- a/video_prediction_amd/lib.py
+++ b/video_prediction_amd/lib.py
@@ -31,7 +31,7 @@
         ('dst_gap_at', c_i32), ('dst_gap', c_i32),
         ('nb_x', c_vp), ('nb_x_sn', c_i64), ('nb_x_sp', c_i64), ('nb_mean', c_vp), ('nb_rstd', c_vp), ('nb_gamma', c_vp), ('nb_beta', c_vp),
         ('nb_ws', c_vp), ('nb_c0', c_i32), ('nb_nc', c_i32), ('nb_act', c_i32), ('nb_alpha', c_f32),
-        ('w_frag', c_vp), ('w_frag_il', c_vp),
+        ('w_frag', c_vp), ('w_frag_il', c_vp), ('y_slab', c_i32),
     ]
 
 
@@ -81,7 +81,8 @@
 
 
 OPTION_NAMES = ('conv_ring', 's2dgrad', 'thin', 'wgp_cfg', 'wgp_split', 'inorm_min_hw', 'colsum_2stage', 'dense_legacy', 'cdna_legacy',
-                'lstm_fused', 'ring_dma', 'lstm_q', 'ring_wwarm', 'wgp_dma', 'ring_early', 'gate_kernel', 'gate_alt', 'gate_cell', 'gate_wwarm', 'splitk_reduced')
+                'lstm_fused', 'ring_dma', 'lstm_q', 'ring_wwarm', 'wgp_dma', 'ring_early', 'gate_kernel', 'gate_alt', 'gate_cell', 'gate_wwarm', 'splitk_reduced',
+                'gate_slab')
 
 
 def set_option(name, value):
@@ -242,6 +243,7 @@
         ('dgamma1', c_vp), ('dbeta1', c_vp), ('dgamma2', c_vp), ('dbeta2', c_vp),
         ('ws', c_vp), ('ws_floats', ctypes.c_int64), ('ws_stats', c_vp), ('ws_stats_clean', c_i32),
         ('gates_bf16', c_i32), ('stats1_ready', c_i32), ('h_bf16', c_i32), ('dgates_bf16', c_i32), ('dgates_raw', c_vp), ('no_norm', c_i32),
+        ('slab', c_i32),
     ]
 
 
diff --git a/video_prediction_amd/models/savp_cell.py b/video_prediction_amd/models/savp_cell.py
--- a/video_prediction_amd/models/savp_cell.py
+++ b/video_prediction_amd/models/savp_cell.py
@@ -244,6 +244,8 @@
                 L['rconv'] = ConvLayer(store, r + 'kernel', (r + 'bias') if self.cell_plain else None, 'conv', (5, 5), (1, 1), (2, 2))
                 if not self.cell_plain and not self.cell_ln:
                     L['rconv'].enable_gate_pack(cell=bool(L['fused']) and h_ * w_ <= 256)
+                L['slab'] = bool(L['fused'] and L['rconv'].wfrag is not None and lib.get_option('gate_slab') and lib.get_option('lstm_fused') and
+                                 h_ * w_ <= 1024 and K.gate_slab_ok(L['rconv'].geom, L['a'].v[0], L['gates'].v[0], L['rconv'].W, L['rconv'].wfrag))
                 if self.cell_ln:
                     L['gn4'] = ConcatNorm([Norm(store, r + nm + '/', T1, N, f, dev, groups=1) for nm in ('input', 'transform', 'forget', 'output')],
                                           T1, N, dev)
@@ -512,7 +514,10 @@
                 if L['rnn']:
                     f, hoff = L['f'], L['f'] + L['zr']
                     L['a'].v[0][..., hoff:hoff + f].copy_(L['h0v'])
-                    if not self.gru:
+                    if not self.gru and L.get('slab'):
+                        hw = L['c0v'].shape[0] * L['c0v'].shape[1]
+                        L['c0'].view(N, f // 4, hw, 4).copy_(L['c0v'].reshape(hw, f // 4, 4).permute(1, 0, 2))
+                    elif not self.gru:
                         L['c0'].copy_(L['c0v'])
         in0, maskin = self.layers[0]['in'], self.maskin
         if self._ones is None:
@@ -609,20 +614,21 @@
                     gk = L.get('gate_ktimer')
                     gargs = (L['gates'].v[t], L['c'].v[t - 1] if t > 0 else L.get('c0'), n1.gamma, n1.beta, n2.gamma, n2.beta, L['c'].v[t], outs,
                              [n1.mean[t], n1.rstd[t], n2.mean[t], n2.rstd[t]])
-                    ca = (L['rconv'].forward(a.v[t], L['gates'].v[t], use_bias=False, stats=s1, defer=True)
+                    slab = L['slab']
+                    ca = (L['rconv'].forward(a.v[t], L['gates'].v[t], use_bias=False, stats=s1, defer=True, slab=slab)
                           if (FUSED_ENTRIES and cp is None and gk is None and K.fused_ok()) else None)
                     if ca is not None:
                         ck = L.get('cell_ktimer')
                         if ck is not None:
                             ck.arm()
-                        K.convlstm_cell_fwd(ca, K.convlstm_gates_fwd(*gargs, eps=EPS_IN, ws=self._lstm_ws(L), stats1=stats1, defer=True))
+                        K.convlstm_cell_fwd(ca, K.convlstm_gates_fwd(*gargs, eps=EPS_IN, ws=self._lstm_ws(L), stats1=stats1, defer=True, slab=slab))
                         if ck is not None:
                             ck.taken()
                     else:
-                        L['rconv'].forward(a.v[t], L['gates'].v[t], use_bias=False, stats=s1)
+                        L['rconv'].forward(a.v[t], L['gates'].v[t], use_bias=False, stats=s1, slab=slab)
                         if gk is not None:
                             gk.arm()
-                        K.convlstm_gates_fwd(*gargs, eps=EPS_IN, ws=self._lstm_ws(L), stats1=stats1)
+                        K.convlstm_gates_fwd(*gargs, eps=EPS_IN, ws=self._lstm_ws(L), stats1=stats1, slab=slab)
                         if gk is not None:
                             gk.taken()
                     if cp is not None:
@@ -877,9 +883,10 @@
                         nb['mean'], nb['rstd'] = nrm.mean[t], nrm.rstd[t]
                     if FUSED_ENTRIES and K.fused_ok():
                         K.convlstm_cell_bwd(L['rconv'].backward_data(L['gates'].g[t], a.g[t], beta=0, skip=skip, norm_bwd=nb, defer=True),
-                                            K.convlstm_gates_bwd(*bargs, eps=EPS_IN, ws=self._lstm_ws(L), dgates_raw=L.get('dg_raw'), defer=True))
+                                            K.convlstm_gates_bwd(*bargs, eps=EPS_IN, ws=self._lstm_ws(L), dgates_raw=L.get('dg_raw'), defer=True,
+                                                                 slab=L['slab']))
                     else:
-                        K.convlstm_gates_bwd(*bargs, eps=EPS_IN, ws=self._lstm_ws(L), dgates_raw=L.get('dg_raw'))
+                        K.convlstm_gates_bwd(*bargs, eps=EPS_IN, ws=self._lstm_ws(L), dgates_raw=L.get('dg_raw'), slab=L['slab'])
                         L['rconv'].backward_data(L['gates'].g[t], a.g[t], beta=0, skip=skip, norm_bwd=nb)
                     self._in_act_conv_bwd(L, t, a.v[t][..., 0:f], [a.g[t][..., 0:f]], nb['ws'] if nb is not None else None)
                     continue
@@ -897,7 +904,10 @@
                 if L['rnn']:
                     f, hoff = L['f'], L['f'] + L['zr']
                     L['h0g'].add_(L['a'].g[0][..., hoff:hoff + f].float().sum(0))
-                    if not self.gru:
+                    if not self.gru and L.get('slab'):
+                        hh, ww = L['c0g'].shape[0], L['c0g'].shape[1]
+                        L['c0g'].add_(L['dc'][0].sum(0).view(f // 4, hh * ww, 4).permute(1, 0, 2).reshape(hh, ww, f))
+                    elif not self.gru:
                         L['c0g'].add_(L['dc'][0].sum(0))
         for L in self.layers:
             b, pre = L['in'], L['pre']
```
